# MonsieurETM/QPSK

Measured on AMD Instinct MI355X. Metric: complex Msamples/s demodulated + % HBM roofline, 2400-baud RRC+Costas path, higher is better.
Workload: dtype f32

## Files before the change

### include/qpsk_hip.h

```cpp
#ifndef QPSK_HIP_H
#define QPSK_HIP_H

#include <stddef.h>
#include <stdint.h>

#ifdef __cplusplus
extern "C" {
#endif

#define QPSK_NTAPS 127

typedef enum {
    QPSK_OK = 0,
    QPSK_ERR_NO_DEVICE = -1,
    QPSK_ERR_ARG = -2,
    QPSK_ERR_HIP = -3,
    QPSK_ERR_ALLOC = -4,
    QPSK_ERR_STATE = -5,
    QPSK_ERR_RANGE = -6
} qpsk_status;

typedef enum {
    QPSK_TIMING_HIST = 0,
    QPSK_TIMING_FIXED = 1,
    QPSK_TIMING_FFT = 2
} qpsk_timing_mode;

typedef struct {
    double fs;
    double rs;
    int frame_size;
    float rrc_alpha;
    float loop_bw;
    float min_freq;
    float max_freq;
    int timing_mode;
    int fixed_index;
} qpsk_params;

typedef struct qpsk_ctx qpsk_ctx;

const char *qpsk_last_error(void);
const char *qpsk_version(void);
int qpsk_device_count(void);

void qpsk_params_default(qpsk_params *p);

int qpsk_ctx_create(qpsk_ctx **out, int device, const qpsk_params *p, void *stream);
void qpsk_ctx_destroy(qpsk_ctx *ctx);
int qpsk_ctx_sync(qpsk_ctx *ctx);
int qpsk_ctx_check(qpsk_ctx *ctx);
int qpsk_ctx_set_stream(qpsk_ctx *ctx, void *stream);
int qpsk_ctx_set_tuning(qpsk_ctx *ctx, const char *name, int value);
int qpsk_ctx_cycles(const qpsk_ctx *ctx);
int qpsk_ctx_nsym(const qpsk_ctx *ctx);
const char *qpsk_ctx_last_kernel(const qpsk_ctx *ctx);

int qpsk_ctx_get_taps(const qpsk_ctx *ctx, float h_taps[QPSK_NTAPS]);
int qpsk_ctx_get_gains(const qpsk_ctx *ctx, float *h_alpha, float *h_beta);
int qpsk_ctx_set_taps(qpsk_ctx *ctx, const float h_taps[QPSK_NTAPS]);
int qpsk_ctx_set_loop(qpsk_ctx *ctx, float alpha, float beta, float min_freq, float max_freq);

int qpsk_rx_batch(qpsk_ctx *ctx, const float *d_in, int nframes, uint8_t *d_sym, float *d_freq,
                  float *d_phase, float *d_costas, int32_t *d_index, float *d_hz);

int qpsk_rx_batch_pitched(qpsk_ctx *ctx, const float *d_in, long long frame_pitch, int nframes, uint8_t *d_sym,
                          float *d_freq, float *d_phase, float *d_costas, int32_t *d_index, float *d_hz);

int qpsk_rx_batch_bw(qpsk_ctx *ctx, const float *d_in, int nframes, const float *h_loop_bw, int nbw,
                     uint8_t *d_sym, float *d_freq, float *d_phase, int32_t *d_index);

int qpsk_rx_batch_ext(qpsk_ctx *ctx, const float *d_in, long long frame_pitch, int nframes, const int32_t *d_index_in,
                      const float *d_seed, uint8_t *d_sym, float *d_freq, float *d_phase, float *d_costas, int32_t *d_index,
                      float *d_hz);
int qpsk_rx_batch_data(qpsk_ctx *ctx, const float *d_in, long long frame_pitch, int nframes, const int32_t *d_index_in,
                       const float *d_seed, uint8_t *d_data, uint8_t *d_sym, float *d_freq, float *d_phase, int32_t *d_index,
                       float *d_hz);

int qpsk_sync_batch(qpsk_ctx *ctx, const uint8_t *d_data, int nframes, int nsym, const uint8_t *h_sync, int nsync, int lag_min,
                    int lag_max, int nout, uint8_t *d_out, int32_t *d_lag, int32_t *d_rot, int32_t *d_score);

int qpsk_deframer_reset(qpsk_ctx *ctx, int nstreams, const uint8_t *h_sync, int nsync, int min_score, int nbytes, int max_packets);
int qpsk_deframer_push(qpsk_ctx *ctx, const float *d_costas, const uint8_t *d_data, int nsym, int32_t *d_count, uint8_t *d_bytes,
                       long long *d_pos, int32_t *d_rot, int32_t *d_score, uint8_t *d_crc_ok);

int qpsk_deframer_reset_coded(qpsk_ctx *ctx, int nstreams, const uint8_t *h_sync, int nsync, int min_score, int nbytes,
                              int max_packets, int mode, float scale);
int qpsk_deframer_push_coded(qpsk_ctx *ctx, const float *d_costas, int nsym, const float *d_gain, int32_t *d_count,
                             uint8_t *d_bytes, long long *d_pos, int32_t *d_rot, int32_t *d_score, uint8_t *d_crc_ok,
                             int32_t *d_info);

int qpsk_deframer_reset_coded_punct(qpsk_ctx *ctx, int nstreams, const uint8_t *h_sync, int nsync, int min_score, int nbytes,
                                    int max_packets, int mode, float scale, int period, uint32_t keep0, uint32_t keep1);

int qpsk_rx_batch_bw_ext(qpsk_ctx *ctx, const float *d_in, int nframes, const float *h_loop_bw, int nbw, const int32_t *d_index_in,
                         const float *d_seed, uint8_t *d_sym, float *d_freq, float *d_phase, int32_t *d_index);

int qpsk_carrier_est_batch(qpsk_ctx *ctx, const float *d_in, long long frame_pitch, int nframes, int start, int n,
                           float *d_seed, float *d_freq, int32_t *d_bin, double *d_line);

enum { QPSK_SOFT_UNIT = 0, QPSK_SOFT_LLR = 1 };
int qpsk_soft_batch(qpsk_ctx *ctx, const float *d_costas, long long row_pitch, int nrows, int nsym, int skip, int mode, float scale,
                    const float *d_gain_in, const int32_t *d_lag, const int32_t *d_rot, int first, int nout, int8_t *d_soft,
                    float *d_quality, double *d_sums);

enum { QPSK_CONV_TAIL = 1 };
enum { QPSK_VITERBI_OPEN_START = 1, QPSK_VITERBI_OPEN_END = 2 };
int qpsk_conv_encode_batch(qpsk_ctx *ctx, const uint8_t *d_bits, int nrows, int nbits, int flags, uint8_t *d_dibits);
int qpsk_viterbi_batch(qpsk_ctx *ctx, const int8_t *d_soft, long long row_pitch, int nrows, int nsteps, const uint8_t *d_flip,
                       int flags, uint8_t *d_bits, int32_t *d_info);

#define QPSK_PUNCT_1_2 1, 0x1u, 0x1u
#define QPSK_PUNCT_2_3 2, 0x1u, 0x3u
#define QPSK_PUNCT_3_4 3, 0x5u, 0x3u
#define QPSK_PUNCT_5_6 5, 0x15u, 0x0Bu
#define QPSK_PUNCT_7_8 7, 0x51u, 0x2Fu
int qpsk_punct_ntx(int nsteps, int period, uint32_t keep0, uint32_t keep1);
int qpsk_conv_encode_punct_batch(qpsk_ctx *ctx, const uint8_t *d_bits, int nrows, int nbits, int flags, int period, uint32_t keep0,
                                 uint32_t keep1, uint8_t *d_dibits);
int qpsk_viterbi_punct_batch(qpsk_ctx *ctx, const int8_t *d_soft, long long row_pitch, int nrows, int nsteps, int period, uint32_t keep0,
                             uint32_t keep1, const uint8_t *d_flip, int flags, uint8_t *d_bits, int32_t *d_info);

enum { QPSK_FRAME_UNCODED = 0, QPSK_FRAME_CODED = 1 };
int qpsk_frame_len(int nsync, int nbytes, int coding, int period, uint32_t keep0, uint32_t keep1);
int qpsk_frame_batch(qpsk_ctx *ctx, const uint8_t *d_payload, long long payload_pitch, int nrows, int per_row, int nbytes,
                     const uint8_t *h_sync, int nsync, int coding, int period, uint32_t keep0, uint32_t keep1, int lead, int gap,
                     int row_len, uint8_t *d_out, uint16_t *d_crc);

int qpsk_ilv_stride(int nbits, int want);
int qpsk_conv_encode_ilv_batch(qpsk_ctx *ctx, const uint8_t *d_bits, int nrows, int nbits, int flags, int period, uint32_t keep0,
                               uint32_t keep1, int stride, uint8_t *d_dibits);
int qpsk_viterbi_ilv_batch(qpsk_ctx *ctx, const int8_t *d_soft, long long row_pitch, int nrows, int nsteps, int period, uint32_t keep0,
                           uint32_t keep1, int stride, const uint8_t *d_flip, int flags, uint8_t *d_bits, int32_t *d_info);
int qpsk_frame_batch_ilv(qpsk_ctx *ctx, const uint8_t *d_payload, long long payload_pitch, int nrows, int per_row, int nbytes,
                         const uint8_t *h_sync, int nsync, int coding, int period, uint32_t keep0, uint32_t keep1, int stride, int lead,
                         int gap, int row_len, uint8_t *d_out, uint16_t *d_crc);
int qpsk_deframer_reset_coded_ilv(qpsk_ctx *ctx, int nstreams, const uint8_t *h_sync, int nsync, int min_score, int nbytes,
                                  int max_packets, int mode, float scale, int period, uint32_t keep0, uint32_t keep1, int stride);

int qpsk_rs_generator(int nroots, uint8_t *h_g);
int qpsk_rs_encode_batch(qpsk_ctx *ctx, const uint8_t *d_data, long long data_pitch, int nrows, int k, int nroots, uint8_t *d_out,
                         long long out_pitch);
int qpsk_rs_decode_batch(qpsk_ctx *ctx, const uint8_t *d_in, long long in_pitch, int nrows, int n, int nroots, const uint8_t *d_erase,
                         uint8_t *d_out, long long out_pitch, int32_t *d_info);

enum { QPSK_VITERBI_STREAM_TERMINATED = 1 };
int qpsk_viterbi_stream_reset(qpsk_ctx *ctx, int nstreams, int depth, int window, int period, uint32_t keep0, uint32_t keep1);
int qpsk_viterbi_stream_emits(qpsk_ctx *ctx, int ntx);
int qpsk_viterbi_stream_push(qpsk_ctx *ctx, const int8_t *d_soft, long long row_pitch, int ntx, uint8_t *d_bits, long long bits_pitch,
                             int32_t *d_info, int *h_nbits);
int qpsk_viterbi_stream_flush(qpsk_ctx *ctx, int flags, uint8_t *d_bits, long long bits_pitch, int32_t *d_info, int *h_nbits);
int qpsk_conv_encode_stream_batch(qpsk_ctx *ctx, const uint8_t *d_bits, int nrows, int nbits, int period, uint32_t keep0, uint32_t keep1,
                                  const uint8_t *d_state_in, uint8_t *d_state_out, uint8_t *d_dibits);


int qpsk_rrc_fir_batch(qpsk_ctx *ctx, float *d_memory, const float *d_in, float *d_out, int nframes, int length);

int qpsk_rrc_fir_batch_fast(qpsk_ctx *ctx, float *d_memory, const float *d_in, float *d_out, int nframes, int length);

int qpsk_timing_hist_batch(qpsk_ctx *ctx, const float *d_filtered, int nframes, int32_t *d_index, int32_t *d_hist);

int qpsk_timing_scan_batch(qpsk_ctx *ctx, const float *d_in, int nframes, int32_t *d_index, int32_t *d_hist);

int qpsk_timing_fft_batch(qpsk_ctx *ctx, const float *d_in, int nframes, int32_t *d_index, float *d_filtered,
                          double *d_spectrum);

int qpsk_timing_fft_bin_batch(qpsk_ctx *ctx, const float *d_in, int nframes, int32_t *d_index, float *d_filtered,
                              double *d_bin);

int qpsk_costas_batch(qpsk_ctx *ctx, const float *d_symbols_in, int nframes, int nsym, float *d_state,
                      uint8_t *d_sym, float *d_costas);

int qpsk_fft_batch(qpsk_ctx *ctx, const double *d_in, double *d_out, int nbatch, int n, int inverse);

int qpsk_streams_reset(qpsk_ctx *ctx, int nstreams, double mixer_hz);
int qpsk_streams_set_loop_state(qpsk_ctx *ctx, const float *h_state);
int qpsk_streams_get_loop_state(qpsk_ctx *ctx, float *h_state);
int qpsk_streams_rx_cplx(qpsk_ctx *ctx, const float *d_in, uint8_t *d_sym, float *d_freq, float *d_phase,
                         float *d_costas, int32_t *d_index);
int qpsk_streams_rx_pcm(qpsk_ctx *ctx, const int16_t *d_pcm, uint8_t *d_sym, float *d_freq, float *d_phase,
                        float *d_costas, int32_t *d_index);
int qpsk_streams_rx_pcm_host(qpsk_ctx *ctx, const int16_t *h_pcm, float *h_loop_io, uint8_t *h_sym, float *h_costas,
                             int32_t *h_index);

int qpsk_tx_reset(qpsk_ctx *ctx, int nstreams, double tx_hz);
int qpsk_tx_symbols(qpsk_ctx *ctx, const uint8_t *d_symbols, int nsym, int16_t *d_pcm, float *d_baseband);


int qpsk_crc16_batch(qpsk_ctx *ctx, const uint8_t *d_data, int npackets, int nbytes, uint16_t *d_crc);

int qpsk_interleave_batch(qpsk_ctx *ctx, uint8_t *d_data, int npackets, int nbytes, int dir);

int qpsk_scramble_batch(qpsk_ctx *ctx, uint8_t *d_sym, int npackets, int nsym);

typedef struct qpsk_multi qpsk_multi;
int qpsk_multi_create(qpsk_multi **out, const int *devices, int ndev, const qpsk_params *p);
void qpsk_multi_destroy(qpsk_multi *mj);
int qpsk_multi_shards(const qpsk_multi *mj);
int qpsk_multi_load(qpsk_multi *mj, long long total_frames, const float *h_in);
int qpsk_multi_shard(qpsk_multi *mj, int r, int *device, long long *first, long long *count, qpsk_ctx **ctx, float **d_in);
int qpsk_multi_use_device_input(qpsk_multi *mj, int r, const float *d_in);
int qpsk_multi_set_direct_output(qpsk_multi *mj, int slot, uint8_t *h_sym, float *h_freq, float *h_phase);
int qpsk_multi_set_packed(qpsk_multi *mj, int on);
int qpsk_pack_symbols(qpsk_ctx *ctx, const uint8_t *d_sym, long long nrows, int nsym, uint8_t *d_packed);
int qpsk_unpack_symbols_host(const uint8_t *h_packed, long long nrows, int nsym, uint8_t *h_sym);
int qpsk_host_alloc(void **h_ptr, size_t bytes);
int qpsk_host_free(void *h_ptr);
int qpsk_multi_set_acquisition(qpsk_multi *mj, const int32_t *h_index, const float *h_seed);
int qpsk_multi_set_data(qpsk_multi *mj, int on);
int qpsk_multi_rx_begin(qpsk_multi *mj, int slot);
int qpsk_multi_rx_end(qpsk_multi *mj, int slot, uint8_t *h_sym, float *h_freq, float *h_phase);

int qpsk_dev_alloc(qpsk_ctx *ctx, void **d_ptr, size_t bytes);
int qpsk_dev_free(qpsk_ctx *ctx, void *d_ptr);
int qpsk_dev_upload(qpsk_ctx *ctx, void *d_dst, const void *h_src, size_t bytes);
int qpsk_dev_download(qpsk_ctx *ctx, void *h_dst, const void *d_src, size_t bytes);

int qpsk_selftest_sincos_hash(qpsk_ctx *ctx, uint32_t first, uint32_t count, unsigned long long *h_out);

int qpsk_test_inject_status(qpsk_ctx *ctx, int code);
int qpsk_test_hist_state(qpsk_ctx *ctx, int32_t *out);
int qpsk_test_fir_runs(qpsk_ctx *ctx, int nframes, int length, int32_t out[3]);
int qpsk_test_viterbi_launches(qpsk_ctx *ctx, int *out);
int qpsk_test_deframer_advance(qpsk_ctx *ctx, long long delta);
int qpsk_test_viterbi_stream_advance(qpsk_ctx *ctx, long long delta);

#ifdef __cplusplus
}
#endif
#endif
```

### qpsk_amd/csrc/api_ctx.cpp

```cpp
#include "api_ctx.h"

using namespace qpsk;

static thread_local char g_err[512] = "";

int qpsk::fail(int code, const char *fmt, ...)
{
    va_list ap;
    va_start(ap, fmt);
    vsnprintf(g_err, sizeof g_err, fmt, ap);
    va_end(ap);
    return code;
}

static const struct { const char *name; int Tuning::*field; } TUNING_KEYS[] = {
    {"QPSK_FUSED_G", &Tuning::fused_g},       {"QPSK_FUSED_S", &Tuning::fused_s},     {"QPSK_FUSED_LDS", &Tuning::fused_lds},
    {"QPSK_FUSED_GENERIC", &Tuning::generic}, {"QPSK_PIPE_NF", &Tuning::pipe_nf},
    {"QPSK_PIPE_DBG", &Tuning::pipe_variant}, {"QPSK_HIST_GENERIC", &Tuning::hist_generic},
    {"QPSK_PIPE_V", &Tuning::pipe_v},         {"QPSK_PIPE_G", &Tuning::pipe_g},
    {"QPSK_PIPE_LAYOUT_LO", &Tuning::layout_lo}, {"QPSK_PIPE_LAYOUT_HI", &Tuning::layout_hi},
    {"QPSK_FIR_GENERIC", &Tuning::fir_generic}, {"QPSK_FFT_FUSED", &Tuning::fft_fused},
    {"QPSK_STREAM_BLOCK", &Tuning::stream_block}, {"QPSK_STREAM_POLL", &Tuning::stream_poll},
    {"QPSK_STREAM_SCAN", &Tuning::stream_scan}, {"QPSK_STREAM_CARRIER", &Tuning::stream_carrier},
    {"QPSK_LEAN_DMA", &Tuning::lean_dma},     {"QPSK_LEAN_PAIR", &Tuning::lean_pair},
    {"QPSK_EST_WAVES", &Tuning::est_waves},   {"QPSK_HIST_ONEPASS", &Tuning::hist_onepass},
    {"QPSK_VITERBI_LDS", &Tuning::viterbi_lds},   {"QPSK_VITERBI_CHUNK_ROWS", &Tuning::viterbi_chunk_rows},
};

int qpsk::ensure(qpsk_ctx *c, DevBuf &b, size_t bytes)
{
    if (b.cap >= bytes) return QPSK_OK;
    if (b.p) {
        HIP_TRY(hipStreamSynchronize(c->stream));
        HIP_TRY(hipFree(b.p));
        b.p = nullptr;
        b.cap = 0;
    }
    hipError_t e = hipMalloc(&b.p, bytes);
    if (e != hipSuccess) {
        b.p = nullptr;
        return fail(QPSK_ERR_ALLOC, "hipMalloc(%zu bytes): %s", bytes, hipGetErrorString(e));
    }
    b.cap = bytes;
    return QPSK_OK;
}

int qpsk::check_status(qpsk_ctx *c)
{
    const int st = __atomic_exchange_n(c->status.h_status, 0, __ATOMIC_ACQ_REL);
    if (st != STATUS_PIPE_TIMEOUT) c->streams.stream_work_unchecked = false;
    if (st == STATUS_PIPE_TIMEOUT) {
        if (c->streams.nstreams > 0 && c->streams.stream_work_unchecked) c->streams.poison();
        c->streams.stream_work_unchecked = false;
        return fail(QPSK_ERR_HIP, "pipeline kernel: producer/consumer wait timed out; results of the calls since the last synchronisation are invalid");
    }
    if (st == STATUS_PHASE_RANGE)
        return fail(QPSK_ERR_RANGE, "Costas loop phase beyond the bounded 2 pi wrap (input amplitude far outside the modem's range; "
                                    "the reference's phase_wrap() would spin or hang, costas_loop.c:61-67); results of the calls since the last synchronisation are invalid");
    if (st == STATUS_BAD_INDEX)
        return fail(QPSK_ERR_ARG, "an external timing offset (qpsk_rx_batch_ext d_index_in) lies outside 0..%d: the kernel demodulated that frame "
                                  "at offset 0; results of the calls since the last synchronisation are invalid", MAX_INDEX);
    if (st == STATUS_EST_NONFINITE)
        return fail(QPSK_ERR_RANGE, "qpsk_carrier_est_batch: a NaN / Inf sample inside the window the estimate reads; results of the calls since "
                                    "the last synchronisation are invalid");
    if (st == STATUS_SOFT_NONFINITE)
        return fail(QPSK_ERR_RANGE, "qpsk_soft_batch / qpsk_deframer_push_coded: a NaN / Inf sample among those a row's sums or soft output use, or a NaN / Inf gain; "
                                    "results of the calls since the last synchronisation are invalid");
    if (st == STATUS_SOFT_BAD_LAG)
        return fail(QPSK_ERR_ARG, "qpsk_soft_batch: a lag in d_lag is negative or puts the payload beyond the row (that row's soft output is zeros); "
                                  "results of the calls since the last synchronisation are invalid");
    if (st == STATUS_NONFINITE)
        return fail(QPSK_ERR_RANGE, "a Costas loop ended on a NaN / Inf state: the input held a non-finite sample (the reference hangs in phase_wrap() "
                                    "on an infinite phase, costas_loop.c:61-67); results of the calls since the last synchronisation are invalid");
    if (st != 0) return fail(QPSK_ERR_HIP, "kernel status %d", st);
    return QPSK_OK;
}

int qpsk_test_inject_status(qpsk_ctx *c, int code)
{
    if (!c || !c->status.h_status) return fail(QPSK_ERR_ARG, "null context");
    __atomic_store_n(c->status.h_status, code, __ATOMIC_RELEASE);
    return QPSK_OK;
}

int qpsk::bind(const qpsk_ctx *c)
{
    HIP_TRY(hipSetDevice(c->device));
    return QPSK_OK;
}

int qpsk::use_context_gains(qpsk_ctx *c)
{
    const float g[2] = {c->alpha, c->beta};
    if (c->h_gains.size() != 2 || c->h_gains[0] != g[0] || c->h_gains[1] != g[1]) {
        HIP_TRY(hipStreamSynchronize(c->stream));
        c->h_gains.assign(g, g + 2);
        HIP_TRY(hipMemcpyAsync(c->d_gains, c->h_gains.data(), sizeof g, hipMemcpyHostToDevice, c->stream));
    }
    return QPSK_OK;
}

const char *qpsk_last_error(void) { return g_err; }
const char *qpsk_version(void) { return "qpsk_hip 0.3 (gfx950)"; }

int qpsk_device_count(void)
{
    int n = 0;
    if (hipGetDeviceCount(&n) != hipSuccess) return 0;
    return n;
}

void qpsk_params_default(qpsk_params *p)
{
    if (!p) return;
    p->fs = 9600.0;
    p->rs = 2400.0;
    p->frame_size = 512;
    p->rrc_alpha = .35f;
    p->loop_bw = (float)(2.0 * 3.14159265358979323846 / 100.0f);
    p->min_freq = -1.0f;
    p->max_freq = 1.0f;
    p->timing_mode = QPSK_TIMING_HIST;
    p->fixed_index = 0;
}

static int upload_config(qpsk_ctx *c)
{
    float t128[128];
    memset(t128, 0, sizeof t128);
    memcpy(t128, c->taps, sizeof c->taps);
    c->taps_symmetric = true;
    for (int k = 0; k < QPSK_NTAPS / 2; k++)
        if (memcmp(&c->taps[k], &c->taps[QPSK_NTAPS - 1 - k], sizeof(float)) != 0) c->taps_symmetric = false;
    HIP_TRY(hipMemcpyAsync(c->d_taps, t128, sizeof t128, hipMemcpyHostToDevice, c->stream));
    const float g[2] = {c->alpha, c->beta};
    c->h_gains.assign(g, g + 2);
    HIP_TRY(hipMemcpyAsync(c->d_gains, c->h_gains.data(), sizeof g, hipMemcpyHostToDevice, c->stream));
    HIP_TRY(hipStreamSynchronize(c->stream));
    return QPSK_OK;
}

int qpsk_ctx_create(qpsk_ctx **out, int device, const qpsk_params *p, void *stream)
{
    if (!out || !p) return fail(QPSK_ERR_ARG, "qpsk_ctx_create: null argument");
    *out = nullptr;
    int ndev = 0;
    hipError_t e = hipGetDeviceCount(&ndev);
    if (e != hipSuccess || ndev <= 0)
        return fail(QPSK_ERR_NO_DEVICE, "no HIP device available (%s); this library has no CPU path",
                    e == hipSuccess ? "device count 0" : hipGetErrorString(e));
    if (device < 0) HIP_TRY(hipGetDevice(&device));
    if (device >= ndev) return fail(QPSK_ERR_NO_DEVICE, "device %d out of range (%d devices)", device, ndev);
    if (!(p->fs > 0.0) || !(p->rs > 0.0) || p->frame_size <= 0)
        return fail(QPSK_ERR_ARG, "fs, rs and frame_size must be positive");
    const int cycles = (int)(p->fs / p->rs);
    if (cycles < 1 || cycles > 64) return fail(QPSK_ERR_ARG, "CYCLES = (int)(fs/rs) = %d out of range 1..64", cycles);
    if (p->frame_size % cycles != 0)
        return fail(QPSK_ERR_ARG, "frame_size %d is not a multiple of CYCLES %d", p->frame_size, cycles);
    if (p->timing_mode < QPSK_TIMING_HIST || p->timing_mode > QPSK_TIMING_FFT)
        return fail(QPSK_ERR_ARG, "unknown timing_mode %d", p->timing_mode);
    if (p->fixed_index < 0 || p->fixed_index > MAX_INDEX)
        return fail(QPSK_ERR_ARG, "fixed_index %d outside 0..%d", p->fixed_index, MAX_INDEX);

    HIP_TRY(hipSetDevice(device));
    KERNEL_TRY(prepare_kernels());
    KERNEL_TRY(prepare_pipe_kernel());
    KERNEL_TRY(prepare_timing_scan());
    KERNEL_TRY(prepare_stream_block());
    KERNEL_TRY(prepare_stream_scan());
    KERNEL_TRY(prepare_carrier_est());
    qpsk_ctx *c = new qpsk_ctx();
    c->device = device;
    for (const auto &k : TUNING_KEYS) {
        const char *v = getenv(k.name);
        if (!v || !*v) continue;
        if (k.field == &Tuning::viterbi_chunk_rows) {
            char *end = nullptr;
            const long n = strtol(v, &end, 10);
            if (end == v || *end) continue;
            c->tune.*(k.field) = n < 0 ? -1 : n > INT_MAX ? INT_MAX : (int)n;
            continue;
        }
        c->tune.*(k.field) = atoi(v);
    }
    if (c->tune.viterbi_chunk_rows == 0) {
        delete c;
        return fail(QPSK_ERR_ARG, "qpsk_ctx_create: QPSK_VITERBI_CHUNK_ROWS = 0 in the environment (>= 1, or negative for the library's own choice)");
    }
    {
        int ncu = 0;
        if (hipDeviceGetAttribute(&ncu, hipDeviceAttributeMultiprocessorCount, device) == hipSuccess && ncu > 0)
            c->ncu = ncu;
    }
    c->prm = *p;
    c->cycles = cycles;
    c->nsym = p->frame_size / cycles;
    c->stream = (hipStream_t)stream;
    qpsk_host_rrc_taps((float)p->fs, (float)p->rs, p->rrc_alpha, c->taps);
    c->damping = sqrtf(2.0f) / 2.0f;
    qpsk_host_loop_gains(c->damping, p->loop_bw, &c->alpha, &c->beta);
    c->min_freq = p->min_freq;
    c->max_freq = p->max_freq;
    if (hipMalloc((void **)&c->d_taps, 128 * sizeof(float)) != hipSuccess ||
        hipMalloc((void **)&c->d_gains, MAX_BW * 2 * sizeof(float)) != hipSuccess ||
        hipHostMalloc((void **)&c->status.h_status, sizeof(int), hipHostMallocMapped) != hipSuccess ||
        hipHostGetDevicePointer((void **)&c->status.d_status, c->status.h_status, 0) != hipSuccess) {
        qpsk_ctx_destroy(c);
        return fail(QPSK_ERR_ALLOC, "hipMalloc of configuration buffers failed");
    }
    *c->status.h_status = 0;
    if (hipHostMalloc((void **)&c->streams.h_done, sizeof(unsigned), hipHostMallocMapped) != hipSuccess ||
        hipHostGetDevicePointer((void **)&c->streams.d_done, c->streams.h_done, 0) != hipSuccess) {
        qpsk_ctx_destroy(c);
        return fail(QPSK_ERR_ALLOC, "pinned counter");
    }
    *c->streams.h_done = 0;
    int rc = upload_config(c);
    if (rc != QPSK_OK) { qpsk_ctx_destroy(c); return rc; }
    *out = c;
    return QPSK_OK;
}

void qpsk_ctx_destroy(qpsk_ctx *c)
{
    if (!c) return;
    hipSetDevice(c->device);
    hipStreamSynchronize(c->stream);
    hipFree(c->d_taps);
    hipFree(c->d_gains);
    if (c->status.h_status) hipHostFree(c->status.h_status);
    if (c->streams.h_done) hipHostFree(c->streams.h_done);
    for (DevBuf *b : {&c->index, &c->filtered, &c->mixed, &c->keystream, &c->sympad, &c->mislist, &c->datacostas, &c->vitdec, &c->softgain, &c->dfstage})
        b->release();
    for (auto &kv : c->twiddles) hipFree(kv.second);
    hipFree(c->d_fast);
    c->hist.release();
    c->streams.release();
    c->tx.release();
    c->df.release();
    c->framer.release();
    c->vs.release();
    delete c;
}

int qpsk_ctx_sync(qpsk_ctx *c)
{
    if (!c) return fail(QPSK_ERR_ARG, "null context");
    HIP_TRY(hipSetDevice(c->device));
    HIP_TRY(hipStreamSynchronize(c->stream));
    return check_status(c);
}

int qpsk_pack_symbols(qpsk_ctx *c, const uint8_t *d_sym, long long nrows, int nsym, uint8_t *d_packed)
{
    if (!c || !d_sym || !d_packed || nrows < 0 || nsym <= 0) return fail(QPSK_ERR_ARG, "qpsk_pack_symbols: bad argument");
    if (bind(c)) return QPSK_ERR_HIP;
    if ((nsym & 15) == 0 && (((uintptr_t)d_sym & 15) || ((uintptr_t)d_packed & 3)))
        return fail(QPSK_ERR_ARG, "qpsk_pack_symbols: d_sym must be 16-byte and d_packed 4-byte aligned");
    KERNEL_TRY(launch_pack_dibits(d_sym, d_packed, (size_t)nrows, nsym, c->stream));
    return QPSK_OK;
}

int qpsk_unpack_symbols_host(const uint8_t *h_packed, long long nrows, int nsym, uint8_t *h_sym)
{
    if (!h_packed || !h_sym || nrows < 0 || nsym <= 0) return fail(QPSK_ERR_ARG, "qpsk_unpack_symbols_host: bad argument");
    const size_t pb = (size_t)(nsym + 3) / 4;
    for (long long r = 0; r < nrows; r++) {
        const uint8_t *p = h_packed + (size_t)r * pb;
        uint8_t *o = h_sym + (size_t)r * (size_t)nsym;
        for (int i = 0; i < nsym; i++) o[i] = (uint8_t)((p[i >> 2] >> (2 * (i & 3))) & 3u);
    }
    return QPSK_OK;
}

int qpsk_ctx_check(qpsk_ctx *c)
{
    if (!c) return fail(QPSK_ERR_ARG, "null context");
    return check_status(c);
}

extern "C" int qpsk_set_error(int code, const char *msg)
{
    return fail(code, "%s", msg ? msg : "");
}

int qpsk_ctx_set_stream(qpsk_ctx *c, void *stream)
{
    if (!c) return fail(QPSK_ERR_ARG, "null context");
    HIP_TRY(hipSetDevice(c->device));
    HIP_TRY(hipStreamSynchronize(c->stream));
    c->stream = (hipStream_t)stream;
    return QPSK_OK;
}

int qpsk_ctx_set_tuning(qpsk_ctx *c, const char *name, int value)
{
    if (!c || !name) return fail(QPSK_ERR_ARG, "null argument");
    for (const auto &k : TUNING_KEYS)
        if (!strcmp(k.name, name)) {
            if (value == 0 && k.field == &Tuning::viterbi_chunk_rows)
                return fail(QPSK_ERR_ARG, "qpsk_ctx_set_tuning: QPSK_VITERBI_CHUNK_ROWS = 0 (>= 1, or negative for the library's own choice)");
            c->tune.*(k.field) = value < 0 ? -1 : value;
            return QPSK_OK;
        }
    return fail(QPSK_ERR_ARG, "qpsk_ctx_set_tuning: unknown name '%s'", name);
}

int qpsk_ctx_cycles(const qpsk_ctx *c) { return c ? c->cycles : 0; }
int qpsk_ctx_nsym(const qpsk_ctx *c) { return c ? c->nsym : 0; }
const char *qpsk_ctx_last_kernel(const qpsk_ctx *c) { return c ? c->last_kernel : ""; }

int qpsk_ctx_get_taps(const qpsk_ctx *c, float *h)
{
    if (!c || !h) return fail(QPSK_ERR_ARG, "null argument");
    memcpy(h, c->taps, sizeof c->taps);
    return QPSK_OK;
}

int qpsk_ctx_get_gains(const qpsk_ctx *c, float *a, float *b)
{
    if (!c || !a || !b) return fail(QPSK_ERR_ARG, "null argument");
    *a = c->alpha;
    *b = c->beta;
    return QPSK_OK;
}

int qpsk_ctx_set_taps(qpsk_ctx *c, const float *h)
{
    if (!c || !h) return fail(QPSK_ERR_ARG, "null argument");
    if (bind(c)) return QPSK_ERR_HIP;
    memcpy(c->taps, h, sizeof c->taps);
    c->fast_valid = false;
    return upload_config(c);
}

int qpsk_ctx_set_loop(qpsk_ctx *c, float alpha, float beta, float min_freq, float max_freq)
{
    if (!c) return fail(QPSK_ERR_ARG, "null argument");
    if (bind(c)) return QPSK_ERR_HIP;
    c->min_freq = min_freq; c->max_freq = max_freq;
    if (alpha == c->alpha && beta == c->beta && !(alpha == 0.0f && beta == 0.0f)) return QPSK_OK;
    c->alpha = alpha; c->beta = beta;
    return upload_config(c);
}

int qpsk_dev_alloc(qpsk_ctx *c, void **d_ptr, size_t bytes)
{
    if (!c || !d_ptr) return fail(QPSK_ERR_ARG, "null argument");
    if (bind(c)) return QPSK_ERR_HIP;
    hipError_t e = hipMalloc(d_ptr, bytes);
    if (e != hipSuccess) return fail(QPSK_ERR_ALLOC, "hipMalloc(%zu): %s", bytes, hipGetErrorString(e));
    return QPSK_OK;
}

int qpsk_dev_free(qpsk_ctx *c, void *d_ptr)
{
    if (!c) return fail(QPSK_ERR_ARG, "null argument");
    if (bind(c)) return QPSK_ERR_HIP;
    HIP_TRY(hipStreamSynchronize(c->stream));
    HIP_TRY(hipFree(d_ptr));
    return QPSK_OK;
}

int qpsk_dev_upload(qpsk_ctx *c, void *d_dst, const void *h_src, size_t bytes)
{
    if (!c || !d_dst || !h_src) return fail(QPSK_ERR_ARG, "null argument");
    if (bind(c)) return QPSK_ERR_HIP;
    HIP_TRY(hipMemcpyAsync(d_dst, h_src, bytes, hipMemcpyHostToDevice, c->stream));
    HIP_TRY(hipStreamSynchronize(c->stream));
    return QPSK_OK;
}

int qpsk_dev_download(qpsk_ctx *c, void *h_dst, const void *d_src, size_t bytes)
{
    if (!c || !h_dst || !d_src) return fail(QPSK_ERR_ARG, "null argument");
    if (bind(c)) return QPSK_ERR_HIP;
    HIP_TRY(hipMemcpyAsync(h_dst, d_src, bytes, hipMemcpyDeviceToHost, c->stream));
    HIP_TRY(hipStreamSynchronize(c->stream));
    return check_status(c);
}

int qpsk_selftest_sincos_hash(qpsk_ctx *c, uint32_t first, uint32_t count, unsigned long long *h_out)
{
    if (!c || !h_out) return fail(QPSK_ERR_ARG, "null argument");
    if (bind(c)) return QPSK_ERR_HIP;
    unsigned long long *d = nullptr;
    HIP_TRY(hipMalloc((void **)&d, sizeof *d));
    HIP_TRY(hipMemsetAsync(d, 0, sizeof *d, c->stream));
    KERNEL_TRY(launch_sincos_hash(first, count, d, c->stream));
    HIP_TRY(hipMemcpyAsync(h_out, d, sizeof *d, hipMemcpyDeviceToHost, c->stream));
    HIP_TRY(hipStreamSynchronize(c->stream));
    HIP_TRY(hipFree(d));
    return QPSK_OK;
}
```

### qpsk_amd/csrc/api_ctx.h

```cpp
#ifndef QPSK_API_CTX_H
#define QPSK_API_CTX_H

#include "../../include/qpsk_hip.h"
#include "host_math.h"
#include "kernels.h"

#include <hip/hip_runtime.h>
#include <limits.h>
#include <math.h>
#include <stdarg.h>
#include <stdio.h>
#include <stdlib.h>
#include <string.h>
#include <time.h>
#include <algorithm>
#include <initializer_list>
#include <map>
#include <vector>

struct qpsk_ctx;

namespace qpsk {

QPSK_UNIT_LOCAL int fail(int code, const char *fmt, ...);

#define HIP_TRY(expr)                                                                         \
    do {                                                                                      \
        hipError_t e_ = (expr);                                                               \
        if (e_ != hipSuccess)                                                                 \
            return fail(QPSK_ERR_HIP, "%s: %s (%s:%d)", #expr, hipGetErrorString(e_), __FILE__, __LINE__); \
    } while (0)

#define KERNEL_TRY(expr)                                                                      \
    do {                                                                                      \
        (void)hipGetLastError();  \
        int e_ = (expr);                                                                      \
        if (e_ != 0)                                                                          \
            return fail(QPSK_ERR_HIP, "%s: %s (%s:%d)", #expr, hipGetErrorString((hipError_t)e_), __FILE__, __LINE__); \
    } while (0)

struct QPSK_UNIT_LOCAL DevBuf {
    void *p = nullptr;
    size_t cap = 0;
    void release() { hipFree(p); *this = DevBuf(); }
};

struct Tuning {
    int fused_g = -1, fused_s = -1, fused_lds = -1;
    int generic = -1;
    int pipe_nf = -1;
    int pipe_v = -1, pipe_g = -1;
    int layout_lo = -1, layout_hi = -1;
    int pipe_variant = -1;
    int hist_generic = -1;
    int fir_generic = -1;
    int stream_scan = -1;
    int stream_poll = -1;
    int stream_block = -1;
    int stream_carrier = -1;
    int lean_dma = -1;
    int hist_onepass = -1;
    int est_waves = -1;
    int lean_pair = -1;
    int viterbi_lds = -1;
    int fft_fused = -1;
    int viterbi_chunk_rows = -1;
};

static inline int tuned(int v, int dflt) { return v >= 0 ? v : dflt; }


struct StatusWord {
    int *h_status = nullptr;
    int *d_status = nullptr;
};

struct QPSK_UNIT_LOCAL HistGuess {
    int32_t *d_hint = nullptr;
    int32_t *h_hist_stats = nullptr, *d_hist_stats = nullptr;
    bool hint_valid = false;
    void release();
};

struct QPSK_UNIT_LOCAL Streams {
    int nstreams = 0;
    float *s_memory = nullptr, *s_dec = nullptr, *s_loop = nullptr, *s_mixer = nullptr;
    float *s_ctab = nullptr, *s_cstate = nullptr;
    bool carrier_shared = false;
    unsigned carrier_blocks = 0;
    unsigned carrier_scans = 0;
    float *carrier_pending = nullptr;
    bool stream_work_unchecked = false;
    bool streams_poisoned = false;
    unsigned char *h_stage = nullptr, *d_stage = nullptr;
    size_t stage_cap = 0;
    unsigned *h_done = nullptr, *d_done = nullptr;
    unsigned done_expect = 0;
    void poison()
    {
        streams_poisoned = true;
        carrier_shared = false;
        carrier_pending = nullptr;
    }
    void release();
};

struct QPSK_UNIT_LOCAL Transmitters {
    int ntx = 0;
    uint8_t *t_hist = nullptr;
    float *t_mixer = nullptr;
    DevBuf tx_b;
    void release();
};

struct QPSK_UNIT_LOCAL Deframer {
    uint8_t *state = nullptr, *tables = nullptr;
    size_t stride = 0;
    int nstreams = 0, nsync = 0, min_score = 0, nbytes = 0, max_packets = 0;
    unsigned long long sync_lo[2] = {0, 0}, sync_hi[2] = {0, 0};
    bool ready = false;
    bool coded = false;
    int mode = 0, nsteps = 0;
    int nbody = 0;
    CodedLayout layout;
    float scale = 0.f;
    unsigned crc_init = 0;
    void release();
};

struct QPSK_UNIT_LOCAL Framer {
    uint8_t *ks = nullptr;
    int ks_len = 0;
    void release();
};

struct QPSK_UNIT_LOCAL ViterbiStream {
    uint8_t *state = nullptr;
    size_t stride = 0;
    int nstreams = 0, depth = 0, window = 0;
    Puncture punct = {1, 1u, 1u, 2};
    bool punctured = false;
    long long total = 0;
    long long advanced = 0;
    void release();
};

}

struct qpsk_ctx {
    int device = 0;
    qpsk::Tuning tune;
    int ncu = 256;
    const char *last_kernel = "";
    int viterbi_launches = 0;
    bool taps_symmetric = false;
    hipStream_t stream = nullptr;
    qpsk_params prm{};
    int cycles = 0, nsym = 0;
    float taps[QPSK_NTAPS];
    float damping = 0.f, alpha = 0.f, beta = 0.f;
    float min_freq = 0.f, max_freq = 0.f;
    float *d_taps = nullptr;
    float *d_gains = nullptr;
    std::vector<float> h_gains;
    qpsk::DevBuf index, filtered, mixed, keystream, sympad, mislist;
    qpsk::DevBuf datacostas;
    qpsk::DevBuf vitdec;
    qpsk::DevBuf softgain;
    qpsk::DevBuf dfstage;
    int keystream_len = 0;
    std::map<int, double *> twiddles;
    float *d_fast = nullptr;
    bool fast_valid = false;
    qpsk::StatusWord status;
    qpsk::HistGuess hist;
    qpsk::Streams streams;
    qpsk::Transmitters tx;
    qpsk::Deframer df;
    qpsk::Framer framer;
    qpsk::ViterbiStream vs;
};

namespace qpsk {

static const int MAX_BW = 64;

QPSK_UNIT_LOCAL int ensure(qpsk_ctx *c, DevBuf &b, size_t bytes);
QPSK_UNIT_LOCAL int check_status(qpsk_ctx *c);
QPSK_UNIT_LOCAL int bind(const qpsk_ctx *c);
QPSK_UNIT_LOCAL int use_context_gains(qpsk_ctx *c);

QPSK_UNIT_LOCAL int fir_full_rate(qpsk_ctx *c, const float *x, const float *memory, float *y, int nframes, int length, size_t in_pitch = 0);
QPSK_UNIT_LOCAL int fft_timing_indices(qpsk_ctx *c, const float *d_in, int nframes, int32_t *d_index, float *d_y = nullptr,
                                       double *d_X = nullptr, size_t pitch = 0, double *d_bin = nullptr);
QPSK_UNIT_LOCAL int costas_over_symbols(qpsk_ctx *c, float *d_symbols, int nframes, int nsym, int dstride, float *d_state,
                                        uint8_t *d_sym, float *d_costas, const float *refill = nullptr,
                                        const int32_t *refill_index = nullptr, bool refill_planar = false);

struct Pattern {
    int period;
    uint32_t keep0, keep1;
};
QPSK_UNIT_LOCAL int layout_add_pattern(const char *who, const Pattern *pattern, CodedLayout *l);
QPSK_UNIT_LOCAL int layout_add_stride(const char *who, int nsteps, const int *stride, CodedLayout *l);
struct ViterbiRoute {
    size_t per_row;
    bool lds;
    size_t chunk_rows;
};
QPSK_UNIT_LOCAL ViterbiRoute viterbi_route(const qpsk_ctx *c, size_t rows, int nsteps);

}

#endif
```

### qpsk_amd/csrc/api_rx.cpp

```cpp
#include "api_ctx.h"

using namespace qpsk;

#ifdef QPSK_PIPE_PROFILE
static const int PIPE_VARIANT_MASK = ~0;
#else
static const int PIPE_VARIANT_MASK = 4 | 8 | 16 | 64 | 128 | 256 | 512 | 1024 | 8192;
#endif

int qpsk_test_hist_state(qpsk_ctx *c, int32_t *out)
{
    if (!c || !out) return fail(QPSK_ERR_ARG, "null argument");
    out[0] = out[1] = out[2] = out[3] = out[4] = -1;
    if (!c->hist.d_hint) return QPSK_OK;
    HIP_TRY(hipSetDevice(c->device));
    HIP_TRY(hipStreamSynchronize(c->stream));
    int32_t h[2];
    HIP_TRY(hipMemcpy(h, c->hist.d_hint, sizeof h, hipMemcpyDeviceToHost));
    out[0] = c->hist.hint_valid ? h[0] : -1;
    out[1] = h[1];
    out[2] = c->hist.h_hist_stats[0]; out[3] = c->hist.h_hist_stats[1]; out[4] = c->hist.h_hist_stats[2];
    return QPSK_OK;
}

int qpsk_test_fir_runs(qpsk_ctx *c, int nframes, int length, int32_t out[3])
{
    if (!c || !out) return fail(QPSK_ERR_ARG, "qpsk_test_fir_runs: null argument");
    if (nframes < 1 || length < 1) return fail(QPSK_ERR_ARG, "qpsk_test_fir_runs: nframes %d length %d", nframes, length);
    const FirRuns r = rrc_fir_stream_runs(nframes, length, c->ncu);
    out[0] = r.ntiles; out[1] = r.parts; out[2] = r.tpp;
    return QPSK_OK;
}

void HistGuess::release()
{
    if (d_hint) hipFree(d_hint);
    if (h_hist_stats) hipHostFree(h_hist_stats);
    *this = HistGuess();
}

static bool fir_takes_stream(const qpsk_ctx *c) { return c->taps_symmetric && tuned(c->tune.fir_generic, 0) == 0; }

int qpsk::fir_full_rate(qpsk_ctx *c, const float *x, const float *memory, float *y, int nframes, int length, size_t in_pitch)
{
    if (fir_takes_stream(c))
        return launch_rrc_fir_stream(x, memory, y, c->d_taps, nframes, length, c->stream, in_pitch, c->ncu);
    return launch_rrc_fir(x, memory, y, c->d_taps, nframes, length, c->stream, in_pitch);
}

static void pick_tiling(const qpsk_ctx *c, int nframes, int nbw, int *G, int *S)
{
    int g = nframes / 256;
    if (g < 1) g = 1;
    if (g > 64 / nbw) g = 64 / nbw;
    if (g < 1) g = 1;
    g = tuned(c->tune.fused_g, g);
    if (g < 1) g = 1;
    if (g * nbw > 64) g = 64 / nbw;
    int s = tuned(c->tune.fused_s, 64);
    s &= ~7;
    if (s < 8) s = 8;
    const size_t budget = (size_t)tuned(c->tune.fused_lds, 64 * 1024);
    while (s > 8 && fused_lds_bytes(g, s, c->cycles, nbw) > budget) s -= 8;
    while (g > 1 && fused_lds_bytes(g, s, c->cycles, nbw) > (size_t)MAX_LDS_BYTES) g--;
    *G = g;
    *S = s;
}

static int get_twiddles(qpsk_ctx *c, int n, double **out)
{
    auto it = c->twiddles.find(n);
    if (it != c->twiddles.end()) { *out = it->second; return QPSK_OK; }
    const size_t cnt = n >= 2 ? (size_t)n / 2 : 1;
    std::vector<double> h(2 * cnt, 0.0);
    qpsk_host_twiddles(n, h.data());
    double *tw = nullptr;
    HIP_TRY(hipMalloc((void **)&tw, sizeof(double) * 2 * cnt));
    HIP_TRY(hipMemcpy(tw, h.data(), sizeof(double) * 2 * cnt, hipMemcpyHostToDevice));
    c->twiddles[n] = tw;
    *out = tw;
    return QPSK_OK;
}

static int fft_timing_tables(qpsk_ctx *c, double **tw_out, double **cs_out)
{
    const int C = c->cycles, nfft = timing_fft_nfft();
    if (C < 2 || C > 8 || (C & (C - 1)))
        return fail(QPSK_ERR_ARG, "QPSK_TIMING_FFT needs CYCLES in {2,4,8} (the symbol-rate bin NFFT/CYCLES must be exact and the offset < 8); CYCLES = %d", C);
    if (c->prm.frame_size < timing_fft_first() + nfft)
        return fail(QPSK_ERR_ARG, "QPSK_TIMING_FFT needs frame_size >= %d", timing_fft_first() + nfft);
    double *tw = nullptr;
    int rc = get_twiddles(c, nfft, &tw);
    if (rc) return rc;
    double *cs = nullptr;
    auto it = c->twiddles.find(-C);
    if (it == c->twiddles.end()) {
        std::vector<double> full(2 * (size_t)C);
        qpsk_host_phases(C, full.data());
        HIP_TRY(hipMalloc((void **)&cs, sizeof(double) * 2 * C));
        HIP_TRY(hipMemcpy(cs, full.data(), sizeof(double) * 2 * C, hipMemcpyHostToDevice));
        c->twiddles[-C] = cs;
    } else {
        cs = it->second;
    }
    *tw_out = tw;
    *cs_out = cs;
    return QPSK_OK;
}

int qpsk::fft_timing_indices(qpsk_ctx *c, const float *d_in, int nframes, int32_t *d_index, float *d_y, double *d_X, size_t pitch, double *d_bin)
{
    double *tw = nullptr, *cs = nullptr;
    int rc = fft_timing_tables(c, &tw, &cs);
    if (rc) return rc;
    KERNEL_TRY(launch_timing_fft(d_in, nframes, c->prm.frame_size, c->cycles, c->d_taps, tw, cs, d_index, d_y, d_X, d_bin, c->stream, pitch,
                                 c->ncu, c->taps_symmetric && tuned(c->tune.fir_generic, 0) == 0));
    return QPSK_OK;
}

static bool scan_fused_ok(const qpsk_ctx *c, const float *d_in)
{
    return c->cycles == 8 && c->prm.frame_size % timing_scan_tile() == 0 && ((uintptr_t)d_in % 16) == 0 &&
           tuned(c->tune.hist_generic, 0) == 0;
}

static int timing_indices(qpsk_ctx *c, const float *d_in, size_t pitch, int nframes, const int32_t **d_index_out, bool fused_fft = false)
{
    *d_index_out = nullptr;
    if (c->prm.timing_mode == QPSK_TIMING_FIXED) return QPSK_OK;
    int rc = ensure(c, c->index, sizeof(int32_t) * (size_t)nframes);
    if (rc) return rc;
    if (fused_fft && c->prm.timing_mode == QPSK_TIMING_FFT) return QPSK_OK;
    if (c->prm.timing_mode == QPSK_TIMING_HIST) {
        if (scan_fused_ok(c, d_in) && (pitch & 1) == 0) {
            KERNEL_TRY(launch_timing_scan(d_in, nframes, c->prm.frame_size, c->d_taps, (int32_t *)c->index.p, nullptr,
                                          c->status.d_status, c->stream, pitch, c->taps_symmetric && tuned(c->tune.fir_generic, 0) == 0));
            *d_index_out = (const int32_t *)c->index.p;
            return QPSK_OK;
        }
        const size_t bytes = sizeof(float) * 2 * (size_t)nframes * c->prm.frame_size;
        rc = ensure(c, c->filtered, bytes);
        if (rc) return rc;
        KERNEL_TRY(fir_full_rate(c, d_in, nullptr, (float *)c->filtered.p, nframes, c->prm.frame_size, pitch));
        KERNEL_TRY(launch_timing_hist((const float *)c->filtered.p, nframes, c->prm.frame_size, c->cycles,
                                      (int32_t *)c->index.p, nullptr, tuned(c->tune.hist_generic, 0) == 2, c->stream));
        *d_index_out = (const int32_t *)c->index.p;
        return QPSK_OK;
    }
    rc = fft_timing_indices(c, d_in, nframes, (int32_t *)c->index.p, nullptr, nullptr, pitch);
    if (rc) return rc;
    *d_index_out = (const int32_t *)c->index.p;
    return QPSK_OK;
}

struct ExtAcq {
    const int32_t *index;
    const float *seed;
};

enum RxKind { K_GENERIC, K_FUSED_PIPE, K_PIPE2, K_LEAN };

struct RxRoute {
    RxKind kind = K_GENERIC;
    int G = 0;
    int nf = 0;
    unsigned long long layout = 0;
    bool pipe_ok = false;
    bool fused_fft = false;
    bool need_pad = false;
    bool data_rule = false;
    bool need_dump = false;
};

static bool tuned_layout(const qpsk_ctx *c, unsigned long long *layout)
{
    if (c->tune.layout_lo < 0 && c->tune.layout_hi < 0) return false;
    *layout = ((unsigned long long)(unsigned)tuned(c->tune.layout_lo, 0) << 4) | ((unsigned long long)(unsigned)tuned(c->tune.layout_hi, 0) << 24);
    return true;
}

static int rx_route(const qpsk_ctx *c, const FusedArgs &a, bool want_data, RxRoute *rt)
{
    const int nframes = a.nframes, nbw = a.nbw;
    *rt = RxRoute{};
    const bool pipe_ok = rt->pipe_ok = c->cycles == pipe_cycles() && (a.frame_size % 2) == 0 && (a.frame_pitch % 2) == 0 &&
                                       ((uintptr_t)a.x % 16) == 0 && nbw * pipe_frames(1) <= 64 && tuned(c->tune.generic, 0) == 0;
    const int by_size = nframes > 16 * c->ncu ? 2 : 1;
    int pipe_v = tuned(c->tune.pipe_v, by_size);
    unsigned long long own_layout = 0;
    const bool has_layout = tuned_layout(c, &own_layout);

    if (pipe_ok && c->taps_symmetric && (pipe_v == 3 || c->tune.pipe_v < 0) && !(want_data && !a.data_rule)) {
        int G = tuned(c->tune.pipe_g, (nframes + c->ncu - 1) / c->ncu);
        if (G > pipe2_max_frames()) G = pipe2_max_frames();
        G += G & 1;
        const bool wanted = pipe_v == 3 || G >= 4;
        const unsigned long long layout = has_layout ? own_layout : G >= 2 ? lean_default_layout(G / 2) : 0;
        if (wanted && layout && lean_shape_ok(a, G)) {
            const LayoutCount n = layout_count(layout);
            if (n.units == G / 2 && lean_lds_bytes(G, n.nwin) <= (size_t)MAX_LDS_BYTES) {
                rt->kind = K_LEAN;
                rt->G = G;
                rt->layout = layout;
                rt->need_pad = nframes % G != 0;
                rt->data_rule = a.data_rule != 0;
            }
        }
    }
    const bool older = rt->kind != K_LEAN && pipe_ok;
    if (pipe_v == 3) pipe_v = by_size;
    if (older && pipe_v == 2) {
        int G = tuned(c->tune.pipe_g, (nframes + c->ncu - 1) / c->ncu);
        if (G > pipe2_max_frames()) G = pipe2_max_frames();
        if (G * nbw > 64) G = 64 / nbw;
        if (G < 1) G = 1;
        unsigned long long layout = own_layout;
        if (has_layout) {
            const LayoutCount n = layout_count(layout);
            if (n.units < 1 || (G + 1) / 2 != n.units || pipe2_lds_bytes(G, n.nwin, nbw) > (size_t)MAX_LDS_BYTES)
                return fail(QPSK_ERR_ARG, "QPSK_PIPE_LAYOUT_*: %d units on %d waves do not match %d frames per workgroup", n.units, n.nwin, G);
        } else {
            for (;;) {
                layout = pipe2_default_layout((G + 1) / 2);
                if (layout && pipe2_lds_bytes(G, layout_count(layout).nwin, nbw) <= (size_t)MAX_LDS_BYTES) break;
                if (G == 1) return fail(QPSK_ERR_ARG, "pipeline geometry does not fit: %d loops per frame", nbw);
                G--;
            }
        }
        rt->kind = K_PIPE2;
        rt->G = G;
        rt->layout = layout;
    } else if (older) {
        const int full = pipe_max_nf();
        int nf = 1;
        while (nf < full && (long long)c->ncu * pipe_frames(nf) < nframes) nf++;
        nf = tuned(c->tune.pipe_nf, nf);
        if (nf < 1) nf = 1;
        if (nf > full) nf = full;
        while (pipe_frames(nf) * nbw > 64 || pipe_lds_bytes(nf, nbw) > (size_t)MAX_LDS_BYTES) {
            if (nf == 1) return fail(QPSK_ERR_ARG, "pipeline geometry does not fit: nf %d, %d loops per frame", nf, nbw);
            nf--;
        }
        rt->kind = K_FUSED_PIPE;
        rt->nf = nf;
    }
    rt->need_dump = want_data && !rt->data_rule && !a.costas;
    rt->fused_fft = c->prm.timing_mode == QPSK_TIMING_FFT && !a.index && nbw == 1 && tuned(c->tune.fft_fused, 1) != 0 &&
                    a.frame_size >= timing_fft_first() + timing_fft_nfft() &&
                    ((rt->kind == K_FUSED_PIPE && rt->nf == pipe_max_nf() && !(a.dbg & (128 | 4))) ||
                     (rt->kind == K_LEAN && lean_est_ok(a, rt->G, rt->layout)));
    return QPSK_OK;
}

static int rx_hist_onepass(qpsk_ctx *c, const FusedArgs &a, const RxRoute &rt, int32_t *d_index, bool *taken)
{
    *taken = false;
    if (!rt.pipe_ok || !c->taps_symmetric || !scan_fused_ok(c, (const float *)a.x) || c->tune.pipe_v >= 0) return QPSK_OK;
    if (!c->hist.d_hint) {
        int32_t *hint = nullptr, *h_stats = nullptr, *d_stats = nullptr;
        hipError_t e = hipMalloc((void **)&hint, 2 * sizeof(int32_t));
        if (e == hipSuccess) e = hipMemset(hint, 0, 2 * sizeof(int32_t));
        if (e == hipSuccess) e = hipHostMalloc((void **)&h_stats, 4 * sizeof(int32_t), hipHostMallocMapped);
        if (e == hipSuccess) e = hipHostGetDevicePointer((void **)&d_stats, h_stats, 0);
        if (e != hipSuccess) {
            if (h_stats) hipHostFree(h_stats);
            if (hint) hipFree(hint);
            return fail(QPSK_ERR_ALLOC, "one-pass histogram route: %s", hipGetErrorString(e));
        }
        h_stats[0] = h_stats[1] = h_stats[2] = -1;
        c->hist.d_hint = hint;
        c->hist.h_hist_stats = h_stats;
        c->hist.d_hist_stats = d_stats;
        c->hist.hint_valid = false;
    }
    const int op = tuned(c->tune.hist_onepass, -1);
    const int seen = __atomic_load_n(&c->hist.h_hist_stats[1], __ATOMIC_ACQUIRE), off_majority = __atomic_load_n(&c->hist.h_hist_stats[2], __ATOMIC_ACQUIRE);
    const bool guess_is_good = seen > 0 && off_majority == 0;
    if (op == 0 || !c->hist.hint_valid || !(op == 1 || guess_is_good) || !rx_hist_shape_ok(a)) return QPSK_OK;
    if (int rc = ensure(c, c->index, sizeof(int32_t) * (size_t)a.nframes)) return rc;
    if (int rc = ensure(c, c->mislist, sizeof(int32_t) * (size_t)a.nframes)) return rc;
    int32_t *mis_count = c->hist.d_hint + 1;
    HIP_TRY(hipMemsetAsync(mis_count, 0, sizeof(int32_t), c->stream));
    KERNEL_TRY(launch_rx_hist(a, (int32_t *)c->index.p, c->hist.d_hint, (int32_t *)c->mislist.p, mis_count, c->status.d_status, c->stream));
    FusedArgs af = a;
    af.index = (const int32_t *)c->index.p;
    af.frame_list = (const int32_t *)c->mislist.p;
    af.frame_list_count = mis_count;
    af.G = 4;
    af.S = 64;
    KERNEL_TRY(launch_rx_fused(af, c->stream));
    KERNEL_TRY(launch_index_majority((const int32_t *)c->index.p, a.nframes, c->hist.d_hint, mis_count, c->hist.d_hist_stats, c->stream));
    c->last_kernel = "rx_hist_kernel (one pass on the guessed index) + rx_fused_kernel (fall-back list)";
    if (d_index)
        HIP_TRY(hipMemcpyAsync(d_index, c->index.p, sizeof(int32_t) * (size_t)a.nframes, hipMemcpyDeviceToDevice, c->stream));
    *taken = true;
    return QPSK_OK;
}

static int rx_launch(qpsk_ctx *c, const FusedArgs &a, const RxRoute &rt)
{
    if (a.est_tw && !(rt.kind == K_FUSED_PIPE && rt.nf == pipe_max_nf()) && rt.kind != K_LEAN)
        return fail(QPSK_ERR_STATE, "internal: in-launch FFT timing estimate planned for a kernel that has none");
    if (a.data_rule && rt.kind != K_LEAN)
        return fail(QPSK_ERR_STATE, "internal: data rule planned for a kernel that has none");
    switch (rt.kind) {
    case K_LEAN:
        KERNEL_TRY(launch_rx_lean(a, rt.G, rt.layout, c->status.d_status, c->stream));
        c->last_kernel = a.est_tw ? "rx_lean_kernel (FFT timing estimate inside the launch)" : "rx_lean_kernel";
        break;
    case K_PIPE2:
        KERNEL_TRY(launch_rx_pipe2(a, rt.G, rt.layout, c->status.d_status, c->stream));
        c->last_kernel = "rx_pipe2_kernel";
        break;
    case K_FUSED_PIPE:
        KERNEL_TRY(launch_rx_fused_pipe(a, rt.nf, c->status.d_status, c->stream));
        c->last_kernel = a.est_tw ? "rx_fused_pipe_kernel (FFT timing estimate inside the launch)" : "rx_fused_pipe_kernel";
        break;
    default:
        KERNEL_TRY(launch_rx_fused(a, c->stream));
        c->last_kernel = "rx_fused_kernel";
    }
    return QPSK_OK;
}

static int rx_batch_common(qpsk_ctx *c, const float *d_in, long long frame_pitch, int nframes, int nbw, uint8_t *d_sym,
                           float *d_freq, float *d_phase, float *d_costas, int32_t *d_index, float *d_hz,
                           const ExtAcq *ext = nullptr, uint8_t *d_data = nullptr)
{
    if (!c || !d_in || !(d_sym || d_data)) return fail(QPSK_ERR_ARG, "qpsk_rx_batch: null context, input or symbol buffer");
    if (nframes <= 0) return fail(QPSK_ERR_ARG, "qpsk_rx_batch: nframes = %d", nframes);
    if (frame_pitch == 0) frame_pitch = c->prm.frame_size;
    if (frame_pitch < c->prm.frame_size)
        return fail(QPSK_ERR_ARG, "qpsk_rx_batch_pitched: frame_pitch %lld below frame_size %d", frame_pitch, c->prm.frame_size);
    if (bind(c)) return QPSK_ERR_HIP;
    FusedArgs a{};
    a.x = reinterpret_cast<const float2 *>(d_in);
    a.frame_pitch = (size_t)frame_pitch;
    a.nframes = nframes;
    a.frame_size = c->prm.frame_size;
    a.cycles = c->cycles;
    a.nsym = c->nsym;
    pick_tiling(c, nframes, nbw, &a.G, &a.S);
    a.fixed_index = c->prm.fixed_index;
    a.dbg = tuned(c->tune.pipe_variant, 0) & PIPE_VARIANT_MASK;
    a.lean_dma = tuned(c->tune.lean_dma, 1) != 0;
    a.lean_twowin = tuned(c->tune.lean_dma, 1) != 2 ? 1 : 0;
    a.est_waves = tuned(c->tune.est_waves, 0);
    a.lean_pair = tuned(c->tune.lean_pair, 3);
    a.taps = c->d_taps;
    a.gains = c->d_gains;
    a.nbw = nbw;
    a.min_freq = c->min_freq;
    a.max_freq = c->max_freq;
    a.rs = c->prm.rs;
    a.sym = d_sym ? d_sym : d_data;
    a.data_rule = d_data && !d_sym;
    a.freq = d_freq;
    a.phase = d_phase;
    a.costas = reinterpret_cast<float2 *>(d_costas);
    a.hz = d_hz;
    a.status = c->status.d_status;
    if (ext) a.index = ext->index;
    if (ext && ext->seed) {
        a.state_in = ext->seed;
        a.seed_setters = 1;
    }

    RxRoute rt;
    if (int rc = rx_route(c, a, d_data != nullptr, &rt)) return rc;

    a.data_rule = rt.data_rule;
    if (rt.need_pad) {
        if (int rc = ensure(c, c->sympad, (size_t)rt.G * (size_t)c->nsym)) return rc;
        a.sym_pad = (uint8_t *)c->sympad.p;
    }
    if (rt.need_dump) {
        if (int rc = ensure(c, c->datacostas, sizeof(float2) * (size_t)nframes * (size_t)c->nsym)) return rc;
        a.costas = (float2 *)c->datacostas.p;
    }

    const bool hist_guess = c->prm.timing_mode == QPSK_TIMING_HIST && !ext;
    if (hist_guess) {
        bool taken = false;
        const int rc = rx_hist_onepass(c, a, rt, d_index, &taken);
        if (rc || taken) return rc;
    }

    const int32_t *idx = a.index;
    if (!idx) {
        if (int rc = timing_indices(c, d_in, (size_t)frame_pitch, nframes, &idx, rt.fused_fft)) return rc;
        a.index = idx;
    }
    if (rt.fused_fft) {
        double *est_tw = nullptr, *est_cs = nullptr;
        if (int rc = fft_timing_tables(c, &est_tw, &est_cs)) return rc;
        a.est_tw = reinterpret_cast<const double2 *>(est_tw);
        a.est_cs = reinterpret_cast<const double2 *>(est_cs);
        a.index_out = d_index ? (int32_t *)c->index.p : nullptr;
        if (d_index) idx = (const int32_t *)c->index.p;
    }

    if (int rc = rx_launch(c, a, rt)) return rc;

    if (hist_guess && c->hist.d_hint && idx && tuned(c->tune.hist_onepass, -1) != 0) {
        KERNEL_TRY(launch_index_majority(idx, nframes, c->hist.d_hint, c->hist.d_hint + 1, c->hist.d_hist_stats, c->stream));
        c->hist.hint_valid = true;
    }
    if (rt.kind == K_LEAN && (nframes & 1)) {
        const size_t last0 = (size_t)((nframes - 1) / rt.G) * (size_t)rt.G;
        HIP_TRY(hipMemcpyAsync(a.sym + (size_t)(nframes - 1) * (size_t)c->nsym, a.sym_pad + ((size_t)(nframes - 1) - last0) * (size_t)c->nsym,
                               (size_t)c->nsym, hipMemcpyDeviceToDevice, c->stream));
    }
    if (d_data && !a.data_rule)
        KERNEL_TRY(launch_data_from_costas(a.costas, d_data, (size_t)nframes * (size_t)c->nsym, c->stream));
    if (d_index) {
        if (idx == d_index) {
        } else if (idx)
            HIP_TRY(hipMemcpyAsync(d_index, idx, sizeof(int32_t) * (size_t)nframes, hipMemcpyDeviceToDevice, c->stream));
        else
            KERNEL_TRY(launch_fill_i32(d_index, nframes, c->prm.fixed_index, c->stream));
    }
    return QPSK_OK;
}

static int rx_prologue(qpsk_ctx *c)
{
    if (!c) return QPSK_OK;
    if (bind(c)) return QPSK_ERR_HIP;
    return use_context_gains(c);
}

int qpsk_rx_batch(qpsk_ctx *c, const float *d_in, int nframes, uint8_t *d_sym, float *d_freq, float *d_phase,
                  float *d_costas, int32_t *d_index, float *d_hz)
{
    if (int rp = rx_prologue(c)) return rp;
    return rx_batch_common(c, d_in, 0, nframes, 1, d_sym, d_freq, d_phase, d_costas, d_index, d_hz);
}

int qpsk_rx_batch_pitched(qpsk_ctx *c, const float *d_in, long long frame_pitch, int nframes, uint8_t *d_sym, float *d_freq,
                          float *d_phase, float *d_costas, int32_t *d_index, float *d_hz)
{
    if (int rp = rx_prologue(c)) return rp;
    if (frame_pitch <= 0) return fail(QPSK_ERR_ARG, "qpsk_rx_batch_pitched: frame_pitch = %lld", frame_pitch);
    return rx_batch_common(c, d_in, frame_pitch, nframes, 1, d_sym, d_freq, d_phase, d_costas, d_index, d_hz);
}

static int rx_batch_bw_impl(qpsk_ctx *c, const float *d_in, int nframes, const float *h_loop_bw, int nbw, uint8_t *d_sym,
                            float *d_freq, float *d_phase, int32_t *d_index, const ExtAcq *ext)
{
    if (!c || !h_loop_bw) return fail(QPSK_ERR_ARG, "qpsk_rx_batch_bw: null argument");
    if (nbw < 1 || nbw > MAX_BW) return fail(QPSK_ERR_ARG, "nbw = %d outside 1..%d", nbw, MAX_BW);
    if (bind(c)) return QPSK_ERR_HIP;
    std::vector<float> g(2 * (size_t)nbw);
    for (int b = 0; b < nbw; b++)
        qpsk_host_loop_gains(c->damping, h_loop_bw[b], &g[2 * b], &g[2 * b + 1]);
    if (g != c->h_gains) {
        HIP_TRY(hipStreamSynchronize(c->stream));
        c->h_gains = g;
        HIP_TRY(hipMemcpyAsync(c->d_gains, c->h_gains.data(), sizeof(float) * g.size(), hipMemcpyHostToDevice, c->stream));
    }
    return rx_batch_common(c, d_in, 0, nframes, nbw, d_sym, d_freq, d_phase, nullptr, d_index, nullptr, ext);
}

int qpsk_rx_batch_bw(qpsk_ctx *c, const float *d_in, int nframes, const float *h_loop_bw, int nbw, uint8_t *d_sym,
                     float *d_freq, float *d_phase, int32_t *d_index)
{
    return rx_batch_bw_impl(c, d_in, nframes, h_loop_bw, nbw, d_sym, d_freq, d_phase, d_index, nullptr);
}

int qpsk_rx_batch_ext(qpsk_ctx *c, const float *d_in, long long frame_pitch, int nframes, const int32_t *d_index_in, const float *d_seed,
                      uint8_t *d_sym, float *d_freq, float *d_phase, float *d_costas, int32_t *d_index, float *d_hz)
{
    if (int rp = rx_prologue(c)) return rp;
    if (frame_pitch < 0) return fail(QPSK_ERR_ARG, "qpsk_rx_batch_ext: frame_pitch = %lld", frame_pitch);
    const ExtAcq ext = {d_index_in, d_seed};
    return rx_batch_common(c, d_in, frame_pitch, nframes, 1, d_sym, d_freq, d_phase, d_costas, d_index, d_hz, &ext);
}

int qpsk_rx_batch_data(qpsk_ctx *c, const float *d_in, long long frame_pitch, int nframes, const int32_t *d_index_in, const float *d_seed,
                       uint8_t *d_data, uint8_t *d_sym, float *d_freq, float *d_phase, int32_t *d_index, float *d_hz)
{
    if (int rp = rx_prologue(c)) return rp;
    if (frame_pitch < 0) return fail(QPSK_ERR_ARG, "qpsk_rx_batch_data: frame_pitch = %lld", frame_pitch);
    if (!d_data) return fail(QPSK_ERR_ARG, "qpsk_rx_batch_data: d_data is NULL");
    const ExtAcq ext = {d_index_in, d_seed};
    return rx_batch_common(c, d_in, frame_pitch, nframes, 1, d_sym, d_freq, d_phase, nullptr, d_index, d_hz, &ext, d_data);
}

int qpsk_sync_batch(qpsk_ctx *c, const uint8_t *d_data, int nframes, int nsym, const uint8_t *h_sync, int nsync, int lag_min, int lag_max,
                    int nout, uint8_t *d_out, int32_t *d_lag, int32_t *d_rot, int32_t *d_score)
{
    if (!c || !d_data || !h_sync) return fail(QPSK_ERR_ARG, "qpsk_sync_batch: null context, data or sync word");
    if (nframes <= 0 || nsym <= 0) return fail(QPSK_ERR_ARG, "qpsk_sync_batch: nframes = %d, nsym = %d", nframes, nsym);
    if (nsync < 1 || nsync > SYNC_MAX_WORD) return fail(QPSK_ERR_ARG, "qpsk_sync_batch: nsync = %d outside 1..%d", nsync, SYNC_MAX_WORD);
    if (nout < 0 || lag_min < 0 || lag_max < lag_min || (long long)lag_max + nsync + nout > nsym)
        return fail(QPSK_ERR_ARG, "qpsk_sync_batch: lags %d..%d, nsync %d, nout %d do not fit a row of %d", lag_min, lag_max, nsync, nout, nsym);
    if (!d_out && !d_lag && !d_rot && !d_score) return fail(QPSK_ERR_ARG, "qpsk_sync_batch: every output is NULL");
    for (int i = 0; i < nsync; i++)
        if (h_sync[i] > 3) return fail(QPSK_ERR_ARG, "qpsk_sync_batch: sync[%d] = %d is not a dibit", i, (int)h_sync[i]);
    if (d_out && nout > 0) {
        const uintptr_t o0 = (uintptr_t)d_out, o1 = o0 + (size_t)nframes * (size_t)nout;
        const uintptr_t d0 = (uintptr_t)d_data, d1 = d0 + (size_t)nframes * (size_t)nsym;
        if (o0 < d1 && d0 < o1) return fail(QPSK_ERR_ARG, "qpsk_sync_batch: d_out overlaps d_data");
    }
    if (bind(c)) return QPSK_ERR_HIP;
    KERNEL_TRY(launch_sync_search(d_data, nframes, nsym, h_sync, nsync, lag_min, lag_max, nout, nout > 0 ? d_out : nullptr, d_lag, d_rot,
                                  d_score, c->stream));
    c->last_kernel = "sync_search_kernel";
    return QPSK_OK;
}

int qpsk_rx_batch_bw_ext(qpsk_ctx *c, const float *d_in, int nframes, const float *h_loop_bw, int nbw, const int32_t *d_index_in,
                         const float *d_seed, uint8_t *d_sym, float *d_freq, float *d_phase, int32_t *d_index)
{
    const ExtAcq ext = {d_index_in, d_seed};
    return rx_batch_bw_impl(c, d_in, nframes, h_loop_bw, nbw, d_sym, d_freq, d_phase, d_index, &ext);
}

int qpsk::costas_over_symbols(qpsk_ctx *c, float *d_symbols, int nframes, int nsym, int dstride, float *d_state,
                              uint8_t *d_sym, float *d_costas, const float *refill, const int32_t *refill_index, bool refill_planar)
{
    float *carrier_tab = c->streams.carrier_pending;
    c->streams.carrier_pending = nullptr;
    if (tuned(c->tune.generic, 0)) {
        if (carrier_tab) KERNEL_TRY(launch_carrier_table(c->streams.s_cstate, carrier_tab, c->prm.frame_size, true, c->stream));
        KERNEL_TRY(launch_costas(d_symbols, nframes, nsym, dstride, 1, c->d_gains, c->min_freq, c->max_freq, d_state, d_state,
                                 d_sym, d_costas, c->status.d_status, c->stream));
        if (refill) {
            if (dstride != nsym) return fail(QPSK_ERR_ARG, "internal: refill needs packed rows");
            KERNEL_TRY(launch_decimate(refill, refill_index, d_symbols, nframes, nsym * c->cycles, c->cycles, nsym, c->stream));
        }
        return QPSK_OK;
    }
    FusedArgs a{};
    a.nframes = nframes;
    a.nsym = nsym;
    a.frame_size = nsym * c->cycles;
    a.cycles = c->cycles;
    a.refill = reinterpret_cast<const float2 *>(refill);
    a.refill_dst = reinterpret_cast<float2 *>(d_symbols);
    a.refill_planar = refill_planar ? 1 : 0;
    a.index = refill_index;
    a.gains = c->d_gains;
    a.nbw = 1;
    a.min_freq = c->min_freq;
    a.max_freq = c->max_freq;
    a.rs = c->prm.rs;
    a.state_in = d_state;
    a.state_out = d_state;
    a.sym = d_sym;
    a.costas = reinterpret_cast<float2 *>(d_costas);
    a.dsrc = reinterpret_cast<const float2 *>(d_symbols);
    a.dstride = dstride;
    a.status = c->status.d_status;
    if (carrier_tab) {
        a.carrier_state = c->streams.s_cstate;
        a.carrier_tab = reinterpret_cast<float2 *>(carrier_tab);
        a.carrier_frame = c->prm.frame_size;
    }
    a.dbg = tuned(c->tune.pipe_variant, 0) & PIPE_VARIANT_MASK;
    int nf = (nframes + c->ncu * pipe_frames(1) - 1) / (c->ncu * pipe_frames(1));
    if (nf < 1) nf = 1;
    if (nf > pipe_max_nf()) nf = pipe_max_nf();
    KERNEL_TRY(launch_costas_pipe(a, nf, c->status.d_status, c->stream));
    return QPSK_OK;
}

int qpsk_rrc_fir_batch(qpsk_ctx *c, float *d_memory, const float *d_in, float *d_out, int nframes, int length)
{
    if (!c || !d_in || !d_out) return fail(QPSK_ERR_ARG, "qpsk_rrc_fir_batch: null argument");
    if (nframes <= 0 || length <= 0) return fail(QPSK_ERR_ARG, "qpsk_rrc_fir_batch: nframes %d length %d", nframes, length);
    if (bind(c)) return QPSK_ERR_HIP;
    const float *src = d_in;
    if (d_in == d_out) {
        const size_t bytes = sizeof(float) * 2 * (size_t)nframes * length;
        int rc = ensure(c, c->mixed, bytes);
        if (rc) return rc;
        HIP_TRY(hipMemcpyAsync(c->mixed.p, d_in, bytes, hipMemcpyDeviceToDevice, c->stream));
        src = (const float *)c->mixed.p;
    }
    KERNEL_TRY(fir_full_rate(c, src, d_memory, d_out, nframes, length));
    c->last_kernel = fir_takes_stream(c) ? "rrc_fir_stream_kernel" : "rrc_fir_kernel";
    if (d_memory) KERNEL_TRY(launch_delay_line(src, d_memory, nframes, length, c->stream));
    return QPSK_OK;
}

int qpsk_rrc_fir_batch_fast(qpsk_ctx *c, float *d_memory, const float *d_in, float *d_out, int nframes, int length)
{
    if (!c || !d_in || !d_out) return fail(QPSK_ERR_ARG, "qpsk_rrc_fir_batch_fast: null argument");
    if (nframes <= 0 || length <= 0) return fail(QPSK_ERR_ARG, "qpsk_rrc_fir_batch_fast: nframes %d length %d", nframes, length);
    if (d_in == d_out) return fail(QPSK_ERR_ARG, "qpsk_rrc_fir_batch_fast: every block reads 126 samples in front of it: separate buffers");
    if (bind(c)) return QPSK_ERR_HIP;
    if (!c->fast_valid) {
        const int n = rrc_fir_fast_nfft();
        std::vector<float> t(4 * (size_t)n);
        qpsk_host_fir_fast_tables(c->taps, t.data(), t.data() + 2 * n);
        if (!c->d_fast) HIP_TRY(hipMalloc((void **)&c->d_fast, sizeof(float) * t.size()));
        HIP_TRY(hipStreamSynchronize(c->stream));
        HIP_TRY(hipMemcpy(c->d_fast, t.data(), sizeof(float) * t.size(), hipMemcpyHostToDevice));
        c->fast_valid = true;
    }
    KERNEL_TRY(launch_rrc_fir_fast(d_in, d_memory, d_out, c->d_fast, c->d_fast + 2 * rrc_fir_fast_nfft(), nframes, length, c->stream));
    if (d_memory) KERNEL_TRY(launch_delay_line(d_in, d_memory, nframes, length, c->stream));
    return QPSK_OK;
}

int qpsk_timing_hist_batch(qpsk_ctx *c, const float *d_filtered, int nframes, int32_t *d_index, int32_t *d_hist)
{
    if (!c || !d_filtered || !d_index) return fail(QPSK_ERR_ARG, "qpsk_timing_hist_batch: null argument");
    if (nframes <= 0) return fail(QPSK_ERR_ARG, "nframes = %d", nframes);
    if (bind(c)) return QPSK_ERR_HIP;
    KERNEL_TRY(launch_timing_hist(d_filtered, nframes, c->prm.frame_size, c->cycles, d_index, d_hist,
                                  tuned(c->tune.hist_generic, 0) == 2, c->stream));
    return QPSK_OK;
}

int qpsk_timing_scan_batch(qpsk_ctx *c, const float *d_in, int nframes, int32_t *d_index, int32_t *d_hist)
{
    if (!c || !d_in || !d_index) return fail(QPSK_ERR_ARG, "qpsk_timing_scan_batch: null argument");
    if (nframes <= 0) return fail(QPSK_ERR_ARG, "nframes = %d", nframes);
    if (bind(c)) return QPSK_ERR_HIP;
    if (!(c->cycles == 8 && c->prm.frame_size % timing_scan_tile() == 0 && ((uintptr_t)d_in % 16) == 0))
        return fail(QPSK_ERR_ARG, "qpsk_timing_scan_batch needs CYCLES = 8, frame_size %% %d == 0 and 16-byte aligned input "
                                  "(use qpsk_rrc_fir_batch + qpsk_timing_hist_batch otherwise)", timing_scan_tile());
    KERNEL_TRY(launch_timing_scan(d_in, nframes, c->prm.frame_size, c->d_taps, d_index, d_hist, c->status.d_status, c->stream, 0,
                                  c->taps_symmetric && tuned(c->tune.fir_generic, 0) == 0));
    return QPSK_OK;
}

int qpsk_timing_fft_batch(qpsk_ctx *c, const float *d_in, int nframes, int32_t *d_index, float *d_filtered, double *d_spectrum)
{
    if (!c || !d_in || !d_index) return fail(QPSK_ERR_ARG, "qpsk_timing_fft_batch: null argument");
    if (nframes <= 0) return fail(QPSK_ERR_ARG, "nframes = %d", nframes);
    if (bind(c)) return QPSK_ERR_HIP;
    return fft_timing_indices(c, d_in, nframes, d_index, d_filtered, d_spectrum);
}

int qpsk_timing_fft_bin_batch(qpsk_ctx *c, const float *d_in, int nframes, int32_t *d_index, float *d_filtered, double *d_bin)
{
    if (!c || !d_in || !d_index) return fail(QPSK_ERR_ARG, "qpsk_timing_fft_bin_batch: null argument");
    if (nframes <= 0) return fail(QPSK_ERR_ARG, "nframes = %d", nframes);
    if (bind(c)) return QPSK_ERR_HIP;
    return fft_timing_indices(c, d_in, nframes, d_index, d_filtered, nullptr, 0, d_bin);
}

static float carrier_est_omega(int k, int C, int n)
{
    const double tau = 2.0 * 3.14159265358979323846;
    return (float)(tau * (double)(k * C) / (double)(4 * n));
}

int qpsk_carrier_est_batch(qpsk_ctx *c, const float *d_in, long long frame_pitch, int nframes, int start, int n, float *d_seed,
                           float *d_freq, int32_t *d_bin, double *d_line)
{
    if (!c || !d_in) return fail(QPSK_ERR_ARG, "qpsk_carrier_est_batch: null context or input");
    if (!d_seed && !d_freq && !d_bin && !d_line) return fail(QPSK_ERR_ARG, "qpsk_carrier_est_batch: every output is NULL");
    if (nframes <= 0) return fail(QPSK_ERR_ARG, "qpsk_carrier_est_batch: nframes = %d", nframes);
    if (n < 64 || n > 8192 || (n & (n - 1)))
        return fail(QPSK_ERR_ARG, "qpsk_carrier_est_batch: n = %d must be a power of two in 64..8192", n);
    const int fs = c->prm.frame_size;
    if (start < 0 || (long long)start + n > fs)
        return fail(QPSK_ERR_ARG, "qpsk_carrier_est_batch: start %d + n %d outside the frame (%d samples)", start, n, fs);
    if (frame_pitch == 0) frame_pitch = fs;
    if (frame_pitch < fs || (frame_pitch % 2) != 0)
        return fail(QPSK_ERR_ARG, "qpsk_carrier_est_batch: frame_pitch = %lld (0, or even and >= frame_size %d)", frame_pitch, fs);
    const int C = c->cycles;
    int klo = 1, khi = 0;
    for (int k = -(n / (2 * C)); k <= n / (2 * C); k++) {
        if ((long long)(k < 0 ? -k : k) * 2 * C >= n) continue;
        const float w = carrier_est_omega(k, C, n);
        if (!(w >= c->min_freq && w <= c->max_freq)) continue;
        if (klo > khi) klo = k;
        khi = k;
    }
    if (klo > khi)
        return fail(QPSK_ERR_ARG, "qpsk_carrier_est_batch: no bin |k| < n / (2 CYCLES) = %d / %d lies in the loop clamp [%g, %g]", n, 2 * C,
                    (double)c->min_freq, (double)c->max_freq);
    const int kdef = klo <= 0 && khi >= 0 ? 0 : (khi < 0 ? khi : klo);
    if (bind(c)) return QPSK_ERR_HIP;
    double *tw = nullptr;
    if (int rt = get_twiddles(c, n, &tw)) return rt;
    KERNEL_TRY(launch_carrier_est(d_in, (size_t)frame_pitch, nframes, start, n, C, klo, khi, kdef, c->d_taps, tw, d_seed, d_freq, d_bin,
                                  d_line, c->status.d_status, c->taps_symmetric && tuned(c->tune.fir_generic, 0) == 0, c->stream));
    c->last_kernel = "carrier_est_kernel";
    return QPSK_OK;
}

int qpsk_costas_batch(qpsk_ctx *c, const float *d_symbols_in, int nframes, int nsym, float *d_state, uint8_t *d_sym,
                      float *d_costas)
{
    if (!c || !d_symbols_in) return fail(QPSK_ERR_ARG, "qpsk_costas_batch: null argument");
    if (nframes <= 0 || nsym <= 0) return fail(QPSK_ERR_ARG, "nframes %d nsym %d", nframes, nsym);
    if (bind(c)) return QPSK_ERR_HIP;
    if (int rg = use_context_gains(c)) return rg;
    return costas_over_symbols(c, const_cast<float *>(d_symbols_in), nframes, nsym, nsym, d_state, d_sym, d_costas);
}

int qpsk_fft_batch(qpsk_ctx *c, const double *d_in, double *d_out, int nbatch, int n, int inverse)
{
    if (!c || !d_in || !d_out) return fail(QPSK_ERR_ARG, "qpsk_fft_batch: null argument");
    if (nbatch <= 0 || n < 1 || (n & (n - 1))) return fail(QPSK_ERR_ARG, "n = %d must be a power of two, nbatch %d > 0", n, nbatch);
    if (n > (1 << 21)) return fail(QPSK_ERR_ARG, "n = %d: transforms above 2^21 points are not supported (the late stages' tile must fit the LDS)", n);
    if (bind(c)) return QPSK_ERR_HIP;
    int log2n = 0;
    while ((1 << log2n) < n) log2n++;
    if (n <= fft_lds_max_n()) {
        double *tw = nullptr;
        if (int rt = get_twiddles(c, n, &tw)) return rt;
        KERNEL_TRY(launch_fft(d_in, d_out, tw, nbatch, n, log2n, inverse ? 1 : 0, c->stream));
        return QPSK_OK;
    }
    double *twb = nullptr, *twn = nullptr;
    if (int rt = get_twiddles(c, fft_big_block(), &twb)) return rt;
    if (int rt = get_twiddles(c, n, &twn)) return rt;
    const double *src = d_in;
    if (d_in == d_out) {
        const size_t bytes = sizeof(double) * 2 * (size_t)nbatch * n;
        int rc = ensure(c, c->mixed, bytes);
        if (rc) return rc;
        HIP_TRY(hipMemcpyAsync(c->mixed.p, d_in, bytes, hipMemcpyDeviceToDevice, c->stream));
        src = (const double *)c->mixed.p;
    }
    KERNEL_TRY(launch_fft_big(src, d_out, twb, twn, nbatch, n, log2n, inverse ? 1 : 0, c->stream));
    return QPSK_OK;
}
```

### qpsk_amd/csrc/kernels.h

```cpp
#ifndef QPSK_KERNELS_H
#define QPSK_KERNELS_H

#include <hip/hip_runtime.h>
#include <stddef.h>
#include <stdint.h>

namespace qpsk {

constexpr int LOOKBACK = 128;
constexpr int LOOKAHEAD = 8;
constexpr int MAX_LDS_BYTES = 160 * 1024;
constexpr int MAX_INDEX = 7;
constexpr int STATUS_PIPE_TIMEOUT = 1;
constexpr int STATUS_PHASE_RANGE = 2;
constexpr int STATUS_NONFINITE = 3;
constexpr int STATUS_BAD_INDEX = 4;
constexpr int STATUS_EST_NONFINITE = 5;
constexpr int STATUS_SOFT_NONFINITE = 6;
constexpr int STATUS_SOFT_BAD_LAG = 7;

struct FusedArgs {
    const float2 *x;
    size_t frame_pitch;
    int nframes, frame_size, cycles, nsym;
    int G, S;
    int mixed;
    int share_simd0;
    const int32_t *index;
    int fixed_index;
    const double2 *est_tw, *est_cs;
    int32_t *index_out;
    int lean_twowin;
    int lean_dma;
    int est_waves;
    int lean_pair;
    int dbg;
    const float2 *dsrc;
    int dstride;
    const float2 *refill;
    float2 *refill_dst;
    int refill_planar;
    const int32_t *frame_list, *frame_list_count;
    const float *taps;
    const float *gains;
    int nbw;
    float min_freq, max_freq;
    double rs;
    const float *state_in;
    int seed_setters;
    float *state_out;
    uint8_t *sym;
    uint8_t *sym_pad;
    float *freq, *phase;
    float2 *costas;
    float *hz;
    int *status;
    float *carrier_state;
    float2 *carrier_tab;
    int carrier_frame;
    int data_rule;
};

size_t fused_lds_bytes(int G, int S, int cycles, int nbw);
int prepare_kernels(void);
int launch_rx_fused(const FusedArgs &a, hipStream_t s);
size_t pipe_lds_bytes(int NF, int nbw);
int pipe_frames(int NF);
int pipe_cycles(void);
int pipe_max_nf(void);
int prepare_pipe_kernel(void);
#define QPSK_UNIT_LOCAL __attribute__((visibility("hidden")))
QPSK_UNIT_LOCAL int prepare_costas_pipe(void);
QPSK_UNIT_LOCAL int prepare_rx_fused_pipe(void);
int launch_rx_fused_pipe(const FusedArgs &a, int NF, int *status, hipStream_t s);
int launch_costas_pipe(const FusedArgs &a, int NF, int *status, hipStream_t s);
size_t pipe2_lds_bytes(int G, int nwin, int nbw);
int pipe2_max_fir(void);
int pipe2_max_frames(void);
int pipe2_max_units_per_wave(void);
int pipe2_max_hw_waves(void);
unsigned long long pipe2_default_layout(int NU);
struct LayoutCount {
    int units, nwin, hw;
    bool share_simd0, valid;
};
inline LayoutCount layout_count(unsigned long long layout, int max_per_wave = pipe2_max_units_per_wave())
{
    LayoutCount n = {0, 0, 1, false, (layout & 15) == 0};
    for (int w = 1; w < 16; w++) {
        const int cw = (int)((layout >> (4 * w)) & 15);
        if (cw > max_per_wave || (cw && w >= pipe2_max_hw_waves())) n.valid = false;
        n.units += cw;
        n.nwin += cw != 0;
        if (cw) n.hw = w + 1;
        if (cw && (w == 4 || w == 8)) n.share_simd0 = true;
    }
    return n;
}
int launch_rx_pipe2(const FusedArgs &a, int G, unsigned long long layout, int *status, hipStream_t s);
QPSK_UNIT_LOCAL int prepare_rx_pipe2(void);
size_t lean_lds_bytes(int G, int nwin);
unsigned long long lean_default_layout(int NU);
bool lean_shape_ok(const FusedArgs &a, int G);
int launch_rx_lean(const FusedArgs &a, int G, unsigned long long layout, int *status, hipStream_t s);
QPSK_UNIT_LOCAL int prepare_rx_lean(void);
bool lean_est_ok(const FusedArgs &a, int G, unsigned long long layout);
bool rx_hist_shape_ok(const FusedArgs &a);
int launch_rx_hist(const FusedArgs &a, int32_t *index_true, const int32_t *hint, int32_t *mis_list, int32_t *mis_count, int *status, hipStream_t s);
int launch_index_majority(const int32_t *index, int nframes, int32_t *hint, int32_t *mis_count, int32_t *h_stats, hipStream_t s);
QPSK_UNIT_LOCAL int prepare_rx_hist(void);
int launch_rrc_fir(const float *x, const float *memory, float *y, const float *taps, int nframes, int length,
                   hipStream_t s, size_t in_pitch = 0);
int launch_rrc_fir_stream(const float *x, const float *memory, float *y, const float *taps, int nframes, int length,
                          hipStream_t s, size_t in_pitch = 0, int ncu = 0);
struct FirRuns { int ntiles, parts, tpp; };
FirRuns rrc_fir_stream_runs(int nframes, int length, int ncu);
int launch_delay_line(const float *x, float *memory, int nframes, int length, hipStream_t s);
int launch_rrc_fir_fast(const float *x, const float *memory, float *y, const float *H, const float *tw, int nframes, int length,
                        hipStream_t s);
int rrc_fir_fast_hop(void);
int rrc_fir_fast_nfft(void);
int launch_timing_hist(const float *y, int nframes, int frame_size, int cycles, int32_t *index, int32_t *hist,
                       bool generic, hipStream_t s);
int launch_costas(const float *d, int nframes, int nsym, int dstride, int nbw, const float *gains, float min_freq,
                  float max_freq, const float *state_in, float *state_out, uint8_t *sym, float *costas, int *status,
                  hipStream_t s);
int launch_decimate(const float *filtered, const int32_t *index, float *dec, int nstreams, int frame_size,
                    int cycles, int nsym, hipStream_t s);
int launch_mixer(const int16_t *pcm, float *out, float *state, int nstreams, int frame_size, hipStream_t s);
int launch_fft(const double *in, double *out, const double *tw, int nbatch, int n, int log2n, int inverse,
               hipStream_t s);
int fft_lds_max_n(void);
int fft_big_block(void);
int launch_fft_big(const double *in, double *out, const double *twb, const double *twn, int nbatch, int n, int log2n,
                   int inverse, hipStream_t s);
size_t timing_scan_lds_bytes(void);
int timing_scan_tile(void);
int prepare_timing_scan(void);
int launch_timing_scan(const float *x, int nframes, int frame_size, const float *taps, int32_t *index, int32_t *hist,
                       int *status, hipStream_t s, size_t pitch = 0, bool symmetric = false);
int launch_timing_fft(const float *x, int nframes, int frame_size, int cycles, const float *taps, const double *tw,
                      const double *cs, int32_t *index, float *yout, double *Xout, double *Xk, hipStream_t s, size_t pitch = 0,
                      int ncu = 0, bool symmetric = false);
int timing_fft_nfft(void);
int timing_fft_first(void);
int prepare_carrier_est(void);
int launch_carrier_est(const float *x, size_t pitch, int nframes, int start, int n, int cycles, int klo, int khi, int kdef,
                       const float *taps, const double *tw, float *seed, float *freq, int32_t *bin, double *line, int *status,
                       bool symmetric, hipStream_t s);
struct StreamBlockArgs {
    const int16_t *pcm;
    const float2 *cplx;
    float *mixer;
    float2 *memory;
    float2 *dec;
    float *loop;
    const float *loop_in;
    float *loop_out;
    const float *taps, *gains;
    float min_freq, max_freq;
    int frame_size, cycles, nsym, hist_timing, fixed_index;
    uint8_t *sym;
    float2 *costas;
    int32_t *index;
    float2 *filtered;
    int *status;
    unsigned *done;
    const float2 *ctab;
    float2 *ctab_next;
    float *cstate;
};
struct StreamBlockInline {
    static constexpr int MAX_STREAMS = 8, MAX_SAMPLES = 1024;
    float loop[2 * MAX_STREAMS];
    uint4 pcm[MAX_SAMPLES / 8];
};
size_t stream_block_lds_bytes(int frame_size, int nsym);
int stream_block_max_frame(void);
int prepare_stream_block(void);
int launch_stream_block(const StreamBlockArgs &a, int nstreams, hipStream_t s, const StreamBlockInline *inl = nullptr);
int stream_scan_tile(void);
int prepare_stream_scan(void);
int launch_stream_scan(const int16_t *pcm, const float *x, float *mixer, float *memory, float *yout, const float *taps, int32_t *index,
                       int nstreams, int frame_size, int *status, hipStream_t s, const float *ctab = nullptr, float *ctab_next = nullptr,
                       float *cstate = nullptr, unsigned cseq = 0, int cycles = 8);
int launch_carrier_table(float *cstate, float *tab, int frame_size, bool rest_only, hipStream_t s);
int launch_carrier_broadcast(const float *cstate, float *mixer, int nstreams, hipStream_t s);
int launch_crc16(const uint8_t *data, int npackets, int nbytes, uint16_t *crc, hipStream_t s);
int launch_interleave(uint8_t *data, int npackets, int nbytes, unsigned b, int dir, hipStream_t s);
int launch_scramble(uint8_t *sym, const uint8_t *keystream, int npackets, int nsym, hipStream_t s);
int launch_pack_dibits(const uint8_t *sym, uint8_t *packed, size_t nrows, int nsym, hipStream_t s);
constexpr int SYNC_MAX_WORD = 128;
int launch_sync_search(const uint8_t *data, int nframes, int nsym, const uint8_t *h_sync, int nsync, int lag_min, int lag_max, int nout,
                       uint8_t *out, int32_t *lag, int32_t *rot, int32_t *score, hipStream_t s);
int launch_data_from_costas(const float2 *costas, uint8_t *data, size_t n, hipStream_t s);
constexpr int SOFT_ONE_PASS_MAX = 4096;
constexpr int SOFT_MAX_NSYM = 1 << 21;
constexpr int SOFT_MODE_UNIT = 0, SOFT_MODE_LLR = 1;
int launch_soft_onepass(const float *x, size_t pitch, int nrows, int nsym, int skip, int mode, float scale, const float *gain_in,
                        const int32_t *lag, const int32_t *rot, int first, int nout, int8_t *soft, float *quality, double *sums, int *status,
                        hipStream_t s);
int launch_soft_sums(const float *x, size_t pitch, int nrows, int nsym, int skip, int mode, float scale, float *gain_out, float *quality,
                     double *sums, int *status, hipStream_t s);
int launch_soft_apply(const float *x, size_t pitch, int nrows, int nsym, const float *gain, bool check_gain, const int32_t *lag,
                      const int32_t *rot, int first, int nout, int8_t *soft, int *status, hipStream_t s);
constexpr int VITERBI_MAX_STEPS = 131072;
constexpr int VITERBI_LDS_MAX_BYTES = 65536;
constexpr int VITERBI_OPEN_START = 1, VITERBI_OPEN_END = 2, VITERBI_PROFILE_FORWARD_ONLY = 0x100, VITERBI_PROFILE_CYCLES = 0x200;
size_t viterbi_scratch_bytes_per_row(int nsteps);
struct Puncture {
    int period;
    unsigned keep0, keep1;
    int K;
};
inline long long punct_nsent(const Puncture &p, int nsteps)
{
    const unsigned r = (unsigned)(nsteps % p.period), low = (1u << r) - 1u;
    return (long long)(nsteps / p.period) * p.K + __builtin_popcount(p.keep0 & low) + __builtin_popcount(p.keep1 & low);
}
struct Interleave {
    unsigned n, s, sinv;
};
struct IlvMul {
    unsigned n, m, m9;
    __host__ __device__ __forceinline__ unsigned at(unsigned k) const { return ((k >> 9) * m9 + (k & 511u) * m) % n; }
    __host__ __device__ __forceinline__ unsigned next(unsigned a) const { return a + m >= n ? a + m - n : a + m; }
    __host__ __device__ __forceinline__ unsigned ahead(unsigned a, unsigned b) const { return b ? next(a) : a; }
};
inline IlvMul ilv_mul(unsigned n, unsigned m) { return IlvMul{n, m, (unsigned)(((unsigned long long)m << 9) % n)}; }
struct FlatMap {
    template <class Pos> __host__ __device__ __forceinline__ Pos at(Pos k) const { return k; }
    template <class Pos> __host__ __device__ __forceinline__ Pos next(Pos a) const { return a + 1; }
    template <class Pos> __host__ __device__ __forceinline__ Pos ahead(Pos a, unsigned b) const { return a + b; }
};
enum CodedKind { CODED_PLAIN = 0, CODED_PUNCT = 1, CODED_ILV = 2 };
struct CodedLayout {
    CodedKind kind = CODED_PLAIN;
    Puncture punct = {1, 1u, 1u, 2};
    Interleave ilv = {2u, 1u, 1u};
};
inline long long coded_nsent(const CodedLayout &l, int nsteps) { return punct_nsent(l.punct, nsteps); }
inline long long coded_ndibits(const CodedLayout &l, int nsteps) { return (coded_nsent(l, nsteps) + 1) / 2; }
inline bool coded_layout_fits(const CodedLayout &l, int nsteps)
{
    if (nsteps < 1 || nsteps > VITERBI_MAX_STEPS || l.punct.period < 1 || l.punct.period > 32 || l.punct.K < 1 || l.punct.K > 64) return false;
    if (l.kind != CODED_ILV) return true;
    const long long ntx = coded_ndibits(l, nsteps);
    return ntx >= 1 && l.ilv.n == 2u * (unsigned)ntx && l.ilv.s >= 1 && l.ilv.s < l.ilv.n && l.ilv.sinv >= 1 && l.ilv.sinv < l.ilv.n;
}
int launch_viterbi(const int8_t *soft, size_t pitch, int nrows, int nsteps, const CodedLayout &layout, const uint8_t *flip, int flags,
                   unsigned long long *scratch, bool lds, uint8_t *bits, int32_t *info, hipStream_t s);
int launch_conv_encode(const uint8_t *bits, int nrows, int nbits, int nsteps, const CodedLayout &layout, uint8_t *dibits, hipStream_t s);
constexpr int VSTREAM_MAX_SPAN = 8192;
constexpr int VSTREAM_TERMINATED = 1;
struct VStreamArgs {
    const int8_t *soft;
    size_t pitch;
    int n, pc, slot, have, wphase;
    int nring, dblk, wblk;
    int flags;
    uint8_t *state;
    size_t state_stride;
    uint8_t *bits;
    size_t bits_pitch;
    int32_t *info;
    Puncture punct;
};
size_t vstream_state_stride(int nring);
int launch_vstream_init(const VStreamArgs &a, int nstreams, hipStream_t s);
int launch_vstream_push(const VStreamArgs &a, int nstreams, bool punctured, hipStream_t s);
int launch_vstream_flush(const VStreamArgs &a, int nstreams, hipStream_t s);
int launch_conv_encode_stream(const uint8_t *bits, int nrows, int nbits, const Puncture &p, const uint8_t *state_in, uint8_t *state_out,
                              uint8_t *dibits, hipStream_t s);
struct DeframeHeader {
    long long len;
    long long h;
    long long ppos;
    int pending, have, prot, pscore;
};
constexpr int DEFRAME_TAIL_OFFSET = 64, DEFRAME_PEND_OFFSET = 192;
constexpr int DEFRAME_MAX_BYTES = 1024, DEFRAME_MAX_PACKETS = 64, DEFRAME_MAX_NSYM = 1 << 21;
struct DeframeHuntArgs {
    int nstreams, nsym;
    int nsync, min_score;
    uint8_t *state;
    size_t state_stride;
    unsigned long long sync_lo[2], sync_hi[2];
    long long *pos;
    int32_t *rot, *score;
    int32_t *count;
};
__device__ __forceinline__ void report(const DeframeHuntArgs &a, size_t r, long long pos, int rot, int score, int lane)
{
    if (a.pos) {
        if (lane == 0) a.pos[r] = pos;
    }
    if (a.rot) {
        if (lane == 0) a.rot[r] = rot;
    }
    if (a.score) {
        if (lane == 0) a.score[r] = score;
    }
}
struct DeframeArgs : DeframeHuntArgs {
    uint8_t *bytes;
    const uint8_t *data;
    const float2 *costas;
    int nbytes, max_packets;
    int bytes_per_lane;
    const uint8_t *keystream;
    const uint16_t *crc_adv;
    uint8_t *crc_ok;
};
int launch_deframe(const DeframeArgs &a, hipStream_t s);
constexpr int DEFRAME_CODED_MAX_STEPS = 8 * (DEFRAME_MAX_BYTES + 2) + 6;
struct DeframeCodedArgs : DeframeHuntArgs {
    uint8_t *bytes;
    const float2 *costas;
    const float *gain;
    int check_gain;
    int nbytes, max_packets;
    int nsteps;
    int per_stream;
    int8_t *stage;
    const uint8_t *flip;
    const uint16_t *crc_adv;
    unsigned crc_init;
    uint8_t *crc_ok;
    int32_t *info;
    int *status;
};
struct DeframeCodedBody {
    int nbody;
    int stage_pitch;
    int kind;
    Puncture punct;
};
int launch_deframe_coded_hunt(const DeframeCodedArgs &a, const DeframeCodedBody &b, hipStream_t s);
int launch_deframe_coded_decode(const DeframeCodedArgs &a, DeframeCodedBody b, const CodedLayout &layout, int row0, int nrows,
                                unsigned long long *scratch, bool lds, hipStream_t s);
constexpr int FRAME_MAX_BYTES = DEFRAME_MAX_BYTES, FRAME_MAX_PER_ROW = 64, FRAME_MAX_ROW = DEFRAME_MAX_NSYM;
struct FrameArgs {
    const uint8_t *payload;
    size_t pitch;
    uint8_t *out;
    uint16_t *crc;
    const uint8_t *ks;
    int npackets, per_row, nbytes, nsync;
    int nbody;
    int lead, gap, row_len;
    int bytes_per_lane;
    int coded;
    unsigned nsent;
    Puncture punct;
};
int launch_frame(const FrameArgs &a, const CodedLayout &layout, const uint8_t *h_sync, const uint16_t *h_crc_adv, hipStream_t s);
constexpr int RS_MAX_ROOTS = 64;
void rs_generator(int nroots, uint8_t *g);
int launch_rs_encode(const uint8_t *data, size_t data_pitch, int nrows, int k, int nroots, uint8_t *out, size_t out_pitch, hipStream_t s);
int launch_rs_decode(const uint8_t *in, size_t in_pitch, int nrows, int n, int nroots, const uint8_t *erase, uint8_t *out, size_t out_pitch,
                     int32_t *info, hipStream_t s);
int tx_history_symbols(void);
int launch_tx_shape(const uint8_t *sym, uint8_t *hist, const float *taps, float *sig, int nstreams, int nsym,
                    int cycles, hipStream_t s);
int launch_tx_upmix(const float *sig, int16_t *pcm, float *state, int nstreams, int length, hipStream_t s);
int launch_fill_i32(int32_t *p, int n, int32_t v, hipStream_t s);
int launch_sincos_hash(uint32_t first, uint32_t count, unsigned long long *acc, hipStream_t s);

}
#endif
```

### qpsk_amd/csrc/rx_lean.hip

```cpp
#include <hip/hip_runtime.h>
#include "qpsk_device.h"
#include "fir_lean_asm.h"
#include "fir_lean_data_asm.h"
#ifdef QPSK_PIPE_PROFILE
#include "fir_lean_prof_asm.h"
#endif
#include "rx_pipe2_geom.h"
#include "fir_full8_asm.h"
#include "timing_fft_wave.h"

namespace qpsk {

namespace lean {
constexpr int PRM_DWORDS = 20;
constexpr int HW_WAVES = pipe2::MAX_THREADS / 64;
constexpr int WS = WS_LEAN_SLOTS;
static_assert(PRM_DWORDS * 4 <= ROW_BYTES - Z_OFFSET_BYTES, "a parameter block fits the record half of a row");
static_assert(FIR_LEAN_END_VGPR <= 168, "three waves per SIMD");
static_assert(FIR_LEAN_WOFF == sizeof(float2) * pipe2::UF * WS, "fir_lean_loop2_dma2w: unit 1's window follows unit 0's");
static_assert(WS % 2 == 0 && pipe2::slot_of(pipe2::PAD * (pipe2::QL - 1) + pipe2::TSTEPS - 1) < WS &&
              pipe2::slot_of(pipe2::CH + HIST - 1) < WS + 16, "window: every position a lane reads, and a frame's spill stays in the next frame's history slots");
__device__ __host__ constexpr int rows_of(int G) { return G > HW_WAVES ? G : HW_WAVES; }
}
constexpr size_t LEAN_EST_LDS_BYTES = 128 * sizeof(float) + 32 * sizeof(int);

__device__ __forceinline__ uint8_t *lean_unit_rows(const FusedArgs &a, int f0, int u)
{
    const int fa = f0 + pipe2::UF * u;
    return fa + pipe2::UF <= a.nframes ? a.sym + (size_t)fa * a.nsym : a.sym_pad + (size_t)(pipe2::UF * u) * a.nsym;
}

template <int NUW>
__device__ __forceinline__ void lean_dma_table(unsigned *tab, float2 *mywin, unsigned ixpack, bool two_windows, int lane)
{
    using namespace pipe2;
    constexpr int WS = lean::WS;
#pragma unroll
    for (int ui = 0; ui < NUW; ui++)
#pragma unroll
        for (int ff = 0; ff < UF; ff++) {
            const int k = 2 * ui + ff;
            const int ix = (int)((ixpack >> (4 * k)) & 15u);
            const int S0 = slot_of(HIST - ix);
            for (int j = 0; j < 4; j++) {
                const int sl = S0 + 2 * (64 * j + lane);
                const int grp = sl / (PAD + PADS);
                int r = sl % (PAD + PADS);
                if (r >= PAD) r = PAD - 2;
                int n = PAD * grp + r - HIST + ix;
                if (n > CH - 2) n = CH - 2;
                tab[(4 * k + j) * 64 + lane] = 8u * (unsigned)n;
            }
            tab[(16 + k) * 64 + lane] = lds_addr(mywin + ((two_windows && ui == 1) ? UF * WS : 0) + ff * WS + S0);
        }
}

template <int NUW, bool DATA>
__device__ __forceinline__ void fir_wave_lean(const FusedArgs &a, lean::Ctl *sm, unsigned char *rows, float2 *mywin,
                                              int hwave, int u0, int f0, int lane, int nchunks, int *status, const int *est)
{
    using namespace pipe2;
    using GM = lean::GeomLean;
    constexpr int WS = lean::WS;
    float2 *dring = reinterpret_cast<float2 *>(rows);
    float *zring = reinterpret_cast<float *>(rows + lean::Z_OFFSET_BYTES);
    const int N = a.nsym;
    const int fl = lane / QL, q = lane % QL;
    const bool simd0 = (hwave & 3) == 0;
    unsigned *prm = reinterpret_cast<unsigned *>(rows + (size_t)hwave * lean::ROW_BYTES + lean::Z_OFFSET_BYTES);
    unsigned ixpack = ((unsigned)(4 * u0) << 16) | (simd0 && !(a.dbg & 1024) ? 0x80000000u : 0u);
#pragma unroll
    for (int ui = 0; ui < NUW; ui++)
#pragma unroll
        for (int ff = 0; ff < UF; ff++) {
            const int fr = f0 + UF * (u0 + ui) + ff;
            const int ix = checked_index(__builtin_amdgcn_readfirstlane(est ? est[UF * (u0 + ui) + ff] : a.index ? a.index[min(fr, a.nframes - 1)] : a.fixed_index), status);
            ixpack |= (unsigned)ix << (4 * (2 * ui + ff));
        }
    const bool use_dma = a.lean_dma && (ixpack & 0x1111u) == 0;
    const bool two_windows = NUW == 2 && a.lean_twowin && use_dma;
    LeanLaneAddr w;
#pragma unroll
    for (int ui = 0; ui < 2; ui++) {
        const int u = u0 + (ui < NUW ? ui : 0);
#pragma unroll
        for (int ff = 0; ff < UF; ff++) {
            const int fr = f0 + UF * u + ff;
            const int ix = (int)((ixpack >> (4 * (2 * (ui < NUW ? ui : 0) + ff))) & 7u);
            const int p0 = 2 * lane + HIST - ix;
            const int wu = (two_windows && ui == 1) ? UF * WS : 0;
            w.wr0[ui][ff] = lds_addr(mywin + wu + ff * WS + slot_of(p0)) - 8u * BLK;
            w.wr1[ui][ff] = lds_addr(mywin + wu + ff * WS + slot_of(p0 + 1)) - 8u * BLK;
            if (lane == 0) {
                const size_t fsrc = prof::frame_number(a, UF * u + ff, (size_t)min(fr, a.nframes - 1));
                const unsigned long long src = prof::frame_source(a, f0, UF * u + ff, (unsigned long long)(a.x + fsrc * a.frame_pitch));
                prm[4 * ui + 2 * ff] = (unsigned)src;
                prm[4 * ui + 2 * ff + 1] = (unsigned)(src >> 32);
            }
        }
        const int g = UF * u + fl;
        w.ring[ui] = lds_addr(dring + (size_t)g * GM::DSTRIDE + R * q);
        w.z[ui] = lds_addr(zring + (size_t)g * GM::ZSTRIDE + R * q);
        if (lane == 0) {
            const unsigned long long sb = (unsigned long long)lean_unit_rows(a, f0, u);
            prm[8 + 2 * ui] = (unsigned)sb;
            prm[8 + 2 * ui + 1] = (unsigned)(sb >> 32);
        }
    }
    w.wlim = lds_addr(mywin + WS + (WS - 2));
    w.wpad = lds_addr(mywin + WS + PAD);
    if (lane == 0) {
        prm[12] = (unsigned)nchunks;
        prm[13] = ixpack;
        prm[16] = (unsigned)(unsigned long long)a.taps;
        prm[17] = (unsigned)((unsigned long long)a.taps >> 32);
    }
    if (simd0 && !(a.dbg & 1024)) __builtin_amdgcn_s_setprio(3);
    const unsigned rd = lds_addr(mywin + fl * WS + (PAD + PADS) * q);
    prof::timeline_stamp(a, lane, 32 + hwave);
    int st;
    if (prof::lean_measured_stream<NUW>(a, lds_addr(prm), rd, 16u * lane, (unsigned)(fl * N + R * q), lds_addr(sm), w, lane, hwave, nchunks, st)) {
    } else if constexpr (DATA) {
        unsigned *tab = reinterpret_cast<unsigned *>(mywin);
        if (use_dma) lean_dma_table<NUW>(tab, mywin, ixpack, two_windows, lane);
        if constexpr (NUW == 2) {
            if (use_dma && two_windows)
                st = fir_lean_loop2_dma2w_data(lds_addr(prm), rd, 16u * lane, (unsigned)(fl * N + R * q), lds_addr(sm), lds_addr(tab + lane), w);
            else if (use_dma)
                st = fir_lean_loop2_dma_data(lds_addr(prm), rd, 16u * lane, (unsigned)(fl * N + R * q), lds_addr(sm), lds_addr(tab + lane), w);
            else
                st = fir_lean_loop2_data(lds_addr(prm), rd, 16u * lane, (unsigned)(fl * N + R * q), lds_addr(sm), w);
        } else if (use_dma)
            st = fir_lean_loop1_dma_data(lds_addr(prm), rd, 16u * lane, (unsigned)(fl * N + R * q), lds_addr(sm), lds_addr(tab + lane), w);
        else
            st = fir_lean_loop1_data(lds_addr(prm), rd, 16u * lane, (unsigned)(fl * N + R * q), lds_addr(sm), w);
    } else if (use_dma) {
        unsigned *tab = reinterpret_cast<unsigned *>(mywin);
#pragma unroll
        for (int ui = 0; ui < NUW; ui++)
#pragma unroll
            for (int ff = 0; ff < UF; ff++) {
                const int k = 2 * ui + ff;
                const int ix = (int)((ixpack >> (4 * k)) & 15u);
                const int S0 = slot_of(HIST - ix);
                for (int j = 0; j < 4; j++) {
                    const int sl = S0 + 2 * (64 * j + lane);
                    const int grp = sl / (PAD + PADS);
                    int r = sl % (PAD + PADS);
                    if (r >= PAD) r = PAD - 2;
                    int n = PAD * grp + r - HIST + ix;
                    if (n > CH - 2) n = CH - 2;
                    tab[(4 * k + j) * 64 + lane] = 8u * (unsigned)n;
                }
                tab[(16 + k) * 64 + lane] = lds_addr(mywin + ((two_windows && ui == 1) ? UF * WS : 0) + ff * WS + S0);
            }
        if constexpr (NUW == 2) {
            if (two_windows)
                st = fir_lean_loop2_dma2w(lds_addr(prm), rd, 16u * lane, (unsigned)(fl * N + R * q), lds_addr(sm), lds_addr(tab + lane), w);
            else
                st = fir_lean_loop2_dma(lds_addr(prm), rd, 16u * lane, (unsigned)(fl * N + R * q), lds_addr(sm), lds_addr(tab + lane), w);
        } else
            st = fir_lean_loop1_dma(lds_addr(prm), rd, 16u * lane, (unsigned)(fl * N + R * q), lds_addr(sm), lds_addr(tab + lane), w);
    } else if constexpr (NUW == 2)
        st = fir_lean_loop2(lds_addr(prm), rd, 16u * lane, (unsigned)(fl * N + R * q), lds_addr(sm), w);
    else
        st = fir_lean_loop1(lds_addr(prm), rd, 16u * lane, (unsigned)(fl * N + R * q), lds_addr(sm), w);
    bool ok = st == 0;
    if (ok) {
        for (int c = nchunks - DR; c < nchunks && ok; c++) {
            ok = wait_ge(&sm->consumed, c + 1, &sm->abort_flag);
            if (ok)
#pragma unroll
                for (int ui = 0; ui < NUW; ui++) {
                    const int g = UF * (u0 + ui) + fl;
                    flush_records<GM, R, DATA>(a, zring, dring, g, f0 + g, q, c, lean_unit_rows(a, f0, u0 + ui) + (size_t)fl * N);
                }
        }
    } else if (lane == 0) {
        __hip_atomic_store(&sm->abort_flag, 1, __ATOMIC_RELAXED, __HIP_MEMORY_SCOPE_WORKGROUP);
    }
    prof::timeline_wave_end(a, lane, hwave);
    if (!ok && lane == 0) report_status(status, STATUS_PIPE_TIMEOUT);
}

template <bool DATA>
__global__ void __launch_bounds__(pipe2::MAX_THREADS)
rx_lean_kernel(FusedArgs a, unsigned long long layout, int nwin, int *status)
{
    using namespace pipe2;
    using GM = lean::GeomLean;
    extern __shared__ __attribute__((aligned(16))) unsigned char smem_raw[];
    lean::Ctl *sm = reinterpret_cast<lean::Ctl *>(smem_raw);
    const int G = a.G;
    float2 *win = reinterpret_cast<float2 *>(smem_raw + sizeof(lean::Ctl));
    unsigned char *rows = reinterpret_cast<unsigned char *>(win + (size_t)nwin * UF * lean::WS);
    const int tid = threadIdx.x, lane = tid & 63;
    const int wave = __builtin_amdgcn_readfirstlane(tid >> 6);
    const int f0 = blockIdx.x * G;
    const int nchunks = a.nsym / S;

    prof::timeline_entry(a, tid);
    if (tid < MAX_WAVES) sm->ready[tid] = 0;
    if (tid == 0) { sm->consumed = 0; sm->abort_flag = 0; }
    const int *est = nullptr;
    if (a.est_tw) {
        float *etaps = reinterpret_cast<float *>(rows + (size_t)lean::rows_of(G) * lean::ROW_BYTES);
        int *eidx = reinterpret_cast<int *>(etaps + 128);
        for (int i = tid; i < 128; i += blockDim.x) etaps[i] = i < NTAPS ? a.taps[i] : 0.0f;
        __syncthreads();
        const int nw = (int)blockDim.x / 64;
        const int room = (int)((size_t)nwin * UF * lean::WS / tfft::WSLOTS);
        const int nwe = nw < room ? nw : room;
        if (wave < nwe) {
            float2 *ewin = win + (size_t)wave * tfft::WSLOTS;
            const unsigned erd = lds_addr(ewin + (tfft::R + tfft::PADS) * lane), etap = lds_addr(etaps);
            tfft::Pre5 pre = tfft::load_frame5(a.x + (size_t)min(f0 + wave, a.nframes - 1) * a.frame_pitch, lane);
            for (int fe = wave; fe < G; fe += nwe) {
                tfft::stage_frame5(ewin, lane, pre);
                if (fe + nwe < G) pre = tfft::load_frame5(a.x + (size_t)min(f0 + fe + nwe, a.nframes - 1) * a.frame_pitch, lane);
                tfft::wave_sync();
                v2f e0, e1, e2, e3, e4, e5, e6, e7;
                fir_full8_asm(erd, etap, e0, e1, e2, e3, e4, e5, e6, e7);
                const v2f eacc[tfft::R] = {e0, e1, e2, e3, e4, e5, e6, e7};
                double epv[tfft::R];
                const tfft::cd u = tfft::power_bin(eacc, ewin, lane, a.est_tw, tfft::NFFT / C, nullptr, epv);
                if (lane == 0) {
                    const int best = tfft::pick_index(u, a.est_cs, C, nullptr);
                    eidx[fe] = best;
                    if (a.index_out && f0 + fe < a.nframes) a.index_out[f0 + fe] = best;
                }
                tfft::wave_sync();
            }
        }
        est = eidx;
    }
    __syncthreads();

    if (wave == 0) {
        if (f0 + G > a.nframes) {
            bool ok = true;
            for (int u = (a.nframes - f0 + UF - 1) / UF; u < G / UF && ok; u++) ok = wait_ge(&sm->ready[u], 1, &sm->abort_flag);
            if (!ok) {
                if (lane == 0) report_status(status, STATUS_PIPE_TIMEOUT);
                return;
            }
        }
        costas_wave<GM>(a, sm, reinterpret_cast<const float2 *>(rows), reinterpret_cast<float *>(rows + lean::Z_OFFSET_BYTES), G,
                        f0, lane, nchunks, status);
        return;
    }
    const int mine = wave < 16 ? (int)((layout >> (4 * wave)) & 15) : 0;
    if (mine == 0) return;
    prof::timeline_stamp(a, lane, 16 + wave);
    int u0 = 0, widx = 0;
    for (int v = 1; v < wave; v++) {
        const int cv = (int)((layout >> (4 * v)) & 15);
        u0 += cv;
        widx += a.lean_twowin ? cv : (cv != 0);
    }
    float2 *mywin = win + (size_t)widx * UF * lean::WS;
    if (mine == 2)
        fir_wave_lean<2, DATA>(a, sm, rows, mywin, wave, u0, f0, lane, nchunks, status, est);
    else
        fir_wave_lean<1, DATA>(a, sm, rows, mywin, wave, u0, f0, lane, nchunks, status, est);
}

size_t lean_lds_bytes(int G, int nwin)
{
    size_t b = sizeof(lean::Ctl) + sizeof(float2) * (size_t)nwin * pipe2::UF * lean::WS + (size_t)lean::rows_of(G) * lean::ROW_BYTES;
    return (b + 15) & ~(size_t)15;
}

unsigned long long lean_default_layout(int NU)
{
    if (NU == 8) {
        static const int c8[12] = {0, 2, 2, 2, 0, 1, 1, 0, 0, 0, 0, 0};
        unsigned long long l8 = 0;
        for (int w = 1; w < 12; w++) l8 |= (unsigned long long)c8[w] << (4 * w);
        return l8;
    }
    if (NU != pipe2::MAX_UNITS) return pipe2_default_layout(NU);
    static const int cnt[12] = {0, 2, 2, 2, 1, 2, 2, 2, 0, 1, 1, 1};
    unsigned long long layout = 0;
    for (int w = 1; w < 12; w++) layout |= (unsigned long long)cnt[w] << (4 * w);
    return layout;
}

bool lean_shape_ok(const FusedArgs &a, int G)
{
    return a.nbw == 1 && !a.costas && (!a.state_in || a.seed_setters) && !a.state_out && a.nsym % pipe2::S == 0 && a.nsym >= 2 * pipe2::S &&
           a.frame_size == a.nsym * C && G >= 2 && G % 2 == 0 && G <= pipe2::UF * pipe2::MAX_UNITS && a.nframes >= 1 &&
           !(a.dbg & (8 | 16));
}

struct LeanGeometry {
    bool ok;
    bool est_ok;
    int units, nwin, hw;
    int hw_est, nwe;
    bool twowin, pair;
    bool share_simd0;
    size_t lds, lds_est;
};

static LeanGeometry lean_geometry(const FusedArgs &a, int G, unsigned long long layout)
{
    using namespace pipe2;
    LeanGeometry g{};
    const LayoutCount n = layout_count(layout, 2);
    g.units = n.units;
    g.nwin = n.nwin;
    g.hw = n.hw;
    g.share_simd0 = n.share_simd0;
    const bool valid = n.valid && G >= 2 && g.units == G / UF && lean_lds_bytes(G, g.nwin) <= (size_t)MAX_LDS_BYTES;
    g.twowin = valid && a.lean_twowin && a.lean_dma && g.units > g.nwin && lean_lds_bytes(G, g.units) <= (size_t)MAX_LDS_BYTES;
    if (g.twowin) g.nwin = g.units;
    g.pair = (a.lean_pair == 2 && 2 * G <= 64) || (a.lean_pair == 1 && G <= 16) || (a.lean_pair == 3 && G <= 24);
    g.lds = lean_lds_bytes(G, g.nwin);
    {
        const int want = a.est_waves > 0 ? a.est_waves : 12;
        g.hw_est = g.hw < want ? want : g.hw;
        if (g.hw_est > MAX_THREADS / 64) g.hw_est = MAX_THREADS / 64;
    }
    const int room = (int)((size_t)g.nwin * UF * lean::WS / tfft::WSLOTS);
    g.nwe = g.hw_est < room ? g.hw_est : room;
    g.lds_est = g.lds + LEAN_EST_LDS_BYTES;
    g.ok = valid;
    g.est_ok = valid && a.frame_size >= tfft::N0 + tfft::NFFT && g.nwe >= 1 && (G + g.nwe - 1) / g.nwe <= tfft::MAX_FPW && G <= 32 &&
               g.lds_est <= (size_t)MAX_LDS_BYTES;
    return g;
}

bool lean_est_ok(const FusedArgs &a, int G, unsigned long long layout)
{
    return lean_geometry(a, G, layout).est_ok;
}

int launch_rx_lean(const FusedArgs &a0, int G, unsigned long long layout, int *status, hipStream_t s)
{
    FusedArgs a = a0;
    const LeanGeometry g = lean_geometry(a, G, layout);
    if (!g.ok || !lean_shape_ok(a, G) || (a.nframes % G != 0 && !a.sym_pad)) return (int)hipErrorInvalidValue;
    if (a.est_tw && (!g.est_ok || !a.est_cs || a.index)) return (int)hipErrorInvalidValue;
    a.G = G;
    a.mixed = 2;
    a.share_simd0 = g.share_simd0;
    a.lean_twowin = g.twowin;
    a.lean_pair = g.pair;
    hipLaunchKernelGGL(a.data_rule ? rx_lean_kernel<true> : rx_lean_kernel<false>, dim3((a.nframes + G - 1) / G), dim3(64 * (a.est_tw ? g.hw_est : g.hw)), a.est_tw ? g.lds_est : g.lds, s, a,
                       layout, g.nwin, status);
    return (int)hipGetLastError();
}

int prepare_rx_lean(void)
{
    const hipError_t e = hipFuncSetAttribute(reinterpret_cast<const void *>(rx_lean_kernel<false>), hipFuncAttributeMaxDynamicSharedMemorySize,
                                             MAX_LDS_BYTES);
    if (e != hipSuccess) return (int)e;
    return (int)hipFuncSetAttribute(reinterpret_cast<const void *>(rx_lean_kernel<true>), hipFuncAttributeMaxDynamicSharedMemorySize,
                                    MAX_LDS_BYTES);
}

}

#ifdef QPSK_PIPE_PROFILE
extern "C" __attribute__((visibility("default"))) int qpsk_prof_timeline(unsigned long long *dst, int n)
{
    if (n > 1024 * 48) n = 1024 * 48;
    return (int)hipMemcpyFromSymbol(dst, HIP_SYMBOL(qpsk::prof::g_timeline), sizeof(unsigned long long) * (size_t)n);
}
#endif
```

### qpsk_amd/lib.py

```python
import ctypes as C
import os
import subprocess

import numpy as np

HERE = os.path.dirname(os.path.abspath(__file__))
TAU = 2.0 * 3.14159265358979323846
TIMING_HIST, TIMING_FIXED, TIMING_FFT = 0, 1, 2
NTAPS = 127


class QpskError(RuntimeError):
    pass


class Params(C.Structure):
    _fields_ = [("fs", C.c_double), ("rs", C.c_double), ("frame_size", C.c_int), ("rrc_alpha", C.c_float),
                ("loop_bw", C.c_float), ("min_freq", C.c_float), ("max_freq", C.c_float),
                ("timing_mode", C.c_int), ("fixed_index", C.c_int)]


def lib_path():
    return os.environ.get("QPSK_HIP_LIB") or os.path.join(HERE, "libqpsk_hip.so")


def build(verbose=False):
    cmd = ["make", "-C", os.path.join(HERE, "csrc")]
    if not verbose:
        cmd.insert(1, "-s")
    subprocess.check_call(cmd)
    return lib_path()


_LIB = None

API_SYMBOLS = [
    "qpsk_last_error", "qpsk_version", "qpsk_device_count", "qpsk_params_default", "qpsk_ctx_create",
    "qpsk_ctx_destroy", "qpsk_ctx_sync", "qpsk_ctx_set_stream", "qpsk_ctx_set_tuning", "qpsk_ctx_cycles", "qpsk_ctx_nsym",
    "qpsk_ctx_last_kernel",
    "qpsk_ctx_get_taps", "qpsk_ctx_get_gains", "qpsk_ctx_set_taps", "qpsk_ctx_set_loop", "qpsk_rx_batch", "qpsk_rx_batch_pitched",
    "qpsk_rx_batch_bw", "qpsk_rrc_fir_batch", "qpsk_rrc_fir_batch_fast", "qpsk_timing_hist_batch", "qpsk_timing_scan_batch", "qpsk_timing_fft_batch", "qpsk_timing_fft_bin_batch", "qpsk_costas_batch", "qpsk_fft_batch",
    "qpsk_streams_reset", "qpsk_streams_set_loop_state", "qpsk_streams_get_loop_state", "qpsk_streams_rx_cplx",
    "qpsk_streams_rx_pcm", "qpsk_streams_rx_pcm_host", "qpsk_dev_alloc", "qpsk_dev_free", "qpsk_dev_upload", "qpsk_dev_download",
    "qpsk_selftest_sincos_hash", "qpsk_crc16_batch", "qpsk_interleave_batch", "qpsk_scramble_batch",
    "qpsk_tx_reset", "qpsk_tx_symbols", "qpsk_test_inject_status", "qpsk_test_hist_state", "qpsk_ctx_check",
    "qpsk_multi_create", "qpsk_multi_destroy", "qpsk_multi_shards", "qpsk_multi_load", "qpsk_multi_shard", "qpsk_multi_use_device_input",
    "qpsk_multi_rx_begin", "qpsk_multi_rx_end", "qpsk_multi_set_direct_output", "qpsk_host_alloc", "qpsk_host_free",
    "qpsk_multi_set_packed", "qpsk_pack_symbols", "qpsk_unpack_symbols_host",
    "qpsk_rx_batch_ext", "qpsk_rx_batch_bw_ext", "qpsk_multi_set_acquisition", "qpsk_carrier_est_batch",
    "qpsk_rx_batch_data", "qpsk_sync_batch", "qpsk_multi_set_data", "qpsk_deframer_reset", "qpsk_deframer_push",
    "qpsk_deframer_reset_coded", "qpsk_deframer_push_coded",
    "qpsk_soft_batch", "qpsk_conv_encode_batch", "qpsk_viterbi_batch",
    "qpsk_punct_ntx", "qpsk_conv_encode_punct_batch", "qpsk_viterbi_punct_batch", "qpsk_deframer_reset_coded_punct",
    "qpsk_test_viterbi_launches", "qpsk_test_deframer_advance", "qpsk_test_fir_runs",
    "qpsk_frame_len", "qpsk_frame_batch",
    "qpsk_ilv_stride", "qpsk_conv_encode_ilv_batch", "qpsk_viterbi_ilv_batch", "qpsk_frame_batch_ilv", "qpsk_deframer_reset_coded_ilv",
    "qpsk_rs_generator", "qpsk_rs_encode_batch", "qpsk_rs_decode_batch",
    "qpsk_viterbi_stream_reset", "qpsk_viterbi_stream_emits", "qpsk_viterbi_stream_push", "qpsk_viterbi_stream_flush",
    "qpsk_conv_encode_stream_batch", "qpsk_test_viterbi_stream_advance",
]
PUNCTURE = {"1/2": (1, 0x1, 0x1), "2/3": (2, 0x1, 0x3), "3/4": (3, 0x5, 0x3), "5/6": (5, 0x15, 0x0B), "7/8": (7, 0x51, 0x2F)}


def _pattern(puncture):
    if isinstance(puncture, str):
        if puncture not in PUNCTURE:
            raise ValueError("puncture must be one of %s or a (period, keep0, keep1) tuple" % sorted(PUNCTURE))
        puncture = PUNCTURE[puncture]
    period, keep0, keep1 = puncture
    return int(period), int(keep0), int(keep1)
DROPIN_SYMBOLS = [
    "qpsk_dropin_configure", "qpsk_dropin_set_device", "qpsk_dropin_shutdown", "rrc_fir", "rrc_make",
    "create_control_loop", "phase_detector", "update_gains", "advance_loop", "phase_wrap", "frequency_limit",
    "set_loop_bandwidth", "set_damping_factor", "set_alpha", "set_beta", "set_frequency", "set_phase",
    "set_max_freq", "set_min_freq", "get_loop_bandwidth", "get_damping_factor", "get_alpha", "get_beta",
    "get_frequency", "get_phase", "get_max_freq", "get_min_freq", "fft", "fftn", "ifft", "ifftn", "qpsk_demod",
    "rx_frame", "qpsk_dropin_costas_frame", "qpsk_dropin_symbols", "qpsk_dropin_offset_freq",
    "qpsk_dropin_timing_index",
]


def load():
    global _LIB
    if _LIB is not None:
        return _LIB
    p = lib_path()
    if not os.path.exists(p):
        raise QpskError("%s is missing: run `python -c 'import __graft_entry__ as g; g.build()'` "
                        "(there is no CPU fallback)" % p)
    try:
        import torch
    except ImportError:
        pass
    L = C.CDLL(p)
    vp, i32, f32 = C.c_void_p, C.c_int, C.c_float
    L.qpsk_last_error.restype = C.c_char_p
    L.qpsk_version.restype = C.c_char_p
    L.qpsk_params_default.argtypes = [C.POINTER(Params)]
    L.qpsk_ctx_create.argtypes = [C.POINTER(vp), i32, C.POINTER(Params), vp]
    L.qpsk_ctx_destroy.argtypes = [vp]
    L.qpsk_ctx_destroy.restype = None
    L.qpsk_ctx_sync.argtypes = [vp]
    L.qpsk_ctx_set_stream.argtypes = [vp, vp]
    L.qpsk_ctx_set_tuning.argtypes = [vp, C.c_char_p, i32]
    L.qpsk_ctx_cycles.argtypes = [vp]
    L.qpsk_ctx_nsym.argtypes = [vp]
    L.qpsk_ctx_last_kernel.argtypes = [vp]
    L.qpsk_ctx_last_kernel.restype = C.c_char_p
    L.qpsk_ctx_get_taps.argtypes = [vp, C.POINTER(f32)]
    L.qpsk_ctx_get_gains.argtypes = [vp, C.POINTER(f32), C.POINTER(f32)]
    L.qpsk_ctx_set_taps.argtypes = [vp, C.POINTER(f32)]
    L.qpsk_ctx_set_loop.argtypes = [vp, f32, f32, f32, f32]
    L.qpsk_rx_batch.argtypes = [vp, vp, i32, vp, vp, vp, vp, vp, vp]
    L.qpsk_rx_batch_pitched.argtypes = [vp, vp, C.c_longlong, i32, vp, vp, vp, vp, vp, vp]
    L.qpsk_rx_batch_bw.argtypes = [vp, vp, i32, C.POINTER(f32), i32, vp, vp, vp, vp]
    L.qpsk_rx_batch_ext.argtypes = [vp, vp, C.c_longlong, i32, vp, vp, vp, vp, vp, vp, vp, vp]
    L.qpsk_rx_batch_bw_ext.argtypes = [vp, vp, i32, C.POINTER(f32), i32, vp, vp, vp, vp, vp, vp]
    L.qpsk_multi_set_acquisition.argtypes = [vp, vp, vp]
    L.qpsk_carrier_est_batch.argtypes = [vp, vp, C.c_longlong, i32, i32, i32, vp, vp, vp, vp]
    L.qpsk_rx_batch_data.argtypes = [vp, vp, C.c_longlong, i32, vp, vp, vp, vp, vp, vp, vp, vp]
    L.qpsk_sync_batch.argtypes = [vp, vp, i32, i32, vp, i32, i32, i32, i32, vp, vp, vp, vp]
    L.qpsk_multi_set_data.argtypes = [vp, i32]
    L.qpsk_deframer_reset.argtypes = [vp, i32, vp, i32, i32, i32, i32]
    L.qpsk_deframer_push.argtypes = [vp, vp, vp, i32, vp, vp, vp, vp, vp, vp]
    L.qpsk_deframer_reset_coded.argtypes = [vp, i32, vp, i32, i32, i32, i32, i32, f32]
    L.qpsk_deframer_push_coded.argtypes = [vp, vp, i32, vp, vp, vp, vp, vp, vp, vp, vp]
    L.qpsk_soft_batch.argtypes = [vp, vp, C.c_longlong, i32, i32, i32, i32, f32, vp, vp, vp, i32, i32, vp, vp, vp]
    L.qpsk_conv_encode_batch.argtypes = [vp, vp, i32, i32, i32, vp]
    L.qpsk_viterbi_batch.argtypes = [vp, vp, C.c_longlong, i32, i32, vp, i32, vp, vp]
    u32 = C.c_uint32
    L.qpsk_punct_ntx.argtypes = [i32, i32, u32, u32]
    L.qpsk_conv_encode_punct_batch.argtypes = [vp, vp, i32, i32, i32, i32, u32, u32, vp]
    L.qpsk_viterbi_punct_batch.argtypes = [vp, vp, C.c_longlong, i32, i32, i32, u32, u32, vp, i32, vp, vp]
    L.qpsk_deframer_reset_coded_punct.argtypes = [vp, i32, vp, i32, i32, i32, i32, i32, f32, i32, u32, u32]
    L.qpsk_frame_len.argtypes = [i32, i32, i32, i32, u32, u32]
    L.qpsk_frame_batch.argtypes = [vp, vp, C.c_longlong, i32, i32, i32, vp, i32, i32, i32, u32, u32, i32, i32, i32, vp, vp]
    L.qpsk_ilv_stride.argtypes = [i32, i32]
    L.qpsk_conv_encode_ilv_batch.argtypes = [vp, vp, i32, i32, i32, i32, u32, u32, i32, vp]
    L.qpsk_viterbi_ilv_batch.argtypes = [vp, vp, C.c_longlong, i32, i32, i32, u32, u32, i32, vp, i32, vp, vp]
    L.qpsk_frame_batch_ilv.argtypes = [vp, vp, C.c_longlong, i32, i32, i32, vp, i32, i32, i32, u32, u32, i32, i32, i32, i32, vp, vp]
    L.qpsk_deframer_reset_coded_ilv.argtypes = [vp, i32, vp, i32, i32, i32, i32, i32, f32, i32, u32, u32, i32]
    L.qpsk_rs_generator.argtypes = [i32, vp]
    L.qpsk_rs_encode_batch.argtypes = [vp, vp, C.c_longlong, i32, i32, i32, vp, C.c_longlong]
    L.qpsk_rs_decode_batch.argtypes = [vp, vp, C.c_longlong, i32, i32, i32, vp, vp, C.c_longlong, vp]
    L.qpsk_rrc_fir_batch.argtypes = [vp, vp, vp, vp, i32, i32]
    L.qpsk_rrc_fir_batch_fast.argtypes = [vp, vp, vp, vp, i32, i32]
    L.qpsk_timing_hist_batch.argtypes = [vp, vp, i32, vp, vp]
    L.qpsk_timing_fft_batch.argtypes = [vp, vp, i32, vp, vp, vp]
    L.qpsk_timing_fft_bin_batch.argtypes = [vp, vp, i32, vp, vp, vp]
    L.qpsk_timing_scan_batch.argtypes = [vp, vp, i32, vp, vp]
    L.qpsk_costas_batch.argtypes = [vp, vp, i32, i32, vp, vp, vp]
    L.qpsk_fft_batch.argtypes = [vp, vp, vp, i32, i32, i32]
    L.qpsk_streams_reset.argtypes = [vp, i32, C.c_double]
    L.qpsk_streams_set_loop_state.argtypes = [vp, C.POINTER(f32)]
    L.qpsk_streams_get_loop_state.argtypes = [vp, C.POINTER(f32)]
    L.qpsk_streams_rx_cplx.argtypes = [vp, vp, vp, vp, vp, vp, vp]
    L.qpsk_streams_rx_pcm.argtypes = [vp, vp, vp, vp, vp, vp, vp]
    L.qpsk_streams_rx_pcm_host.argtypes = [vp, vp, vp, vp, vp, vp]
    L.qpsk_selftest_sincos_hash.argtypes = [vp, C.c_uint32, C.c_uint32, C.POINTER(C.c_ulonglong)]
    L.qpsk_test_inject_status.argtypes = [vp, i32]
    L.qpsk_ctx_check.argtypes = [vp]
    L.qpsk_test_hist_state.argtypes = [vp, C.POINTER(i32)]
    L.qpsk_test_viterbi_launches.argtypes = [vp, C.POINTER(i32)]
    L.qpsk_test_deframer_advance.argtypes = [vp, C.c_longlong]
    L.qpsk_viterbi_stream_reset.argtypes = [vp, i32, i32, i32, i32, u32, u32]
    L.qpsk_viterbi_stream_emits.argtypes = [vp, i32]
    L.qpsk_viterbi_stream_push.argtypes = [vp, vp, C.c_longlong, i32, vp, C.c_longlong, vp, C.POINTER(i32)]
    L.qpsk_viterbi_stream_flush.argtypes = [vp, i32, vp, C.c_longlong, vp, C.POINTER(i32)]
    L.qpsk_conv_encode_stream_batch.argtypes = [vp, vp, i32, i32, i32, u32, u32, vp, vp, vp]
    L.qpsk_test_viterbi_stream_advance.argtypes = [vp, C.c_longlong]
    L.qpsk_test_fir_runs.argtypes = [vp, i32, i32, C.POINTER(i32)]
    L.qpsk_multi_create.argtypes = [C.POINTER(vp), C.POINTER(i32), i32, C.POINTER(Params)]
    L.qpsk_multi_destroy.argtypes = [vp]
    L.qpsk_multi_destroy.restype = None
    L.qpsk_multi_shards.argtypes = [vp]
    L.qpsk_multi_load.argtypes = [vp, C.c_longlong, vp]
    L.qpsk_multi_shard.argtypes = [vp, i32, C.POINTER(i32), C.POINTER(C.c_longlong), C.POINTER(C.c_longlong), C.POINTER(vp), C.POINTER(vp)]
    L.qpsk_multi_use_device_input.argtypes = [vp, i32, vp]
    L.qpsk_multi_set_direct_output.argtypes = [vp, i32, vp, vp, vp]
    L.qpsk_multi_set_packed.argtypes = [vp, i32]
    L.qpsk_pack_symbols.argtypes = [vp, vp, C.c_longlong, i32, vp]
    L.qpsk_unpack_symbols_host.argtypes = [vp, C.c_longlong, i32, vp]
    L.qpsk_host_alloc.argtypes = [C.POINTER(vp), C.c_size_t]
    L.qpsk_host_free.argtypes = [vp]
    L.qpsk_multi_rx_begin.argtypes = [vp, i32]
    L.qpsk_multi_rx_end.argtypes = [vp, i32, vp, vp, vp]
    L.qpsk_crc16_batch.argtypes = [vp, vp, i32, i32, vp]
    L.qpsk_interleave_batch.argtypes = [vp, vp, i32, i32, i32]
    L.qpsk_scramble_batch.argtypes = [vp, vp, i32, i32]
    L.qpsk_tx_reset.argtypes = [vp, i32, C.c_double]
    L.qpsk_tx_symbols.argtypes = [vp, vp, i32, vp, vp]
    _LIB = L
    return L


def version():
    return load().qpsk_version().decode()


FRAME_UNCODED, FRAME_CODED = 0, 1


def _coding(coded, puncture):
    if not coded:
        return (FRAME_UNCODED, 1, 1, 1)
    return (FRAME_CODED,) + _pattern("1/2" if puncture is None else puncture)


def frame_len(nsync, nbytes, coded=True, puncture=None):
    L = load()
    rc = L.qpsk_frame_len(int(nsync), int(nbytes), *_coding(coded, puncture))
    if rc < 0:
        raise QpskError("libqpsk_hip error %d: %s" % (rc, L.qpsk_last_error().decode()))
    return rc


def ilv_stride(nbits, want):
    L = load()
    rc = L.qpsk_ilv_stride(int(nbits), int(want))
    if rc < 0:
        raise QpskError("libqpsk_hip error %d: %s" % (rc, L.qpsk_last_error().decode()))
    return rc


def rs_generator(nroots):
    L = load()
    g = np.zeros(max(int(nroots), 0) + 1, np.uint8)
    rc = L.qpsk_rs_generator(int(nroots), g.ctypes.data_as(C.c_void_p))
    if rc < 0:
        raise QpskError("libqpsk_hip error %d: %s" % (rc, L.qpsk_last_error().decode()))
    return g


def _interleaved(interleave):
    return interleave is not None and int(interleave) != 1


def _ptr(t):
    return None if t is None else C.c_void_p(t.data_ptr())


class Modem:

    def __init__(self, fs=9600.0, rs=2400.0, frame_size=512, rrc_alpha=0.35, loop_bw=np.float32(TAU / 100.0),
                 min_freq=-1.0, max_freq=1.0, timing_mode=TIMING_HIST, fixed_index=0, device=None, stream="torch"):
        import torch
        self.torch = torch
        self.L = load()
        if not torch.cuda.is_available():
            raise QpskError("no GPU visible to torch; libqpsk_hip has no CPU path")
        self.device = torch.cuda.current_device() if device is None else int(device)
        self.dev = torch.device("cuda", self.device)
        self.params = Params(fs, rs, frame_size, rrc_alpha, loop_bw, min_freq, max_freq, timing_mode, fixed_index)
        if stream == "torch":
            s = C.c_void_p(torch.cuda.current_stream(self.dev).cuda_stream)
        elif stream is None:
            s = None
        else:
            s = C.c_void_p(int(stream))
        h = C.c_void_p()
        self._check(self.L.qpsk_ctx_create(C.byref(h), self.device, C.byref(self.params), s))
        self.h = h
        self.cycles = self.L.qpsk_ctx_cycles(h)
        self.nsym = self.L.qpsk_ctx_nsym(h)
        self.frame_size = frame_size
        self.nstreams = 0
        self._vs_streams = 0

    def _check(self, rc):
        if rc != 0:
            raise QpskError("libqpsk_hip error %d: %s" % (rc, self.L.qpsk_last_error().decode()))

    def close(self):
        if getattr(self, "h", None):
            self.L.qpsk_ctx_destroy(self.h)
            self.h = None

    def __del__(self):
        try:
            self.close()
        except Exception:
            pass

    def sync(self, data=None, sync=None, lag_min=0, lag_max=0, nout=0):
        if data is None:
            self._check(self.L.qpsk_ctx_sync(self.h))
            return None
        return self._sync_search(data, sync, lag_min, lag_max, nout)

    def last_kernel(self):
        return self.L.qpsk_ctx_last_kernel(self.h).decode()

    def tune(self, **kw):
        for k, v in kw.items():
            self._check(self.L.qpsk_ctx_set_tuning(self.h, ("QPSK_" + k.upper()).encode(), -1 if v is None else int(v)))

    def viterbi_launches(self):
        n = C.c_int(-1)
        self._check(self.L.qpsk_test_viterbi_launches(self.h, C.byref(n)))
        return n.value

    def deframer_advance(self, delta):
        self._check(self.L.qpsk_test_deframer_advance(self.h, int(delta)))

    def fir_runs(self, nframes, length):
        out = (C.c_int * 3)()
        self._check(self.L.qpsk_test_fir_runs(self.h, int(nframes), int(length), out))
        return tuple(out)

    def set_stream(self, stream):
        s = None if stream is None else C.c_void_p(getattr(stream, "cuda_stream", stream))
        self._check(self.L.qpsk_ctx_set_stream(self.h, s))

    @property
    def taps(self):
        t = (C.c_float * NTAPS)()
        self._check(self.L.qpsk_ctx_get_taps(self.h, t))
        return np.array(t, np.float32)

    @property
    def gains(self):
        a, b = C.c_float(), C.c_float()
        self._check(self.L.qpsk_ctx_get_gains(self.h, C.byref(a), C.byref(b)))
        return np.float32(a.value), np.float32(b.value)

    def set_taps(self, taps):
        t = (C.c_float * NTAPS)(*[float(x) for x in taps])
        self._check(self.L.qpsk_ctx_set_taps(self.h, t))

    def set_loop(self, alpha, beta, min_freq, max_freq):
        self._check(self.L.qpsk_ctx_set_loop(self.h, alpha, beta, min_freq, max_freq))

    def _dev(self, a, dtype):
        t = self.torch
        if isinstance(a, np.ndarray):
            a = t.from_numpy(np.ascontiguousarray(a))
        a = a.to(self.dev)
        assert a.dtype == dtype, (a.dtype, dtype)
        return a.contiguous()

    def empty(self, shape, dtype):
        return self.torch.empty(shape, dtype=dtype, device=self.dev)

    def rx_batch(self, frames, want_costas=False, out=None):
        t = self.torch
        x = self._dev(frames, t.float32)
        F = x.shape[0]
        assert x.shape[1] == self.frame_size and x.shape[2] == 2
        o = out or dict(sym=self.empty((F, self.nsym), t.uint8), freq=self.empty((F,), t.float32),
                        phase=self.empty((F,), t.float32), index=self.empty((F,), t.int32),
                        hz=self.empty((F,), t.float32),
                        costas=self.empty((F, self.nsym, 2), t.float32) if want_costas else None)
        self._check(self.L.qpsk_rx_batch(self.h, _ptr(x), F, _ptr(o["sym"]), _ptr(o["freq"]), _ptr(o["phase"]),
                                         _ptr(o.get("costas")), _ptr(o.get("index")), _ptr(o.get("hz"))))
        return o

    def rx_batch_raw(self, x, F, sym, freq, phase, pitch=0, index=None):
        if pitch:
            rc = self.L.qpsk_rx_batch_pitched(self.h, _ptr(x), pitch, F, _ptr(sym), _ptr(freq), _ptr(phase), None, _ptr(index), None)
        else:
            rc = self.L.qpsk_rx_batch(self.h, _ptr(x), F, _ptr(sym), _ptr(freq), _ptr(phase), None, _ptr(index), None)
        if rc:
            self._check(rc)

    def rx_batch_bw(self, frames, loop_bws):
        t = self.torch
        x = self._dev(frames, t.float32)
        F, B = x.shape[0], len(loop_bws)
        bws = (C.c_float * B)(*[float(b) for b in loop_bws])
        o = dict(sym=self.empty((F, B, self.nsym), t.uint8), freq=self.empty((F, B), t.float32),
                 phase=self.empty((F, B), t.float32), index=self.empty((F,), t.int32))
        self._check(self.L.qpsk_rx_batch_bw(self.h, _ptr(x), F, bws, B, _ptr(o["sym"]), _ptr(o["freq"]),
                                            _ptr(o["phase"]), _ptr(o["index"])))
        return o

    def rx_batch_ext(self, frames, index=None, seed=None, want_costas=False, pitch=0):
        t = self.torch
        x = self._dev(frames, t.float32)
        F = x.shape[0]
        assert x.shape[1] == (pitch or self.frame_size) and x.shape[2] == 2
        ix = None if index is None else self._dev(index, t.int32)
        sd = None if seed is None else self._dev(seed, t.float32)
        assert ix is None or tuple(ix.shape) == (F,)
        assert sd is None or tuple(sd.shape) == (F, 2)
        o = dict(sym=self.empty((F, self.nsym), t.uint8), freq=self.empty((F,), t.float32),
                 phase=self.empty((F,), t.float32), index=self.empty((F,), t.int32), hz=self.empty((F,), t.float32),
                 costas=self.empty((F, self.nsym, 2), t.float32) if want_costas else None)
        self._check(self.L.qpsk_rx_batch_ext(self.h, _ptr(x), int(pitch), F, _ptr(ix), _ptr(sd), _ptr(o["sym"]), _ptr(o["freq"]),
                                             _ptr(o["phase"]), _ptr(o["costas"]), _ptr(o["index"]), _ptr(o["hz"])))
        o["_keep"] = (x, ix, sd)
        return o

    def rx_batch_data(self, frames, index=None, seed=None, want_sym=False, pitch=0):
        t = self.torch
        x = self._dev(frames, t.float32)
        F = x.shape[0]
        assert x.shape[1] == (pitch or self.frame_size) and x.shape[2] == 2
        ix = None if index is None else self._dev(index, t.int32)
        sd = None if seed is None else self._dev(seed, t.float32)
        assert ix is None or tuple(ix.shape) == (F,)
        assert sd is None or tuple(sd.shape) == (F, 2)
        o = dict(data=self.empty((F, self.nsym), t.uint8), sym=self.empty((F, self.nsym), t.uint8) if want_sym else None,
                 freq=self.empty((F,), t.float32), phase=self.empty((F,), t.float32), index=self.empty((F,), t.int32),
                 hz=self.empty((F,), t.float32))
        self._check(self.L.qpsk_rx_batch_data(self.h, _ptr(x), int(pitch), F, _ptr(ix), _ptr(sd), _ptr(o["data"]), _ptr(o["sym"]),
                                              _ptr(o["freq"]), _ptr(o["phase"]), _ptr(o["index"]), _ptr(o["hz"])))
        o["_keep"] = (x, ix, sd)
        return o

    def _sync_search(self, data, sync, lag_min, lag_max, nout):
        t = self.torch
        d = self._dev(data, t.uint8)
        F, N = d.shape
        sw = np.ascontiguousarray(np.asarray(sync, dtype=np.uint8))
        o = dict(out=self.empty((F, nout), t.uint8), lag=self.empty((F,), t.int32), rot=self.empty((F,), t.int32),
                 score=self.empty((F,), t.int32))
        self._check(self.L.qpsk_sync_batch(self.h, _ptr(d), F, N, sw.ctypes.data_as(C.c_void_p), len(sw), int(lag_min), int(lag_max),
                                           int(nout), _ptr(o["out"]), _ptr(o["lag"]), _ptr(o["rot"]), _ptr(o["score"])))
        o["_keep"] = (d,)
        return o

    def rx_batch_bw_ext(self, frames, loop_bws, index=None, seed=None):
        t = self.torch
        x = self._dev(frames, t.float32)
        F, B = x.shape[0], len(loop_bws)
        bws = (C.c_float * B)(*[float(b) for b in loop_bws])
        ix = None if index is None else self._dev(index, t.int32)
        sd = None if seed is None else self._dev(seed, t.float32)
        assert ix is None or tuple(ix.shape) == (F,)
        assert sd is None or tuple(sd.shape) == (F, B, 2)
        o = dict(sym=self.empty((F, B, self.nsym), t.uint8), freq=self.empty((F, B), t.float32),
                 phase=self.empty((F, B), t.float32), index=self.empty((F,), t.int32))
        self._check(self.L.qpsk_rx_batch_bw_ext(self.h, _ptr(x), F, bws, B, _ptr(ix), _ptr(sd), _ptr(o["sym"]), _ptr(o["freq"]),
                                                _ptr(o["phase"]), _ptr(o["index"])))
        o["_keep"] = (x, ix, sd)
        return o

    def carrier_est(self, frames, n=1024, start=128, pitch=0, want_line=False):
        t = self.torch
        x = self._dev(frames, t.float32)
        F = x.shape[0]
        assert x.shape[1] == (pitch or self.frame_size) and x.shape[2] == 2
        o = dict(seed=self.empty((F, 2), t.float32), freq=self.empty((F,), t.float32), bin=self.empty((F,), t.int32))
        if want_line:
            o["line"] = self.empty((F, 2), t.float64)
        self._check(self.L.qpsk_carrier_est_batch(self.h, _ptr(x), int(pitch), F, int(start), int(n), _ptr(o["seed"]), _ptr(o["freq"]),
                                                  _ptr(o["bin"]), _ptr(o.get("line"))))
        o["_keep"] = (x,)
        return o

    SOFT_MODES = {"unit": 0, "llr": 1}

    def soft(self, costas, skip=0, mode="unit", scale=64.0, gain=None, lag=None, rot=None, first=0, nout=None, want_sums=False):
        return self._soft(costas, skip, mode, scale, gain, lag, rot, first, nout, want_sums, True)

    def quality(self, costas, skip=0):
        return self._soft(costas, skip, "unit", 64.0, None, None, None, 0, 0, False, False)

    def _soft(self, costas, skip, mode, scale, gain, lag, rot, first, nout, want_sums, want_soft):
        t = self.torch
        if isinstance(costas, dict):
            costas = costas["costas"]
        z = self._dev(costas, t.float32)
        if z.dim() != 3 or z.shape[2] != 2:
            raise ValueError("soft() input must be (rows, nsym, 2) float32")
        R, N = z.shape[0], z.shape[1]
        g = None if gain is None else self._dev(gain, t.float32)
        lg = None if lag is None else self._dev(lag, t.int32)
        rt = None if rot is None else self._dev(rot, t.int32)
        for a in (g, lg, rt):
            assert a is None or tuple(a.shape) == (R,)
        if nout is None:
            nout = N - first
        o = dict(quality=self.empty((R, 4), t.float32))
        if want_soft:
            o["soft"] = self.empty((R, nout, 2), t.int8)
        if want_sums:
            o["sums"] = self.empty((R, 4), t.float64)
        self._check(self.L.qpsk_soft_batch(self.h, _ptr(z), 0, R, N, int(skip), self.SOFT_MODES[mode], float(scale), _ptr(g), _ptr(lg),
                                           _ptr(rt), int(first), int(nout), _ptr(o.get("soft")), _ptr(o["quality"]), _ptr(o.get("sums"))))
        o["_keep"] = (z, g, lg, rt)
        return o

    def punct_ntx(self, nsteps, puncture):
        rc = self.L.qpsk_punct_ntx(int(nsteps), *_pattern(puncture))
        self._check(min(rc, 0))
        return rc

    def conv_encode(self, bits_packed, nbits, tail=True, puncture=None, interleave=None):
        t = self.torch
        b = self._dev(bits_packed, t.uint8)
        if b.dim() != 2 or b.shape[1] != (int(nbits) + 7) // 8:
            raise ValueError("conv_encode() input must be (rows, ceil(nbits / 8)) uint8")
        nsteps = int(nbits) + (6 if tail else 0)
        if _interleaved(interleave):
            pat = _pattern("1/2" if puncture is None else puncture)
            out = self.empty((b.shape[0], self.punct_ntx(nsteps, pat)), t.uint8)
            self._check(self.L.qpsk_conv_encode_ilv_batch(self.h, _ptr(b), b.shape[0], int(nbits), 1 if tail else 0, *pat, int(interleave),
                                                          _ptr(out)))
            return out
        if puncture is not None:
            pat = _pattern(puncture)
            out = self.empty((b.shape[0], self.punct_ntx(nsteps, pat)), t.uint8)
            self._check(self.L.qpsk_conv_encode_punct_batch(self.h, _ptr(b), b.shape[0], int(nbits), 1 if tail else 0, *pat, _ptr(out)))
            return out
        out = self.empty((b.shape[0], nsteps), t.uint8)
        self._check(self.L.qpsk_conv_encode_batch(self.h, _ptr(b), b.shape[0], int(nbits), 1 if tail else 0, _ptr(out)))
        return out

    def viterbi(self, soft, flip=None, open_start=False, open_end=False, pitch=0, nsteps=None, puncture=None, interleave=None):
        t = self.torch
        if isinstance(soft, dict):
            soft = soft["soft"]
        q = self._dev(soft, t.int8)
        ilv = _interleaved(interleave)
        if ilv and puncture is None:
            puncture = "1/2"
            if nsteps is None and q.dim() == 3 and not pitch:
                nsteps = q.shape[1]
        if puncture is not None:
            pat = _pattern(puncture)
            if nsteps is None:
                raise ValueError("viterbi(puncture=...) needs nsteps: the transmitted length does not determine it")
            n = int(nsteps)
            ntx = self.punct_ntx(n, pat)
            if q.dim() != 3 or q.shape[2] != 2 or q.shape[1] != (pitch or ntx):
                raise ValueError("viterbi(puncture=...) input must be (rows, ntx = %d or pitch, 2) int8" % ntx)
            f = None if flip is None else self._dev(flip, t.uint8)
            if f is not None and tuple(f.shape) != (ntx,):
                raise ValueError("viterbi(puncture=...) flip must be (ntx = %d,) uint8" % ntx)
            R = q.shape[0]
            o = dict(bits=self.empty((R, (n + 7) // 8), t.uint8), info=self.empty((R, 4), t.int32))
            flags = (1 if open_start else 0) | (2 if open_end else 0)
            if ilv:
                self._check(self.L.qpsk_viterbi_ilv_batch(self.h, _ptr(q), int(pitch), R, n, *pat, int(interleave), _ptr(f), flags,
                                                          _ptr(o["bits"]), _ptr(o["info"])))
            else:
                self._check(self.L.qpsk_viterbi_punct_batch(self.h, _ptr(q), int(pitch), R, n, *pat, _ptr(f), flags, _ptr(o["bits"]),
                                                            _ptr(o["info"])))
            o["_keep"] = (q, f)
            return o
        if q.dim() != 3 or q.shape[2] != 2 or (pitch and q.shape[1] != pitch):
            raise ValueError("viterbi() input must be (rows, nsteps or pitch, 2) int8")
        R = q.shape[0]
        n = int(nsteps) if nsteps is not None else q.shape[1]
        f = None if flip is None else self._dev(flip, t.uint8)
        assert f is None or tuple(f.shape) == (n,)
        o = dict(bits=self.empty((R, (n + 7) // 8), t.uint8), info=self.empty((R, 4), t.int32))
        self._check(self.L.qpsk_viterbi_batch(self.h, _ptr(q), int(pitch), R, n, _ptr(f), (1 if open_start else 0) | (2 if open_end else 0),
                                              _ptr(o["bits"]), _ptr(o["info"])))
        o["_keep"] = (q, f)
        return o

    def viterbi_stream_reset(self, nstreams, depth=128, window=256, puncture=None):
        pat = _pattern("1/2" if puncture is None else puncture)
        self._check(self.L.qpsk_viterbi_stream_reset(self.h, int(nstreams), int(depth), int(window), *pat))
        self._vs_streams = int(nstreams)

    def viterbi_stream_emits(self, ntx):
        rc = self.L.qpsk_viterbi_stream_emits(self.h, int(ntx))
        self._check(min(rc, 0))
        return rc

    def _viterbi_stream_out(self, nbits):
        t = self.torch
        return dict(bits=self.empty((self._vs_streams, (nbits + 7) // 8), t.uint8), info=self.empty((self._vs_streams, 4), t.int32))

    def viterbi_stream(self, soft, pitch=0, ntx=None):
        t = self.torch
        if isinstance(soft, dict):
            soft = soft["soft"]
        if not self._vs_streams:
            raise QpskError("viterbi_stream() before viterbi_stream_reset()")
        q = self._dev(soft, t.int8)
        if q.dim() != 3 or q.shape[0] != self._vs_streams or q.shape[2] != 2 or (pitch and q.shape[1] != pitch):
            raise ValueError("viterbi_stream() input must be (streams = %d, ntx or pitch, 2) int8" % self._vs_streams)
        ntx = q.shape[1] if ntx is None else int(ntx)
        o = self._viterbi_stream_out(self.viterbi_stream_emits(ntx))
        n = C.c_int32(-1)
        self._check(self.L.qpsk_viterbi_stream_push(self.h, _ptr(q), int(pitch), ntx, _ptr(o["bits"]), o["bits"].shape[1], _ptr(o["info"]),
                                                    C.byref(n)))
        o["nbits"] = n.value
        o["_keep"] = (q,)
        return o

    def viterbi_stream_flush(self, terminated=False):
        if not self._vs_streams:
            raise QpskError("viterbi_stream_flush() before viterbi_stream_reset()")
        o = self._viterbi_stream_out(8192)
        n = C.c_int32(-1)
        self._check(self.L.qpsk_viterbi_stream_flush(self.h, 1 if terminated else 0, _ptr(o["bits"]), o["bits"].shape[1], _ptr(o["info"]),
                                                     C.byref(n)))
        o["nbits"] = n.value
        o["bits"] = o["bits"][:, :(n.value + 7) // 8]
        return o

    def viterbi_stream_advance(self, delta):
        self._check(self.L.qpsk_test_viterbi_stream_advance(self.h, int(delta)))

    def conv_encode_stream(self, bits_packed, nbits, state=None, puncture=None):
        t = self.torch
        b = self._dev(bits_packed, t.uint8)
        if b.dim() != 2 or b.shape[1] != (int(nbits) + 7) // 8:
            raise ValueError("conv_encode_stream() input must be (rows, ceil(nbits / 8)) uint8")
        pat = _pattern("1/2" if puncture is None else puncture)
        K = bin(pat[1]).count("1") + bin(pat[2]).count("1")
        st = None if state is None else self._dev(state, t.uint8)
        if st is not None and tuple(st.shape) != (b.shape[0],):
            raise ValueError("conv_encode_stream() state must be (rows,) uint8")
        out = self.empty((b.shape[0], max(int(nbits) // pat[0] * K // 2, 1)), t.uint8)
        nxt = self.empty((b.shape[0],), t.uint8)
        self._check(self.L.qpsk_conv_encode_stream_batch(self.h, _ptr(b), b.shape[0], int(nbits), *pat, _ptr(st), _ptr(nxt), _ptr(out)))
        return out, nxt

    def rrc_fir(self, x, memory=None, fast=False):
        t = self.torch
        x = self._dev(x, t.float32)
        y = t.empty_like(x)
        fn = self.L.qpsk_rrc_fir_batch_fast if fast else self.L.qpsk_rrc_fir_batch
        self._check(fn(self.h, _ptr(memory), _ptr(x), _ptr(y), x.shape[0], x.shape[1]))
        return y

    def timing_hist(self, filtered, want_hist=False):
        t = self.torch
        y = self._dev(filtered, t.float32)
        idx = self.empty((y.shape[0],), t.int32)
        hist = self.empty((y.shape[0], 8), t.int32) if want_hist else None
        self._check(self.L.qpsk_timing_hist_batch(self.h, _ptr(y), y.shape[0], _ptr(idx), _ptr(hist)))
        return (idx, hist) if want_hist else idx

    def timing_scan(self, frames):
        t = self.torch
        x = self._dev(frames, t.float32)
        idx = self.empty((x.shape[0],), t.int32)
        hist = self.empty((x.shape[0], 8), t.int32)
        self._check(self.L.qpsk_timing_scan_batch(self.h, _ptr(x), x.shape[0], _ptr(idx), _ptr(hist)))
        return idx, hist

    def timing_fft(self, frames, want_internals=False):
        t = self.torch
        x = self._dev(frames, t.float32)
        F = x.shape[0]
        idx = self.empty((F,), t.int32)
        y = self.empty((F, 512, 2), t.float32) if want_internals else None
        X = self.empty((F, 512), t.complex128) if want_internals else None
        self._check(self.L.qpsk_timing_fft_batch(self.h, _ptr(x), F, _ptr(idx), _ptr(y), _ptr(X)))
        return (idx, y, X) if want_internals else idx

    def timing_fft_bin(self, frames):
        t = self.torch
        x = self._dev(frames, t.float32)
        F = x.shape[0]
        idx = self.empty((F,), t.int32)
        y = self.empty((F, 512, 2), t.float32)
        xk = self.empty((F,), t.complex128)
        self._check(self.L.qpsk_timing_fft_bin_batch(self.h, _ptr(x), F, _ptr(idx), _ptr(y), _ptr(xk)))
        return idx, y, xk

    def costas(self, d, state=None, want_costas=True):
        t = self.torch
        d = self._dev(d, t.float32)
        F, N = d.shape[0], d.shape[1]
        sym = self.empty((F, N), t.uint8)
        z = self.empty((F, N, 2), t.float32) if want_costas else None
        self._check(self.L.qpsk_costas_batch(self.h, _ptr(d), F, N, _ptr(state), _ptr(sym), _ptr(z)))
        return sym, z

    def fft(self, x, inverse=False):
        t = self.torch
        if isinstance(x, np.ndarray):
            x = t.from_numpy(np.ascontiguousarray(x, dtype=np.complex128))
        x = x.to(self.dev).contiguous()
        out = t.empty_like(x)
        self._check(self.L.qpsk_fft_batch(self.h, _ptr(x), _ptr(out), x.shape[0], x.shape[1], int(inverse)))
        return out

    def streams_reset(self, nstreams, mixer_hz=1500.0):
        self._check(self.L.qpsk_streams_reset(self.h, nstreams, mixer_hz))
        self.nstreams = nstreams

    def _stream_out(self, want_costas):
        t, n = self.torch, self.nstreams
        return dict(sym=self.empty((n, self.nsym), t.uint8), freq=self.empty((n,), t.float32),
                    phase=self.empty((n,), t.float32), index=self.empty((n,), t.int32),
                    costas=self.empty((n, self.nsym, 2), t.float32) if want_costas else None)

    def streams_rx_cplx(self, blocks, want_costas=True):
        x = self._dev(blocks, self.torch.float32)
        o = self._stream_out(want_costas)
        self._check(self.L.qpsk_streams_rx_cplx(self.h, _ptr(x), _ptr(o["sym"]), _ptr(o["freq"]), _ptr(o["phase"]),
                                                _ptr(o["costas"]), _ptr(o["index"])))
        return o

    def streams_rx_pcm(self, pcm, want_costas=True):
        x = self._dev(pcm, self.torch.int16)
        o = self._stream_out(want_costas)
        self._check(self.L.qpsk_streams_rx_pcm(self.h, _ptr(x), _ptr(o["sym"]), _ptr(o["freq"]), _ptr(o["phase"]),
                                               _ptr(o["costas"]), _ptr(o["index"])))
        return o

    def deframer_reset(self, nstreams, sync, nbytes, min_score, max_packets=8):
        sw = np.ascontiguousarray(np.asarray(sync, dtype=np.uint8))
        self._check(self.L.qpsk_deframer_reset(self.h, int(nstreams), sw.ctypes.data_as(C.c_void_p), len(sw), int(min_score), int(nbytes),
                                               int(max_packets)))
        self.df_shape = (int(nstreams), int(nbytes), int(max_packets))

    def deframe(self, costas=None, data=None):
        t = self.torch
        if isinstance(costas, dict):
            costas = costas["costas"]
        if (costas is None) == (data is None):
            raise ValueError("deframe() takes exactly one of costas, data")
        x = self._dev(costas, t.float32) if costas is not None else self._dev(data, t.uint8)
        S, nb, M = self.df_shape
        if x.shape[0] != S or (costas is not None and (x.dim() != 3 or x.shape[2] != 2)) or (data is not None and x.dim() != 2):
            raise ValueError("deframe() input must be (%d, nsym, 2) float32 or (%d, nsym) uint8" % (S, S))
        o = dict(count=self.empty((S,), t.int32), bytes=self.torch.zeros((S, M, nb + 2), dtype=t.uint8, device=self.dev),
                 pos=t.zeros((S, M), dtype=t.int64, device=self.dev), rot=t.zeros((S, M), dtype=t.int32, device=self.dev),
                 score=t.zeros((S, M), dtype=t.int32, device=self.dev), crc_ok=t.zeros((S, M), dtype=t.uint8, device=self.dev))
        self._check(self.L.qpsk_deframer_push(self.h, _ptr(x) if costas is not None else None, _ptr(x) if data is not None else None,
                                              x.shape[1], _ptr(o["count"]), _ptr(o["bytes"]), _ptr(o["pos"]), _ptr(o["rot"]),
                                              _ptr(o["score"]), _ptr(o["crc_ok"])))
        o["_keep"] = (x,)
        return o

    def deframer_reset_coded(self, nstreams, sync, nbytes, min_score, max_packets=8, mode="unit", scale=64.0, puncture=None, interleave=None):
        sw = np.ascontiguousarray(np.asarray(sync, dtype=np.uint8))
        if _interleaved(interleave):
            self._check(self.L.qpsk_deframer_reset_coded_ilv(self.h, int(nstreams), sw.ctypes.data_as(C.c_void_p), len(sw), int(min_score),
                                                             int(nbytes), int(max_packets), self.SOFT_MODES[mode], float(scale),
                                                             *_pattern("1/2" if puncture is None else puncture), int(interleave)))
            self.df_shape = (int(nstreams), int(nbytes), int(max_packets))
            return
        if puncture is not None:
            self._check(self.L.qpsk_deframer_reset_coded_punct(self.h, int(nstreams), sw.ctypes.data_as(C.c_void_p), len(sw), int(min_score),
                                                               int(nbytes), int(max_packets), self.SOFT_MODES[mode], float(scale),
                                                               *_pattern(puncture)))
            self.df_shape = (int(nstreams), int(nbytes), int(max_packets))
            return
        self._check(self.L.qpsk_deframer_reset_coded(self.h, int(nstreams), sw.ctypes.data_as(C.c_void_p), len(sw), int(min_score), int(nbytes),
                                                     int(max_packets), self.SOFT_MODES[mode], float(scale)))
        self.df_shape = (int(nstreams), int(nbytes), int(max_packets))

    def deframe_coded(self, costas, gain=None):
        t = self.torch
        if isinstance(costas, dict):
            costas = costas["costas"]
        x = self._dev(costas, t.float32)
        S, nb, M = self.df_shape
        if x.dim() != 3 or x.shape[0] != S or x.shape[2] != 2:
            raise ValueError("deframe_coded() input must be (%d, nsym, 2) float32" % S)
        g = None if gain is None else self._dev(gain, t.float32)
        if g is not None and tuple(g.shape) != (S,):
            raise ValueError("deframe_coded() gain must be (%d,) float32" % S)
        z = lambda shape, dt: t.zeros(shape, dtype=dt, device=self.dev)
        o = dict(count=self.empty((S,), t.int32), bytes=z((S, M, nb + 2), t.uint8), pos=z((S, M), t.int64), rot=z((S, M), t.int32),
                 score=z((S, M), t.int32), crc_ok=z((S, M), t.uint8), info=z((S, M, 4), t.int32))
        self._check(self.L.qpsk_deframer_push_coded(self.h, _ptr(x), x.shape[1], _ptr(g), _ptr(o["count"]), _ptr(o["bytes"]), _ptr(o["pos"]),
                                                    _ptr(o["rot"]), _ptr(o["score"]), _ptr(o["crc_ok"]), _ptr(o["info"])))
        o["_keep"] = (x, g)
        return o

    def frame(self, payloads, sync, coded=True, puncture=None, per_row=1, lead=0, gap=0, row_len=None, interleave=None):
        t = self.torch
        p = self._dev(payloads, t.uint8)
        per_row, lead, gap = int(per_row), int(lead), int(gap)
        if p.dim() == 3 and p.shape[1] == per_row:
            p = p.reshape(-1, p.shape[2])
        if p.dim() != 2 or per_row < 1 or p.shape[0] < 1 or p.shape[0] % per_row:
            raise ValueError("frame() payloads must be (nrows * per_row, nbytes) or (nrows, per_row, nbytes) uint8")
        npk, nbytes = p.shape
        sw = np.ascontiguousarray(np.asarray(sync, dtype=np.uint8))
        code = _coding(coded, puncture)
        if row_len is None:
            P = self.L.qpsk_frame_len(len(sw), nbytes, *code)
            self._check(min(P, 0))
            row_len = lead + per_row * P + (per_row - 1) * gap
        o = dict(dibits=self.empty((npk // per_row, int(row_len)), t.uint8), crc=self.empty((npk,), t.int16))
        if _interleaved(interleave):
            self._check(self.L.qpsk_frame_batch_ilv(self.h, _ptr(p), 0, npk // per_row, per_row, nbytes, sw.ctypes.data_as(C.c_void_p), len(sw),
                                                    *code, int(interleave), lead, gap, int(row_len), _ptr(o["dibits"]), _ptr(o["crc"])))
        else:
            self._check(self.L.qpsk_frame_batch(self.h, _ptr(p), 0, npk // per_row, per_row, nbytes, sw.ctypes.data_as(C.c_void_p), len(sw),
                                                *code, lead, gap, int(row_len), _ptr(o["dibits"]), _ptr(o["crc"])))
        o["_keep"] = (p,)
        return o

    def rs_encode(self, data, nroots, pitch=0):
        t = self.torch
        d = self._dev(data, t.uint8)
        if d.dim() != 2:
            raise ValueError("rs_encode() data must be (rows, k) uint8")
        R, k = d.shape
        n = k + int(nroots)
        buf = self.empty((R, int(pitch) or n), t.uint8)
        self._check(self.L.qpsk_rs_encode_batch(self.h, _ptr(d), 0, R, k, int(nroots), _ptr(buf), int(pitch)))
        self._rs_keep = (d,)
        return buf[:, :n]

    def rs_decode(self, words, nroots, erasures=None, pitch=0, n=None, inplace=False):
        t = self.torch
        w = self._dev(words, t.uint8)
        if w.dim() != 2 or (pitch and w.shape[1] != pitch):
            raise ValueError("rs_decode() words must be (rows, n or pitch) uint8")
        R = w.shape[0]
        n = int(n) if n is not None else w.shape[1]
        e = None if erasures is None else self._dev(erasures, t.uint8)
        if e is not None and tuple(e.shape) != (R, n):
            raise ValueError("rs_decode() erasures must be (%d, %d) uint8" % (R, n))
        if inplace and (not isinstance(words, t.Tensor) or w.data_ptr() != words.data_ptr()):
            raise ValueError("rs_decode(inplace=True) needs a contiguous uint8 tensor on the modem's device")
        out = w if inplace else self.empty((R, n), t.uint8)
        info = self.empty((R, 4), t.int32)
        self._check(self.L.qpsk_rs_decode_batch(self.h, _ptr(w), int(pitch), R, n, int(nroots), _ptr(e), _ptr(out), int(pitch) if inplace else 0,
                                                _ptr(info)))
        self._rs_keep = (w, e)
        return out[:, :n], info

    def streams_loop_state(self):
        a = (C.c_float * (2 * self.nstreams))()
        self._check(self.L.qpsk_streams_get_loop_state(self.h, a))
        return np.array(a, np.float32).reshape(-1, 2)

    def tx_reset(self, nstreams, tx_hz=1550.0):
        self._check(self.L.qpsk_tx_reset(self.h, nstreams, tx_hz))
        self.ntx = nstreams

    def tx_symbols(self, symbols, want_pcm=True, want_baseband=False):
        t = self.torch
        d = self._dev(symbols, t.uint8)
        if d.dim() != 2 or d.shape[0] != getattr(self, "ntx", 0):
            raise ValueError("symbols must be (ntx, nsym) after tx_reset(ntx)")
        n = d.shape[1] * self.cycles
        pcm = self.empty((d.shape[0], n), t.int16) if want_pcm else None
        bb = self.empty((d.shape[0], n, 2), t.float32) if want_baseband else None
        self._check(self.L.qpsk_tx_symbols(self.h, _ptr(d), d.shape[1], _ptr(pcm), _ptr(bb)))
        return dict(pcm=pcm, baseband=bb)

    def crc16(self, packets):
        t = self.torch
        d = self._dev(packets, t.uint8)
        out = self.empty((d.shape[0],), t.int16)
        self._check(self.L.qpsk_crc16_batch(self.h, _ptr(d), d.shape[0], d.shape[1], _ptr(out)))
        return out.cpu().numpy().view(np.uint16)

    def interleave(self, packets, direction):
        d = self._dev(packets, self.torch.uint8).clone()
        self._check(self.L.qpsk_interleave_batch(self.h, _ptr(d), d.shape[0], d.shape[1], int(direction)))
        return d

    def scramble(self, symbols):
        d = self._dev(symbols, self.torch.uint8).clone()
        self._check(self.L.qpsk_scramble_batch(self.h, _ptr(d), d.shape[0], d.shape[1]))
        return d

    def sincos_hash(self, first, count):
        h = C.c_ulonglong()
        self._check(self.L.qpsk_selftest_sincos_hash(self.h, first, count, C.byref(h)))
        return h.value


class MultiJob:

    def __init__(self, devices, **params):
        kw = dict(fs=9600.0, rs=2400.0, frame_size=512, rrc_alpha=0.35, loop_bw=np.float32(TAU / 100.0), min_freq=-1.0, max_freq=1.0,
                  timing_mode=TIMING_HIST, fixed_index=0)
        kw.update(params)
        self.L = load()
        self.params = Params(kw["fs"], kw["rs"], kw["frame_size"], kw["rrc_alpha"], kw["loop_bw"], kw["min_freq"], kw["max_freq"],
                             kw["timing_mode"], kw["fixed_index"])
        devs = (C.c_int32 * len(devices))(*[int(d) for d in devices])
        h = C.c_void_p()
        self._check(self.L.qpsk_multi_create(C.byref(h), devs, len(devices), C.byref(self.params)))
        self.h = h
        self.frame_size = kw["frame_size"]
        self.total = 0
        self.nsym = None

    def _check(self, rc):
        if rc != 0:
            raise QpskError("libqpsk_hip error %d: %s" % (rc, self.L.qpsk_last_error().decode()))

    def load(self, frames_host=None, total=None):
        if frames_host is not None:
            x = np.ascontiguousarray(frames_host, np.float32)
            total = x.shape[0]
            self._check(self.L.qpsk_multi_load(self.h, total, x.ctypes.data_as(C.c_void_p)))
        else:
            self._check(self.L.qpsk_multi_load(self.h, int(total), None))
        self.total = int(total)
        ctx = C.c_void_p()
        self._check(self.L.qpsk_multi_shard(self.h, 0, None, None, None, C.byref(ctx), None))
        self.nsym = self.L.qpsk_ctx_nsym(ctx)

    def shard(self, r):
        dev, first, count, ctx, d_in = C.c_int32(), C.c_longlong(), C.c_longlong(), C.c_void_p(), C.c_void_p()
        self._check(self.L.qpsk_multi_shard(self.h, r, C.byref(dev), C.byref(first), C.byref(count), C.byref(ctx), C.byref(d_in)))
        return dict(device=dev.value, first=first.value, count=count.value, ctx=ctx, d_in=d_in.value)

    def tune_shard(self, r, **kw):
        ctx = self.shard(r)["ctx"]
        for k, v in kw.items():
            self._check(self.L.qpsk_ctx_set_tuning(ctx, ("QPSK_" + k.upper()).encode(), -1 if v is None else int(v)))

    def inject_status(self, r, code):
        self._check(self.L.qpsk_test_inject_status(self.shard(r)["ctx"], int(code)))

    def hist_state(self, r):
        st = (C.c_int32 * 5)()
        self._check(self.L.qpsk_test_hist_state(self.shard(r)["ctx"], st))
        return list(st)

    def last_kernel(self, r):
        return self.L.qpsk_ctx_last_kernel(self.shard(r)["ctx"]).decode()

    def use_device_input(self, r, tensor):
        self._check(self.L.qpsk_multi_use_device_input(self.h, r, C.c_void_p(tensor.data_ptr())))

    def begin(self, slot):
        self._check(self.L.qpsk_multi_rx_begin(self.h, slot))

    def end(self, slot, sym=None, freq=None, phase=None):
        p = lambda a: None if a is None else a.ctypes.data_as(C.c_void_p)
        self._check(self.L.qpsk_multi_rx_end(self.h, slot, p(sym), p(freq), p(phase)))

    def set_acquisition(self, index=None, seed=None):
        ix = None if index is None else np.ascontiguousarray(index, np.int32)
        sd = None if seed is None else np.ascontiguousarray(seed, np.float32)
        assert ix is None or ix.shape == (self.total,)
        assert sd is None or sd.shape == (self.total, 2)
        p = lambda a: None if a is None else a.ctypes.data_as(C.c_void_p)
        self._check(self.L.qpsk_multi_set_acquisition(self.h, p(ix), p(sd)))

    def set_packed(self, on):
        self._check(self.L.qpsk_multi_set_packed(self.h, int(bool(on))))
        self.packed = bool(on)

    def set_data(self, on):
        self._check(self.L.qpsk_multi_set_data(self.h, int(bool(on))))
        self.data = bool(on)

    def unpack(self, packed):
        out = np.empty((packed.shape[0], self.nsym), np.uint8)
        self._check(self.L.qpsk_unpack_symbols_host(packed.ctypes.data_as(C.c_void_p), packed.shape[0], self.nsym, out.ctypes.data_as(C.c_void_p)))
        return out

    def pinned_outputs(self):
        out = []
        cols = (self.nsym + 3) // 4 if getattr(self, "packed", False) else self.nsym
        for shape, dt in (((self.total, cols), np.uint8), ((self.total,), np.float32), ((self.total,), np.float32)):
            nbytes = int(np.prod(shape)) * np.dtype(dt).itemsize
            p = C.c_void_p()
            self._check(self.L.qpsk_host_alloc(C.byref(p), nbytes))
            self._pinned = getattr(self, "_pinned", []) + [p]
            buf = (C.c_uint8 * nbytes).from_address(p.value)
            out.append(np.frombuffer(buf, dtype=dt).reshape(shape))
        return tuple(out)

    def set_direct(self, slot, sym=None, freq=None, phase=None):
        p = lambda a: None if a is None else C.c_void_p(a.ctypes.data)
        self._check(self.L.qpsk_multi_set_direct_output(self.h, slot, p(sym), p(freq), p(phase)))

    def outputs(self):
        cols = (self.nsym + 3) // 4 if getattr(self, "packed", False) else self.nsym
        return (np.empty((self.total, cols), np.uint8), np.empty(self.total, np.float32), np.empty(self.total, np.float32))

    def close(self):
        if getattr(self, "h", None):
            self.L.qpsk_multi_destroy(self.h)
            self.h = None
            for p in getattr(self, "_pinned", []):
                self.L.qpsk_host_free(p)
            self._pinned = []

    def __del__(self):
        try:
            self.close()
        except Exception:
            pass
```

Baseline: 432,100.

## Cache per-wave lean FIR lane geometry and DMA tables in a device image

Adds a small LRU cache of device-resident 'lean images' holding each wave's precomputed LDS address geometry and DMA offset/region tables, built once by a separate kernel and keyed on layout/shape. When the fixed-index path is used, worker waves load four quads of geometry from global memory and skip the pre-barrier setup and LDS DMA table construction, feeding the table straight from global memory into new asm loop variants. It also adds a kernarg prefetch touch at kernel entry. The cost is an extra build launch on a cache miss, additional global loads per wave, and more variant code paths.

Measured after the change: 435,300 (median of 3 runs). No clear change (+0.7%).

```diff
diff --git a/include/qpsk_hip.h b/include/qpsk_hip.h
--- a/include/qpsk_hip.h
+++ b/include/qpsk_hip.h
@@ -222,6 +222,7 @@
 int qpsk_test_hist_state(qpsk_ctx *ctx, int32_t *out);
 int qpsk_test_fir_runs(qpsk_ctx *ctx, int nframes, int length, int32_t out[3]);
 int qpsk_test_viterbi_launches(qpsk_ctx *ctx, int *out);
+int qpsk_test_lean_image_builds(qpsk_ctx *ctx, int *out);
 int qpsk_test_deframer_advance(qpsk_ctx *ctx, long long delta);
 int qpsk_test_viterbi_stream_advance(qpsk_ctx *ctx, long long delta);
 
diff --git a/qpsk_amd/csrc/api_ctx.cpp b/qpsk_amd/csrc/api_ctx.cpp
--- a/qpsk_amd/csrc/api_ctx.cpp
+++ b/qpsk_amd/csrc/api_ctx.cpp
@@ -235,6 +235,7 @@
     for (auto &kv : c->twiddles) hipFree(kv.second);
     hipFree(c->d_fast);
     c->hist.release();
+    c->lean_images.release();
     c->streams.release();
     c->tx.release();
     c->df.release();
diff --git a/qpsk_amd/csrc/api_ctx.h b/qpsk_amd/csrc/api_ctx.h
--- a/qpsk_amd/csrc/api_ctx.h
+++ b/qpsk_amd/csrc/api_ctx.h
@@ -79,6 +79,19 @@
     int32_t *d_hint = nullptr;
     int32_t *h_hist_stats = nullptr, *d_hist_stats = nullptr;
     bool hint_valid = false;
+    void release();
+};
+
+struct QPSK_UNIT_LOCAL LeanImages {
+    static const int SLOTS = 4;
+    struct Slot {
+        DevBuf buf;
+        LeanImageKey key{};
+        bool valid = false;
+        unsigned long long used = 0;
+    } slot[SLOTS];
+    unsigned long long clock = 0;
+    unsigned long long builds = 0;
     void release();
 };
 
@@ -174,6 +187,7 @@
     bool fast_valid = false;
     qpsk::StatusWord status;
     qpsk::HistGuess hist;
+    qpsk::LeanImages lean_images;
     qpsk::Streams streams;
     qpsk::Transmitters tx;
     qpsk::Deframer df;
diff --git a/qpsk_amd/csrc/api_rx.cpp b/qpsk_amd/csrc/api_rx.cpp
--- a/qpsk_amd/csrc/api_rx.cpp
+++ b/qpsk_amd/csrc/api_rx.cpp
@@ -32,11 +32,24 @@
     return QPSK_OK;
 }
 
+int qpsk_test_lean_image_builds(qpsk_ctx *c, int *out)
+{
+    if (!c || !out) return fail(QPSK_ERR_ARG, "qpsk_test_lean_image_builds: null argument");
+    *out = (int)c->lean_images.builds;
+    return QPSK_OK;
+}
+
 void HistGuess::release()
 {
     if (d_hint) hipFree(d_hint);
     if (h_hist_stats) hipHostFree(h_hist_stats);
     *this = HistGuess();
+}
+
+void LeanImages::release()
+{
+    for (Slot &sl : slot) sl.buf.release();
+    *this = LeanImages();
 }
 
 static bool fir_takes_stream(const qpsk_ctx *c) { return c->taps_symmetric && tuned(c->tune.fir_generic, 0) == 0; }
@@ -297,8 +310,36 @@
     return QPSK_OK;
 }
 
-static int rx_launch(qpsk_ctx *c, const FusedArgs &a, const RxRoute &rt)
-{
+static int lean_image_for(qpsk_ctx *c, const FusedArgs &a, const RxRoute &rt, const uint4 **image)
+{
+    *image = nullptr;
+    LeanImageKey key;
+    if (!lean_image_key(a, rt.G, rt.layout, &key)) return QPSK_OK;
+    LeanImages &im = c->lean_images;
+    LeanImages::Slot *hit = nullptr, *oldest = &im.slot[0];
+    for (LeanImages::Slot &sl : im.slot) {
+        if (sl.valid && sl.key == key) hit = &sl;
+        if (!sl.valid || (oldest->valid && sl.used < oldest->used)) oldest = &sl;
+    }
+    if (!hit) {
+        oldest->valid = false;
+        if (int rc = ensure(c, oldest->buf, lean_image_bytes(key))) return rc;
+        KERNEL_TRY(launch_lean_image_build(key, oldest->buf.p, c->stream));
+        oldest->key = key;
+        oldest->valid = true;
+        im.builds++;
+        hit = oldest;
+    }
+    hit->used = ++im.clock;
+    *image = static_cast<const uint4 *>(hit->buf.p);
+    return QPSK_OK;
+}
+
+static int rx_launch(qpsk_ctx *c, const FusedArgs &a0, const RxRoute &rt)
+{
+    FusedArgs a = a0;
+    if (rt.kind == K_LEAN)
+        if (int rc = lean_image_for(c, a, rt, &a.lean_image)) return rc;
     if (a.est_tw && !(rt.kind == K_FUSED_PIPE && rt.nf == pipe_max_nf()) && rt.kind != K_LEAN)
         return fail(QPSK_ERR_STATE, "internal: in-launch FFT timing estimate planned for a kernel that has none");
     if (a.data_rule && rt.kind != K_LEAN)
diff --git a/qpsk_amd/csrc/kernels.h b/qpsk_amd/csrc/kernels.h
--- a/qpsk_amd/csrc/kernels.h
+++ b/qpsk_amd/csrc/kernels.h
@@ -59,6 +59,7 @@
     float2 *carrier_tab;
     int carrier_frame;
     int data_rule;
+    const uint4 *lean_image;
 };
 
 size_t fused_lds_bytes(int G, int S, int cycles, int nbw);
@@ -105,6 +106,18 @@
 int launch_rx_lean(const FusedArgs &a, int G, unsigned long long layout, int *status, hipStream_t s);
 QPSK_UNIT_LOCAL int prepare_rx_lean(void);
 bool lean_est_ok(const FusedArgs &a, int G, unsigned long long layout);
+struct LeanImageKey {
+    unsigned long long layout;
+    int G, nwin, twowin, lean_dma, fixed_index, nsym, pair, data_rule, hw;
+    bool operator==(const LeanImageKey &o) const
+    {
+        return layout == o.layout && G == o.G && nwin == o.nwin && twowin == o.twowin && lean_dma == o.lean_dma && fixed_index == o.fixed_index &&
+               nsym == o.nsym && pair == o.pair && data_rule == o.data_rule && hw == o.hw;
+    }
+};
+bool lean_image_key(const FusedArgs &a, int G, unsigned long long layout, LeanImageKey *key);
+size_t lean_image_bytes(const LeanImageKey &key);
+int launch_lean_image_build(const LeanImageKey &key, void *image, hipStream_t s);
 bool rx_hist_shape_ok(const FusedArgs &a);
 int launch_rx_hist(const FusedArgs &a, int32_t *index_true, const int32_t *hint, int32_t *mis_list, int32_t *mis_count, int *status, hipStream_t s);
 int launch_index_majority(const int32_t *index, int nframes, int32_t *hint, int32_t *mis_count, int32_t *h_stats, hipStream_t s);
diff --git a/qpsk_amd/csrc/rx_lean.hip b/qpsk_amd/csrc/rx_lean.hip
--- a/qpsk_amd/csrc/rx_lean.hip
+++ b/qpsk_amd/csrc/rx_lean.hip
@@ -2,12 +2,16 @@
 #include "qpsk_device.h"
 #include "fir_lean_asm.h"
 #include "fir_lean_data_asm.h"
+#include "fir_lean_img_asm.h"
 #ifdef QPSK_PIPE_PROFILE
 #include "fir_lean_prof_asm.h"
 #endif
 #include "rx_pipe2_geom.h"
 #include "fir_full8_asm.h"
 #include "timing_fft_wave.h"
+#ifndef QPSK_LEAN_TOUCH_KERNARGS
+#define QPSK_LEAN_TOUCH_KERNARGS 1
+#endif
 
 namespace qpsk {
 
@@ -30,8 +34,85 @@
     return fa + pipe2::UF <= a.nframes ? a.sym + (size_t)fa * a.nsym : a.sym_pad + (size_t)(pipe2::UF * u) * a.nsym;
 }
 
+namespace lean {
+constexpr int IMG_QUADS = 9, IMG_Q_REGIONS = 4, IMG_Q_OFFSETS = 5;
+static_assert(FIR_LEAN_IMG_QUAD == 64 * sizeof(uint4), "the image streams step from quad to quad of a lane by this many bytes");
+struct LeanLaneGeom {
+    LeanLaneAddr w;
+    unsigned rd;
+    unsigned symoff;
+};
+static_assert(sizeof(LeanLaneGeom) == 4 * sizeof(uint4), "quads 0..3 of the image");
+
+__device__ __forceinline__ int wave_units(unsigned long long layout, int wave, int twowin, int &u0, int &widx)
+{
+    u0 = widx = 0;
+    for (int v = 1; v < wave; v++) {
+        const int cv = (int)((layout >> (4 * v)) & 15);
+        u0 += cv;
+        widx += twowin ? cv : (cv != 0);
+    }
+    return wave < 16 ? (int)((layout >> (4 * wave)) & 15) : 0;
+}
+__device__ __forceinline__ void touch_kernargs()
+{
+#if QPSK_LEAN_TOUCH_KERNARGS
+    static_assert(sizeof(FusedArgs) + sizeof(unsigned long long) + sizeof(int) + sizeof(int *) >= 0x140 + 4, "the last line touched lies inside the explicit arguments");
+    unsigned t0, t1, t2, t3, t4, t5;
+    asm volatile("s_load_dword %0, %6, 0x0\n\t"
+                 "s_load_dword %1, %6, 0x40\n\t"
+                 "s_load_dword %2, %6, 0x80\n\t"
+                 "s_load_dword %3, %6, 0xc0\n\t"
+                 "s_load_dword %4, %6, 0x100\n\t"
+                 "s_load_dword %5, %6, 0x140\n\t"
+                 "s_waitcnt lgkmcnt(0)"
+                 : "=&s"(t0), "=&s"(t1), "=&s"(t2), "=&s"(t3), "=&s"(t4), "=&s"(t5)
+                 : "s"(__builtin_amdgcn_kernarg_segment_ptr())
+                 : "memory");
+#endif
+}
+__device__ __forceinline__ float2 *windows(unsigned char *smem) { return reinterpret_cast<float2 *>(smem + sizeof(Ctl)); }
+__device__ __forceinline__ unsigned char *ring_rows(unsigned char *smem, int nwin)
+{
+    return reinterpret_cast<unsigned char *>(windows(smem) + (size_t)nwin * pipe2::UF * WS);
+}
+__device__ __forceinline__ bool wave_uses_dma(int lean_dma, unsigned ixpack) { return lean_dma && (ixpack & 0x1111u) == 0; }
+}
+
 template <int NUW>
-__device__ __forceinline__ void lean_dma_table(unsigned *tab, float2 *mywin, unsigned ixpack, bool two_windows, int lane)
+__device__ __forceinline__ void lean_lane_geometry(lean::LeanLaneGeom &g, unsigned char *rows, float2 *mywin, int u0, unsigned ixpack,
+                                                   bool two_windows, int nsym, int lane)
+{
+    using namespace pipe2;
+    using GM = lean::GeomLean;
+    constexpr int WS = lean::WS;
+    float2 *dring = reinterpret_cast<float2 *>(rows);
+    float *zring = reinterpret_cast<float *>(rows + lean::Z_OFFSET_BYTES);
+    const int fl = lane / QL, q = lane % QL;
+    LeanLaneAddr &w = g.w;
+#pragma unroll
+    for (int ui = 0; ui < 2; ui++) {
+        const int u = u0 + (ui < NUW ? ui : 0);
+#pragma unroll
+        for (int ff = 0; ff < UF; ff++) {
+            const int ix = (int)((ixpack >> (4 * (2 * (ui < NUW ? ui : 0) + ff))) & 7u);
+            const int p0 = 2 * lane + HIST - ix;
+            const int wu = (two_windows && ui == 1) ? UF * WS : 0;
+            w.wr0[ui][ff] = lds_addr(mywin + wu + ff * WS + slot_of(p0)) - 8u * BLK;
+            w.wr1[ui][ff] = lds_addr(mywin + wu + ff * WS + slot_of(p0 + 1)) - 8u * BLK;
+        }
+        const int gf = UF * u + fl;
+        w.ring[ui] = lds_addr(dring + (size_t)gf * GM::DSTRIDE + R * q);
+        w.z[ui] = lds_addr(zring + (size_t)gf * GM::ZSTRIDE + R * q);
+    }
+    w.wlim = lds_addr(mywin + WS + (WS - 2));
+    w.wpad = lds_addr(mywin + WS + PAD);
+    g.rd = lds_addr(mywin + fl * WS + (PAD + PADS) * q);
+    g.symoff = (unsigned)(fl * nsym + R * q);
+}
+
+template <int NUW, class PutOffset, class PutRegion>
+__device__ __forceinline__ void lean_dma_table(float2 *mywin, unsigned ixpack, bool two_windows, int lane, PutOffset offset, PutRegion region)
 {
     using namespace pipe2;
     constexpr int WS = lean::WS;
@@ -49,19 +130,54 @@
                 if (r >= PAD) r = PAD - 2;
                 int n = PAD * grp + r - HIST + ix;
                 if (n > CH - 2) n = CH - 2;
-                tab[(4 * k + j) * 64 + lane] = 8u * (unsigned)n;
+                offset(k, j, 8u * (unsigned)n);
             }
-            tab[(16 + k) * 64 + lane] = lds_addr(mywin + ((two_windows && ui == 1) ? UF * WS : 0) + ff * WS + S0);
-        }
-}
-
-template <int NUW, bool DATA>
+            region(k, lds_addr(mywin + ((two_windows && ui == 1) ? UF * WS : 0) + ff * WS + S0));
+        }
+}
+
+template <int NUW>
+__device__ __forceinline__ void lean_image_wave(uint4 *img, unsigned char *rows, float2 *mywin, int u0, unsigned ixpack, bool use_dma,
+                                                bool two_windows, int nsym, int lane)
+{
+    lean::LeanLaneGeom g;
+    lean_lane_geometry<NUW>(g, rows, mywin, u0, ixpack, two_windows, nsym, lane);
+    const unsigned *gw = reinterpret_cast<const unsigned *>(&g);
+    for (int qd = 0; qd < 4; qd++) img[(size_t)qd * 64 + lane] = make_uint4(gw[4 * qd], gw[4 * qd + 1], gw[4 * qd + 2], gw[4 * qd + 3]);
+    if (!use_dma) return;
+    unsigned *cell = reinterpret_cast<unsigned *>(img);
+    lean_dma_table<NUW>(mywin, ixpack, two_windows, lane,
+                        [&](int k, int j, unsigned v) { cell[((size_t)(lean::IMG_Q_OFFSETS + k) * 64 + lane) * 4 + j] = v; },
+                        [&](int k, unsigned v) { cell[((size_t)lean::IMG_Q_REGIONS * 64 + lane) * 4 + k] = v; });
+}
+
+__global__ void __launch_bounds__(64)
+lean_image_build_kernel(uint4 *image, unsigned long long layout, int nwin, int twowin, int lean_dma, int fixed_index, int nsym)
+{
+    extern __shared__ __attribute__((aligned(16))) unsigned char smem_raw[];
+    const int wave = blockIdx.x, lane = threadIdx.x;
+    int u0, widx;
+    const int mine = lean::wave_units(layout, wave, twowin, u0, widx);
+    if (wave == 0 || mine == 0) return;
+    float2 *mywin = lean::windows(smem_raw) + (size_t)widx * pipe2::UF * lean::WS;
+    unsigned char *rows = lean::ring_rows(smem_raw, nwin);
+    const unsigned ix = (unsigned)checked_index(fixed_index, nullptr);
+    const unsigned ixpack = ix * (mine == 2 ? 0x1111u : 0x11u);
+    const bool use_dma = lean::wave_uses_dma(lean_dma, ixpack);
+    uint4 *img = image + (size_t)wave * lean::IMG_QUADS * 64;
+    if (mine == 2)
+        lean_image_wave<2>(img, rows, mywin, u0, ixpack, use_dma, twowin && use_dma, nsym, lane);
+    else
+        lean_image_wave<1>(img, rows, mywin, u0, ixpack, use_dma, false, nsym, lane);
+}
+
+template <int NUW, bool DATA, bool IMAGED>
 __device__ __forceinline__ void fir_wave_lean(const FusedArgs &a, lean::Ctl *sm, unsigned char *rows, float2 *mywin,
-                                              int hwave, int u0, int f0, int lane, int nchunks, int *status, const int *est)
+                                              int hwave, int u0, int f0, int lane, int nchunks, int *status, const int *est,
+                                              const lean::LeanLaneGeom &geo)
 {
     using namespace pipe2;
     using GM = lean::GeomLean;
-    constexpr int WS = lean::WS;
     float2 *dring = reinterpret_cast<float2 *>(rows);
     float *zring = reinterpret_cast<float *>(rows + lean::Z_OFFSET_BYTES);
     const int N = a.nsym;
@@ -77,94 +193,66 @@
             const int ix = checked_index(__builtin_amdgcn_readfirstlane(est ? est[UF * (u0 + ui) + ff] : a.index ? a.index[min(fr, a.nframes - 1)] : a.fixed_index), status);
             ixpack |= (unsigned)ix << (4 * (2 * ui + ff));
         }
-    const bool use_dma = a.lean_dma && (ixpack & 0x1111u) == 0;
+    const bool use_dma = lean::wave_uses_dma(a.lean_dma, ixpack);
     const bool two_windows = NUW == 2 && a.lean_twowin && use_dma;
-    LeanLaneAddr w;
-#pragma unroll
-    for (int ui = 0; ui < 2; ui++) {
-        const int u = u0 + (ui < NUW ? ui : 0);
-#pragma unroll
-        for (int ff = 0; ff < UF; ff++) {
-            const int fr = f0 + UF * u + ff;
-            const int ix = (int)((ixpack >> (4 * (2 * (ui < NUW ? ui : 0) + ff))) & 7u);
-            const int p0 = 2 * lane + HIST - ix;
-            const int wu = (two_windows && ui == 1) ? UF * WS : 0;
-            w.wr0[ui][ff] = lds_addr(mywin + wu + ff * WS + slot_of(p0)) - 8u * BLK;
-            w.wr1[ui][ff] = lds_addr(mywin + wu + ff * WS + slot_of(p0 + 1)) - 8u * BLK;
-            if (lane == 0) {
+    lean::LeanLaneGeom g = geo;
+    if constexpr (!IMAGED) lean_lane_geometry<NUW>(g, rows, mywin, u0, ixpack, two_windows, N, lane);
+    const LeanLaneAddr &w = g.w;
+    if (lane == 0) {
+#pragma unroll
+        for (int ui = 0; ui < 2; ui++) {
+            const int u = u0 + (ui < NUW ? ui : 0);
+#pragma unroll
+            for (int ff = 0; ff < UF; ff++) {
+                const int fr = f0 + UF * u + ff;
                 const size_t fsrc = prof::frame_number(a, UF * u + ff, (size_t)min(fr, a.nframes - 1));
                 const unsigned long long src = prof::frame_source(a, f0, UF * u + ff, (unsigned long long)(a.x + fsrc * a.frame_pitch));
                 prm[4 * ui + 2 * ff] = (unsigned)src;
                 prm[4 * ui + 2 * ff + 1] = (unsigned)(src >> 32);
             }
-        }
-        const int g = UF * u + fl;
-        w.ring[ui] = lds_addr(dring + (size_t)g * GM::DSTRIDE + R * q);
-        w.z[ui] = lds_addr(zring + (size_t)g * GM::ZSTRIDE + R * q);
-        if (lane == 0) {
             const unsigned long long sb = (unsigned long long)lean_unit_rows(a, f0, u);
             prm[8 + 2 * ui] = (unsigned)sb;
             prm[8 + 2 * ui + 1] = (unsigned)(sb >> 32);
         }
-    }
-    w.wlim = lds_addr(mywin + WS + (WS - 2));
-    w.wpad = lds_addr(mywin + WS + PAD);
-    if (lane == 0) {
         prm[12] = (unsigned)nchunks;
         prm[13] = ixpack;
         prm[16] = (unsigned)(unsigned long long)a.taps;
         prm[17] = (unsigned)((unsigned long long)a.taps >> 32);
     }
     if (simd0 && !(a.dbg & 1024)) __builtin_amdgcn_s_setprio(3);
-    const unsigned rd = lds_addr(mywin + fl * WS + (PAD + PADS) * q);
+    const unsigned rd = g.rd, symoff = g.symoff;
     prof::timeline_stamp(a, lane, 32 + hwave);
+    unsigned *tab = reinterpret_cast<unsigned *>(mywin);
     int st;
-    if (prof::lean_measured_stream<NUW>(a, lds_addr(prm), rd, 16u * lane, (unsigned)(fl * N + R * q), lds_addr(sm), w, lane, hwave, nchunks, st)) {
-    } else if constexpr (DATA) {
-        unsigned *tab = reinterpret_cast<unsigned *>(mywin);
-        if (use_dma) lean_dma_table<NUW>(tab, mywin, ixpack, two_windows, lane);
+    if (prof::lean_measured_stream<NUW>(a, lds_addr(prm), rd, 16u * lane, symoff, lds_addr(sm), w, lane, hwave, nchunks, st)) {
+    } else if (IMAGED && use_dma) {
+        const uint4 *itab = a.lean_image + ((size_t)hwave * lean::IMG_QUADS + lean::IMG_Q_OFFSETS) * 64 + lane;
+#define QPSK_LEAN_STREAM(NAME) (DATA ? NAME##_data(lds_addr(prm), rd, 16u * lane, symoff, lds_addr(sm), itab, w) \
+                                     : NAME(lds_addr(prm), rd, 16u * lane, symoff, lds_addr(sm), itab, w))
         if constexpr (NUW == 2) {
-            if (use_dma && two_windows)
-                st = fir_lean_loop2_dma2w_data(lds_addr(prm), rd, 16u * lane, (unsigned)(fl * N + R * q), lds_addr(sm), lds_addr(tab + lane), w);
-            else if (use_dma)
-                st = fir_lean_loop2_dma_data(lds_addr(prm), rd, 16u * lane, (unsigned)(fl * N + R * q), lds_addr(sm), lds_addr(tab + lane), w);
-            else
-                st = fir_lean_loop2_data(lds_addr(prm), rd, 16u * lane, (unsigned)(fl * N + R * q), lds_addr(sm), w);
-        } else if (use_dma)
-            st = fir_lean_loop1_dma_data(lds_addr(prm), rd, 16u * lane, (unsigned)(fl * N + R * q), lds_addr(sm), lds_addr(tab + lane), w);
-        else
-            st = fir_lean_loop1_data(lds_addr(prm), rd, 16u * lane, (unsigned)(fl * N + R * q), lds_addr(sm), w);
+            if (two_windows) st = QPSK_LEAN_STREAM(fir_lean_loop2_dma2wi);
+            else st = QPSK_LEAN_STREAM(fir_lean_loop2_dmai);
+        } else
+            st = QPSK_LEAN_STREAM(fir_lean_loop1_dmai);
+#undef QPSK_LEAN_STREAM
     } else if (use_dma) {
-        unsigned *tab = reinterpret_cast<unsigned *>(mywin);
-#pragma unroll
-        for (int ui = 0; ui < NUW; ui++)
-#pragma unroll
-            for (int ff = 0; ff < UF; ff++) {
-                const int k = 2 * ui + ff;
-                const int ix = (int)((ixpack >> (4 * k)) & 15u);
-                const int S0 = slot_of(HIST - ix);
-                for (int j = 0; j < 4; j++) {
-                    const int sl = S0 + 2 * (64 * j + lane);
-                    const int grp = sl / (PAD + PADS);
-                    int r = sl % (PAD + PADS);
-                    if (r >= PAD) r = PAD - 2;
-                    int n = PAD * grp + r - HIST + ix;
-                    if (n > CH - 2) n = CH - 2;
-                    tab[(4 * k + j) * 64 + lane] = 8u * (unsigned)n;
-                }
-                tab[(16 + k) * 64 + lane] = lds_addr(mywin + ((two_windows && ui == 1) ? UF * WS : 0) + ff * WS + S0);
-            }
+        lean_dma_table<NUW>(mywin, ixpack, two_windows, lane, [&](int k, int j, unsigned v) { tab[(4 * k + j) * 64 + lane] = v; },
+                            [&](int k, unsigned v) { tab[(16 + k) * 64 + lane] = v; });
+#define QPSK_LEAN_STREAM(NAME) (DATA ? NAME##_data(lds_addr(prm), rd, 16u * lane, symoff, lds_addr(sm), lds_addr(tab + lane), w) \
+                                     : NAME(lds_addr(prm), rd, 16u * lane, symoff, lds_addr(sm), lds_addr(tab + lane), w))
         if constexpr (NUW == 2) {
-            if (two_windows)
-                st = fir_lean_loop2_dma2w(lds_addr(prm), rd, 16u * lane, (unsigned)(fl * N + R * q), lds_addr(sm), lds_addr(tab + lane), w);
-            else
-                st = fir_lean_loop2_dma(lds_addr(prm), rd, 16u * lane, (unsigned)(fl * N + R * q), lds_addr(sm), lds_addr(tab + lane), w);
+            if (two_windows) st = QPSK_LEAN_STREAM(fir_lean_loop2_dma2w);
+            else st = QPSK_LEAN_STREAM(fir_lean_loop2_dma);
         } else
-            st = fir_lean_loop1_dma(lds_addr(prm), rd, 16u * lane, (unsigned)(fl * N + R * q), lds_addr(sm), lds_addr(tab + lane), w);
-    } else if constexpr (NUW == 2)
-        st = fir_lean_loop2(lds_addr(prm), rd, 16u * lane, (unsigned)(fl * N + R * q), lds_addr(sm), w);
-    else
-        st = fir_lean_loop1(lds_addr(prm), rd, 16u * lane, (unsigned)(fl * N + R * q), lds_addr(sm), w);
+            st = QPSK_LEAN_STREAM(fir_lean_loop1_dma);
+#undef QPSK_LEAN_STREAM
+    } else {
+#define QPSK_LEAN_STREAM(NAME) (DATA ? NAME##_data(lds_addr(prm), rd, 16u * lane, symoff, lds_addr(sm), w) \
+                                     : NAME(lds_addr(prm), rd, 16u * lane, symoff, lds_addr(sm), w))
+        if constexpr (NUW == 2) st = QPSK_LEAN_STREAM(fir_lean_loop2);
+        else st = QPSK_LEAN_STREAM(fir_lean_loop1);
+#undef QPSK_LEAN_STREAM
+    }
     bool ok = st == 0;
     if (ok) {
         for (int c = nchunks - DR; c < nchunks && ok; c++) {
@@ -172,8 +260,8 @@
             if (ok)
 #pragma unroll
                 for (int ui = 0; ui < NUW; ui++) {
-                    const int g = UF * (u0 + ui) + fl;
-                    flush_records<GM, R, DATA>(a, zring, dring, g, f0 + g, q, c, lean_unit_rows(a, f0, u0 + ui) + (size_t)fl * N);
+                    const int g2 = UF * (u0 + ui) + fl;
+                    flush_records<GM, R, DATA>(a, zring, dring, g2, f0 + g2, q, c, lean_unit_rows(a, f0, u0 + ui) + (size_t)fl * N);
                 }
         }
     } else if (lane == 0) {
@@ -192,14 +280,15 @@
     extern __shared__ __attribute__((aligned(16))) unsigned char smem_raw[];
     lean::Ctl *sm = reinterpret_cast<lean::Ctl *>(smem_raw);
     const int G = a.G;
-    float2 *win = reinterpret_cast<float2 *>(smem_raw + sizeof(lean::Ctl));
-    unsigned char *rows = reinterpret_cast<unsigned char *>(win + (size_t)nwin * UF * lean::WS);
+    float2 *win = lean::windows(smem_raw);
+    unsigned char *rows = lean::ring_rows(smem_raw, nwin);
     const int tid = threadIdx.x, lane = tid & 63;
     const int wave = __builtin_amdgcn_readfirstlane(tid >> 6);
     const int f0 = blockIdx.x * G;
     const int nchunks = a.nsym / S;
 
     prof::timeline_entry(a, tid);
+    lean::touch_kernargs();
     if (tid < MAX_WAVES) sm->ready[tid] = 0;
     if (tid == 0) { sm->consumed = 0; sm->abort_flag = 0; }
     const int *est = nullptr;
@@ -234,6 +323,22 @@
         }
         est = eidx;
     }
+    int u0, widx;
+    const int mine = lean::wave_units(layout, wave, a.lean_twowin, u0, widx);
+    if (a.lean_image && !a.index && !a.est_tw && wave != 0 && mine != 0) {
+        const uint4 *ip = a.lean_image + (size_t)wave * lean::IMG_QUADS * 64 + lane;
+        const uint4 q0 = ip[0], q1 = ip[64], q2 = ip[128], q3 = ip[192];
+        __syncthreads();
+        const lean::LeanLaneGeom geo = {LeanLaneAddr{{{q0.x, q0.y}, {q0.z, q0.w}}, {{q1.x, q1.y}, {q1.z, q1.w}}, {q2.x, q2.y}, {q2.z, q2.w}, q3.x, q3.y},
+                                        q3.z, q3.w};
+        prof::timeline_stamp(a, lane, 16 + wave);
+        float2 *mywin = win + (size_t)widx * UF * lean::WS;
+        if (mine == 2)
+            fir_wave_lean<2, DATA, true>(a, sm, rows, mywin, wave, u0, f0, lane, nchunks, status, nullptr, geo);
+        else
+            fir_wave_lean<1, DATA, true>(a, sm, rows, mywin, wave, u0, f0, lane, nchunks, status, nullptr, geo);
+        return;
+    }
     __syncthreads();
 
     if (wave == 0) {
@@ -249,20 +354,13 @@
                         f0, lane, nchunks, status);
         return;
     }
-    const int mine = wave < 16 ? (int)((layout >> (4 * wave)) & 15) : 0;
     if (mine == 0) return;
     prof::timeline_stamp(a, lane, 16 + wave);
-    int u0 = 0, widx = 0;
-    for (int v = 1; v < wave; v++) {
-        const int cv = (int)((layout >> (4 * v)) & 15);
-        u0 += cv;
-        widx += a.lean_twowin ? cv : (cv != 0);
-    }
     float2 *mywin = win + (size_t)widx * UF * lean::WS;
     if (mine == 2)
-        fir_wave_lean<2, DATA>(a, sm, rows, mywin, wave, u0, f0, lane, nchunks, status, est);
+        fir_wave_lean<2, DATA, false>(a, sm, rows, mywin, wave, u0, f0, lane, nchunks, status, est, lean::LeanLaneGeom{});
     else
-        fir_wave_lean<1, DATA>(a, sm, rows, mywin, wave, u0, f0, lane, nchunks, status, est);
+        fir_wave_lean<1, DATA, false>(a, sm, rows, mywin, wave, u0, f0, lane, nchunks, status, est, lean::LeanLaneGeom{});
 }
 
 size_t lean_lds_bytes(int G, int nwin)
@@ -336,10 +434,29 @@
     return lean_geometry(a, G, layout).est_ok;
 }
 
+bool lean_image_key(const FusedArgs &a, int G, unsigned long long layout, LeanImageKey *key)
+{
+    const LeanGeometry g = lean_geometry(a, G, layout);
+    if (!g.ok || a.index || a.est_tw) return false;
+    *key = LeanImageKey{layout, G, g.nwin, g.twowin ? 1 : 0, a.lean_dma ? 1 : 0, a.fixed_index, a.nsym, g.pair ? 1 : 0, a.data_rule ? 1 : 0, g.hw};
+    return true;
+}
+
+size_t lean_image_bytes(const LeanImageKey &key) { return sizeof(uint4) * 64 * (size_t)lean::IMG_QUADS * (size_t)key.hw; }
+
+int launch_lean_image_build(const LeanImageKey &key, void *image, hipStream_t s)
+{
+    if (key.hw < 2 || key.hw > lean::HW_WAVES || !image) return (int)hipErrorInvalidValue;
+    hipLaunchKernelGGL(lean_image_build_kernel, dim3(key.hw), dim3(64), 0, s, static_cast<uint4 *>(image), key.layout, key.nwin, key.twowin,
+                       key.lean_dma, key.fixed_index, key.nsym);
+    return (int)hipGetLastError();
+}
+
 int launch_rx_lean(const FusedArgs &a0, int G, unsigned long long layout, int *status, hipStream_t s)
 {
     FusedArgs a = a0;
     const LeanGeometry g = lean_geometry(a, G, layout);
+    if (a.index || a.est_tw) a.lean_image = nullptr;
     if (!g.ok || !lean_shape_ok(a, G) || (a.nframes % G != 0 && !a.sym_pad)) return (int)hipErrorInvalidValue;
     if (a.est_tw && (!g.est_ok || !a.est_cs || a.index)) return (int)hipErrorInvalidValue;
     a.G = G;
diff --git a/qpsk_amd/lib.py b/qpsk_amd/lib.py
--- a/qpsk_amd/lib.py
+++ b/qpsk_amd/lib.py
@@ -52,7 +52,7 @@
     "qpsk_deframer_reset_coded", "qpsk_deframer_push_coded",
     "qpsk_soft_batch", "qpsk_conv_encode_batch", "qpsk_viterbi_batch",
     "qpsk_punct_ntx", "qpsk_conv_encode_punct_batch", "qpsk_viterbi_punct_batch", "qpsk_deframer_reset_coded_punct",
-    "qpsk_test_viterbi_launches", "qpsk_test_deframer_advance", "qpsk_test_fir_runs",
+    "qpsk_test_viterbi_launches", "qpsk_test_deframer_advance", "qpsk_test_fir_runs", "qpsk_test_lean_image_builds",
     "qpsk_frame_len", "qpsk_frame_batch",
     "qpsk_ilv_stride", "qpsk_conv_encode_ilv_batch", "qpsk_viterbi_ilv_batch", "qpsk_frame_batch_ilv", "qpsk_deframer_reset_coded_ilv",
     "qpsk_rs_generator", "qpsk_rs_encode_batch", "qpsk_rs_decode_batch",
@@ -162,6 +162,8 @@
     L.qpsk_ctx_check.argtypes = [vp]
     L.qpsk_test_hist_state.argtypes = [vp, C.POINTER(i32)]
     L.qpsk_test_viterbi_launches.argtypes = [vp, C.POINTER(i32)]
+    if hasattr(L, "qpsk_test_lean_image_builds"):
+        L.qpsk_test_lean_image_builds.argtypes = [vp, C.POINTER(i32)]
     L.qpsk_test_deframer_advance.argtypes = [vp, C.c_longlong]
     L.qpsk_viterbi_stream_reset.argtypes = [vp, i32, i32, i32, i32, u32, u32]
     L.qpsk_viterbi_stream_emits.argtypes = [vp, i32]
@@ -298,6 +300,11 @@
     def viterbi_launches(self):
         n = C.c_int(-1)
         self._check(self.L.qpsk_test_viterbi_launches(self.h, C.byref(n)))
+        return n.value
+
+    def lean_image_builds(self):
+        n = C.c_int(-1)
+        self._check(self.L.qpsk_test_lean_image_builds(self.h, C.byref(n)))
         return n.value
 
     def deframer_advance(self, delta):
```
